# xmlyqing00/V-FloodNet

Measured on AMD Instinct MI355X. Metric: segmented frames/sec at 480p, higher is better.
Workload: dtype f32

## Files before the change

### v-floodnet_amd/_lib.py

```python
import ctypes as C
import os
import re

import torch

_HERE = os.path.dirname(os.path.abspath(__file__))
LIB_PATH = os.environ.get('VFN_LIB_PATH') or os.path.join(_HERE, 'libvfn_hip.so')

_lib = None

c_fp = C.c_void_p

_SCALARS = {'int': C.c_int, 'float': C.c_float, 'double': C.c_double, 'long long': C.c_longlong}
_POINTEES = set(_SCALARS) | {'void', 'char', 'unsigned char', 'short', 'unsigned short', 'unsigned long long'}
_RENAMED = {'in': 'inp'}
_DECLARATOR = re.compile(r'(?:const\s+)?([A-Za-z_][\w ]*?)(?:\s*(\*)\s*|\s+)(\w+)\s*(?:\[([^\]]*)\])?')


def parse_header(text):
    defines, enums, structs, protos = {}, {}, {}, {}

    def fail(why, decl):
        raise RuntimeError(f'vfn_hip.h: {why}: {" ".join(decl.split())[:120]!r}')

    def number(expr, decl):
        try:
            if not re.fullmatch(r'[\w\s()+*-]+', expr):
                raise ValueError(expr)
            return int(eval(expr, {'__builtins__': {}}, {**defines, **enums}))
        except Exception:
            fail(f'cannot evaluate {expr.strip()!r}', decl)

    def declarator(item, decl, param):
        m = _DECLARATOR.fullmatch(item.strip())
        if not m:
            fail('declaration not understood', decl)
        base, star, name, bound = ' '.join(m.group(1).split()), m.group(2), m.group(3), m.group(4)
        if base not in _POINTEES and base not in structs:
            fail(f'unknown base type {base!r}', decl)
        if bound is not None and (star or param):
            fail('array of pointers or array parameter', decl)
        if star:
            if base == 'char':
                t = C.c_char_p
            elif base in structs and param and not name.endswith('_dev'):
                t = C.POINTER(structs[base])
            else:
                t = C.c_void_p
        elif base in _SCALARS:
            t = _SCALARS[base]
        elif base in structs and not param:
            t = structs[base]
        else:
            fail(f'{base!r} by value', decl)
        return _RENAMED.get(name, name), t if bound is None else t * number(bound, decl)

    text = re.sub(r'/\*.*?\*/', ' ', text, flags=re.S)
    text = re.sub(r'//[^\n]*', ' ', text)
    text = re.sub(r'^[ \t]*#[ \t]*ifdef[ \t]+__cplusplus\b.*?^[ \t]*#[ \t]*endif\b[^\n]*$', ' ', text, flags=re.S | re.M)
    code = []
    for line in text.split('\n'):
        if not line.lstrip().startswith('#'):
            code.append(line)
        elif not re.fullmatch(r'\s*#\s*(ifndef\s+\w+|define\s+\w+|endif)\s*', line):
            m = re.fullmatch(r'\s*#\s*define\s+(\w+)\b(?!\()(.+)', line)
            if not m:
                fail('directive not understood', line)
            defines[m.group(1)] = number(m.group(2), line)
    text = '\n'.join(code)

    decls, depth, start = [], 0, 0
    for pos, ch in enumerate(text):
        depth += (ch == '{') - (ch == '}')
        if depth < 0:
            fail('unbalanced declaration', text[start:pos + 1])
        if ch == ';' and depth == 0:
            decls.append(text[start:pos])
            start = pos + 1
    if text[start:].strip():
        fail('unbalanced declaration', text[start:])

    for decl in decls:
        m = re.fullmatch(r'\s*enum\s*\{(.*)\}\s*', decl, flags=re.S)
        if m:
            value = -1
            for item in m.group(1).split(','):
                name, _, expr = item.partition('=')
                value = number(expr, decl) if expr.strip() else value + 1
                enums[name.strip()] = value
            continue
        m = re.fullmatch(r'\s*typedef\s+struct\s*(\w*)\s*\{(.*)\}\s*(\w+)\s*', decl, flags=re.S)
        if m:
            if m.group(1) not in ('', m.group(3)):
                fail('struct tag and typedef name differ', decl)
            fields = []
            for member in m.group(2).split(';'):
                if member.strip():
                    first, *more = member.split(',')
                    head = _DECLARATOR.fullmatch(first.strip())
                    if more and (not head or head.group(2)):
                        fail('several declarators after a pointer', member)
                    fields.append(declarator(first, member, False))
                    fields += [declarator(f'{head.group(1)} {item}', member, False) for item in more]
            structs[m.group(3)] = type(m.group(3), (C.Structure,), {'_fields_': fields})
            continue
        m = re.fullmatch(r'\s*int\s+(vfn_\w+)\s*\((.*)\)\s*', decl, flags=re.S)
        if m:
            if m.group(1) in protos:
                fail('declared twice', decl)
            params = m.group(2).strip()
            protos[m.group(1)] = [] if params == 'void' else [declarator(p, decl, True)[1] for p in params.split(',')]
            continue
        fail('declaration not understood', decl)
    return defines, enums, structs, protos


with open(os.path.join(os.path.dirname(_HERE), 'include', 'vfn_hip.h')) as _f:
    DEFINES, ENUMS, STRUCTS, SIGNATURES = parse_header(_f.read())
ALL_SYMBOLS = sorted(SIGNATURES)
ABI_VERSION = DEFINES['VFN_ABI_VERSION']
TRAIN_AUG_MAX_T, TRAIN_AUG_MAX_SIDE, TRAIN_AUG_MAX_OUT, TRAIN_AUG_MAX_OBJ = (
    DEFINES['VFN_TRAIN_AUG_MAX_' + _k] for _k in ('T', 'SIDE', 'OUT', 'OBJ'))

ConvDesc = STRUCTS['vfn_conv_desc']
WgradDesc = STRUCTS['vfn_wgrad_desc']
RefreshFilter = STRUCTS['vfn_refresh_filter']
RefreshEpilogue = STRUCTS['vfn_refresh_epilogue']
GatherEntry = STRUCTS['vfn_gather_entry']
StemDesc = STRUCTS['vfn_stem_desc']
BankScanDesc = STRUCTS['vfn_bankscan_desc']
MemReadDesc = STRUCTS['vfn_memread_desc']
BankMatchDesc = STRUCTS['vfn_bankmatch_desc']
BankDesc = STRUCTS['vfn_bank_desc']
TrainAugFrame = STRUCTS['vfn_train_aug_frame']
TrainAugDesc = STRUCTS['vfn_train_aug_desc']

DESC_IDS = {ENUMS['VFN_DESC_' + _k]: _c for _k, _c in (
    ('CONV', ConvDesc), ('STEM', StemDesc), ('BANKSCAN', BankScanDesc), ('MEMREAD', MemReadDesc), ('BANK', BankDesc),
    ('WGRAD', WgradDesc), ('REFRESH_FILTER', RefreshFilter), ('REFRESH_EPILOGUE', RefreshEpilogue), ('GATHER', GatherEntry),
    ('BANKMATCH', BankMatchDesc), ('TRAIN_AUG', TrainAugDesc))}


def lib():
    global _lib
    if _lib is None:
        if not os.path.isfile(LIB_PATH):
            raise RuntimeError(
                f'{LIB_PATH} not found: build the HIP kernels first '
                '(python -c "import __graft_entry__ as g; g.build()" or make -C v-floodnet_amd/csrc)')
        L = C.CDLL(LIB_PATH)

        def declare(name):
            if not hasattr(L, name):
                raise RuntimeError(f'{LIB_PATH} lacks {name}, which include/vfn_hip.h declares: rebuild it (make -C v-floodnet_amd/csrc)')
            fn = getattr(L, name)
            fn.argtypes, fn.restype = SIGNATURES[name], C.c_int
            return fn

        if declare('vfn_abi_version')() != ABI_VERSION:
            raise RuntimeError(f'{LIB_PATH} has ABI version {L.vfn_abi_version()}, this package expects {ABI_VERSION} '
                               '(descriptor layouts differ): rebuild it (make -C v-floodnet_amd/csrc)')
        declare('vfn_sizeof_desc')
        for which, cls in DESC_IDS.items():
            if L.vfn_sizeof_desc(which) != C.sizeof(cls):
                raise RuntimeError(f'{LIB_PATH}: sizeof({cls.__name__}) is {L.vfn_sizeof_desc(which)} in the library, '
                                   f'{C.sizeof(cls)} in this binding: rebuild it (make -C v-floodnet_amd/csrc)')
        for name in SIGNATURES:
            declare(name)
        _lib = L
    return _lib


def check(status, what):
    if status != 0:
        raise RuntimeError(f'HIP kernel launcher {what} failed with status {status}')


def ptr(t):
    if t is None:
        return None
    return C.c_void_p(t.data_ptr())


_raw_stream = getattr(torch._C, '_cuda_getCurrentRawStream', None)


def stream():
    if _raw_stream is not None:
        return C.c_void_p(_raw_stream(torch.cuda.current_device()))
    return C.c_void_p(torch.cuda.current_stream().cuda_stream)


def require_gpu(t, what='tensor'):
    if not t.is_cuda:
        raise RuntimeError(f'{what} must live on the GPU: the V-FloodNet hot path has no CPU fallback')


PROBES = []


def independent_stream(device, beside=(), tries=12, priority=0):
    device = torch.device(device)
    cur = torch.cuda.current_stream(device)
    others = [cur] + [s_ for s_ in beside if s_ is not None]
    big, small = torch.zeros(16 * 1024 * 1024, device=device), torch.zeros(16, device=device)

    def overlaps(cand, ref):
        torch.cuda.synchronize(device)
        ref_end, cand_end = torch.cuda.Event(), torch.cuda.Event()
        with torch.cuda.stream(ref):
            for _ in range(64):
                big.add_(1.0)
            ref_end.record()
        with torch.cuda.stream(cand):
            small.add_(1.0)
            cand_end.record()
        cand_end.synchronize()
        ok = not ref_end.query()
        torch.cuda.synchronize(device)
        return ok

    cand = None
    for n_ in range(tries):
        cand = torch.cuda.Stream(device=device, priority=priority)
        if all(overlaps(cand, o_) for o_ in others):
            PROBES.append((True, n_ + 1))
            return cand
    PROBES.append((False, tries))
    import warnings
    warnings.warn('vfloodnet_amd: no stream with a hardware queue of its own found; side-stream work will run in order with the frame loop')
    return cand
```

### v-floodnet_amd/csrc/conv_winograd.hip

```cpp
#include "common.h"
#include "conv_internal.h"
#include "../../include/vfn_hip.h"

namespace {

__device__ __forceinline__ void bt6(const f32x4 (&v)[6], f32x4 (&t)[6]) {
    t[0] = 4.f * v[0] - 5.f * v[2] + v[4];
    t[1] = -4.f * (v[1] + v[2]) + v[3] + v[4];
    t[2] = 4.f * (v[1] - v[2]) - v[3] + v[4];
    t[3] = -2.f * v[1] - v[2] + 2.f * v[3] + v[4];
    t[4] = 2.f * v[1] - v[2] - 2.f * v[3] + v[4];
    t[5] = 4.f * v[1] - 5.f * v[3] + v[5];
}

template <bool LPOUT = false>
__global__ __launch_bounds__(256)
void winograd_input_kernel(const float* __restrict__ x, int N, int H, int W, int C, int ld_x, int relu, float* __restrict__ V,
                           int rows_pad) {
    const int th = (H + 3) / 4, tw = (W + 3) / 4;
    const int c4n = C / 4;
    const long long total = (long long)N * th * tw * c4n;
    const __amdgpu_buffer_rsrc_t rx = __builtin_amdgcn_make_buffer_rsrc(const_cast<float*>(x), 0, (int)((size_t)N * H * W * ld_x * 4), 0x00020000);
    const float floor_ = relu ? 0.f : -INFINITY;
    for (long long i = vfn_xcd_block(blockIdx.x, gridDim.x) * (long long)blockDim.x + threadIdx.x; i < total; i += (long long)gridDim.x * blockDim.x) {
        const int c4 = (int)(i % c4n);
        const int tile = (int)(i / c4n);
        const int tx = tile % tw, ty = (tile / tw) % th, n = tile / (tw * th);
        f32x4 d[6][6];
#pragma unroll
        for (int a = 0; a < 6; ++a) {
            const int yy = 4 * ty - 1 + a;
#pragma unroll
            for (int b = 0; b < 6; ++b) {
                const int xx = 4 * tx - 1 + b;
                const bool ok = (unsigned)yy < (unsigned)H && (unsigned)xx < (unsigned)W;
                const int off = ok ? (((n * H + yy) * W + xx) * ld_x + c4 * 4) * 4 : 0x7ffffff0;
                d[a][b] = __builtin_bit_cast(f32x4, __builtin_amdgcn_raw_buffer_load_b128(rx, off, 0, 0));
            }
        }
#pragma unroll
        for (int a = 0; a < 6; ++a)
#pragma unroll
            for (int b = 0; b < 6; ++b)
#pragma unroll
                for (int e = 0; e < 4; ++e) d[a][b][e] = vfn_floor_nan(d[a][b][e], floor_);
#pragma unroll
        for (int b = 0; b < 6; ++b) {
            f32x4 v[6], t[6];
#pragma unroll
            for (int a = 0; a < 6; ++a) v[a] = d[a][b];
            bt6(v, t);
#pragma unroll
            for (int a = 0; a < 6; ++a) d[a][b] = t[a];
        }
#pragma unroll
        for (int a = 0; a < 6; ++a) {
            f32x4 t[6];
            bt6(d[a], t);
#pragma unroll
            for (int b = 0; b < 6; ++b) {
                if constexpr (LPOUT) {
                    const vfn_bf16x4 h = {(__bf16)t[b][0], (__bf16)t[b][1], (__bf16)t[b][2], (__bf16)t[b][3]};
                    *reinterpret_cast<vfn_bf16x4*>(reinterpret_cast<__bf16*>(V) + ((size_t)(a * 6 + b) * rows_pad + tile) * C + c4 * 4) = h;
                } else {
                    *reinterpret_cast<f32x4*>(V + ((size_t)(a * 6 + b) * rows_pad + tile) * C + c4 * 4) = t[b];
                }
            }
        }
    }
}

__device__ __forceinline__ void at6(const f32x4 (&m)[6], f32x4 (&y)[4]) {
    const f32x4 s12 = m[1] + m[2], d12 = m[1] - m[2], s34 = m[3] + m[4], d34 = m[3] - m[4];
    y[0] = m[0] + s12 + s34;
    y[1] = d12 + 2.f * d34;
    y[2] = s12 + 4.f * s34;
    y[3] = d12 + 8.f * d34 + m[5];
}

template <bool MASK>
__global__ __launch_bounds__(256)
void winograd_output_kernel(const float* __restrict__ Mb, int rows_pad, int N, int H, int W, int Cout,
                            const float* __restrict__ scale, const float* __restrict__ shift, const float* __restrict__ res, int res_ld,
                            int res_mod, int relu_out, float* __restrict__ out, int out_ld, const float* __restrict__ mask, int mask_ld,
                            int mask_after) {
    const int th = (H + 3) / 4, tw = (W + 3) / 4;
    const int c4n = Cout / 4;
    const long long total = (long long)N * th * tw * c4n;
    const int npix = N * H * W;
    const __amdgpu_buffer_rsrc_t ro = __builtin_amdgcn_make_buffer_rsrc(out, 0, (int)((size_t)npix * out_ld * 4), 0x00020000);
    const __amdgpu_buffer_rsrc_t rr = __builtin_amdgcn_make_buffer_rsrc(const_cast<float*>(res ? res : Mb), 0,
                                                                        res ? (int)((size_t)(res_mod > 0 ? res_mod : npix) * res_ld * 4) : 0, 0x00020000);
    const __amdgpu_buffer_rsrc_t rm = __builtin_amdgcn_make_buffer_rsrc(const_cast<float*>(MASK ? mask : Mb), 0,
                                                                        MASK ? (int)((size_t)npix * mask_ld * 4) : 0, 0x00020000);
    const float floor_ = relu_out ? 0.f : -INFINITY;
    for (long long i = vfn_xcd_block(blockIdx.x, gridDim.x) * (long long)blockDim.x + threadIdx.x; i < total; i += (long long)gridDim.x * blockDim.x) {
        const int c4 = (int)(i % c4n);
        const int tile = (int)(i / c4n);
        const int tx = tile % tw, ty = (tile / tw) % th, n = tile / (tw * th);
        f32x4 m[6][6];
#pragma unroll
        for (int a = 0; a < 6; ++a)
#pragma unroll
            for (int b = 0; b < 6; ++b) m[a][b] = *reinterpret_cast<const f32x4*>(Mb + ((size_t)(a * 6 + b) * rows_pad + tile) * Cout + c4 * 4);
        f32x4 sc = {1.f, 1.f, 1.f, 1.f}, sh = {0.f, 0.f, 0.f, 0.f};
        if (scale) sc = *reinterpret_cast<const f32x4*>(scale + c4 * 4);
        if (shift) sh = *reinterpret_cast<const f32x4*>(shift + c4 * 4);
        f32x4 t[6][4];
#pragma unroll
        for (int a = 0; a < 6; ++a) at6(m[a], t[a]);
        int rowi[4][4];
#pragma unroll
        for (int a = 0; a < 4; ++a)
#pragma unroll
            for (int b = 0; b < 4; ++b) {
                const int yy = 4 * ty + a, xx = 4 * tx + b;
                rowi[a][b] = (yy < H && xx < W) ? (n * H + yy) * W + xx : -1;
            }
        f32x4 rv[4][4], mk[MASK ? 4 : 1][MASK ? 4 : 1];
#pragma unroll
        for (int a = 0; a < 4; ++a)
#pragma unroll
            for (int b = 0; b < 4; ++b) {
                const int row = rowi[a][b];
                const int rrow = res_mod > 0 ? row % res_mod : row;
                rv[a][b] = __builtin_bit_cast(f32x4, __builtin_amdgcn_raw_buffer_load_b128(rr, row >= 0 ? (rrow * res_ld + c4 * 4) * 4 : 0x7ffffff0, 0, 0));
                if constexpr (MASK)
                    mk[a][b] = __builtin_bit_cast(f32x4, __builtin_amdgcn_raw_buffer_load_b128(rm, row >= 0 ? (row * mask_ld + c4 * 4) * 4 : 0x7ffffff0, 0, 0));
            }
#pragma unroll
        for (int b = 0; b < 4; ++b) {
            f32x4 col[6], y[4];
#pragma unroll
            for (int a = 0; a < 6; ++a) col[a] = t[a][b];
            at6(col, y);
#pragma unroll
            for (int a = 0; a < 4; ++a) {
                f32x4 v;
#pragma unroll
                for (int e = 0; e < 4; ++e) v[e] = y[a][e] * sc[e] + sh[e];
                if constexpr (MASK) {
                    if (!mask_after) {
#pragma unroll
                        for (int e = 0; e < 4; ++e) v[e] = mk[a][b][e] > 0.f ? v[e] : 0.f;
                    }
                }
                v += rv[a][b];
                if constexpr (MASK) {
                    if (mask_after) {
#pragma unroll
                        for (int e = 0; e < 4; ++e) v[e] = mk[a][b][e] > 0.f ? v[e] : 0.f;
                    }
                }
#pragma unroll
                for (int e = 0; e < 4; ++e) v[e] = vfn_floor_nan(v[e], floor_);
                const int row = rowi[a][b];
                __builtin_amdgcn_raw_buffer_store_b128(__builtin_bit_cast(__attribute__((ext_vector_type(4))) unsigned, v), ro,
                                                       row >= 0 ? (row * out_ld + c4 * 4) * 4 : 0x7ffffff0, 0, 0);
            }
        }
    }
}

__device__ __forceinline__ void a6(const f32x4 (&v)[4], f32x4 (&z)[6]) {
    const f32x4 e = v[0] + v[2], o = v[1] + v[3];
    const f32x4 e4 = v[0] + 4.f * v[2], o8 = 2.f * v[1] + 8.f * v[3];
    z[0] = v[0];
    z[1] = e + o;
    z[2] = e - o;
    z[3] = e4 + o8;
    z[4] = e4 - o8;
    z[5] = v[3];
}

__global__ __launch_bounds__(256)
void winograd_gy_kernel(const float* __restrict__ gy, int N, int H, int W, int C, int ld, float* __restrict__ Z, int rows_pad) {
    const int th = (H + 3) / 4, tw = (W + 3) / 4;
    const int c4n = C / 4;
    const long long total = (long long)N * th * tw * c4n;
    for (long long i = vfn_xcd_block(blockIdx.x, gridDim.x) * (long long)blockDim.x + threadIdx.x; i < total; i += (long long)gridDim.x * blockDim.x) {
        const int c4 = (int)(i % c4n);
        const int tile = (int)(i / c4n);
        const int tx = tile % tw, ty = (tile / tw) % th, n = tile / (tw * th);
        f32x4 t[6][4];
#pragma unroll
        for (int b = 0; b < 4; ++b) {
            f32x4 col[4], z[6];
            const int xx = 4 * tx + b;
#pragma unroll
            for (int a = 0; a < 4; ++a) {
                const int yy = 4 * ty + a;
                f32x4 v = {0.f, 0.f, 0.f, 0.f};
                if (yy < H && xx < W) v = *reinterpret_cast<const f32x4*>(gy + ((size_t)(n * H + yy) * W + xx) * ld + c4 * 4);
                col[a] = v;
            }
            a6(col, z);
#pragma unroll
            for (int a = 0; a < 6; ++a) t[a][b] = z[a];
        }
#pragma unroll
        for (int a = 0; a < 6; ++a) {
            f32x4 z[6];
            a6(t[a], z);
#pragma unroll
            for (int b = 0; b < 6; ++b)
                *reinterpret_cast<f32x4*>(Z + ((size_t)(a * 6 + b) * rows_pad + tile) * C + c4 * 4) = z[b];
        }
    }
}

__device__ __forceinline__ void gt3(const f32x4 (&u)[6], f32x4 (&w)[3]) {
    const f32x4 s12 = u[1] + u[2], d12 = u[2] - u[1], s34 = u[3] + u[4], d34 = u[3] - u[4];
    w[0] = 0.25f * u[0] - (1.f / 6.f) * s12 + (1.f / 24.f) * s34;
    w[1] = (1.f / 6.f) * d12 + (1.f / 12.f) * d34;
    w[2] = -(1.f / 6.f) * s12 + (1.f / 6.f) * s34 + u[5];
}

__global__ __launch_bounds__(256)
void winograd_dw_kernel(const float* __restrict__ dU, int Cout, int Cin, const float* __restrict__ rowscale, float* __restrict__ dw,
                        int accumulate) {
    const int c4n = Cin / 4;
    const long long total = (long long)Cout * c4n;
    const size_t bank = (size_t)Cout * Cin;
    for (long long i = vfn_xcd_block(blockIdx.x, gridDim.x) * (long long)blockDim.x + threadIdx.x; i < total; i += (long long)gridDim.x * blockDim.x) {
        const int c4 = (int)(i % c4n), co = (int)(i / c4n);
        f32x4 t[3][6];
#pragma unroll
        for (int j = 0; j < 6; ++j) {
            f32x4 u[6], w[3];
#pragma unroll
            for (int a = 0; a < 6; ++a) u[a] = *reinterpret_cast<const f32x4*>(dU + (size_t)(a * 6 + j) * bank + (size_t)co * Cin + c4 * 4);
            gt3(u, w);
#pragma unroll
            for (int a = 0; a < 3; ++a) t[a][j] = w[a];
        }
        const float sc = rowscale ? rowscale[co] : 1.f;
#pragma unroll
        for (int a = 0; a < 3; ++a) {
            f32x4 w[3];
            gt3(t[a], w);
#pragma unroll
            for (int b = 0; b < 3; ++b) {
                f32x4* o = reinterpret_cast<f32x4*>(dw + ((size_t)co * 9 + a * 3 + b) * Cin + c4 * 4);
                f32x4 v = w[b] * sc;
                if (accumulate) v += *o;
                *o = v;
            }
        }
    }
}


struct wino_gemm_args {
    const float* V;
    const float* U;
    float* Mb;
    int comps, rows_pad, C, Cout, cout_pad;
    int mtiles, ntiles;
    int a_ld, out_ld, res_ld, res_mod, relu_in, relu_out;
    const float* scale;
    const float* shift;
    const float* res;
};

template <int BM, int BN, int WM, int WN, int PD, bool CONV = false, bool LP = false>
__global__ __launch_bounds__(WM * WN * 64)
void wino_gemm_kernel(const wino_gemm_args p) {
    static_assert(!(CONV && LP), "the reduced-precision form is the transform-domain GEMM only");
    constexpr int BK = 32;
    constexpr int KT = LP ? 64 : 32;
    constexpr int ES = LP ? 2 : 4;
    constexpr int NT = WM * WN * 64;
    constexpr int TM = BM / WM / 32, TN = BN / WN / 32;
    constexpr int AC = BM * 8 / NT, BC = BN * 8 / NT, RSTEP = NT / 8;
    static_assert(AC >= 1 && BC >= 1, "tile too small for the thread count");
    extern __shared__ __attribute__((aligned(16))) char smem[];
    float* sA = reinterpret_cast<float*>(smem);
    float* sB = sA + 2 * BM * BK;

    const int tid = threadIdx.x, lane = tid & 63, wave = tid >> 6;
    const int wm = wave / WN, wn = wave % WN;
    const int li = lane & 31, lh = lane >> 5;

    const int per = p.mtiles * p.ntiles, total = p.comps * per;
    const int gx = (int)gridDim.x >> 3, xcd = (int)blockIdx.x & 7, loc = (int)blockIdx.x >> 3;
    const int q = total >> 3, r8 = total & 7;
    const int u_begin = xcd < r8 ? xcd * (q + 1) : r8 * (q + 1) + (xcd - r8) * q;
    const int u_end = u_begin + q + (xcd < r8 ? 1 : 0);
    const int first = u_begin + loc;
    const int n_units = first < u_end ? (u_end - first + gx - 1) / gx : 0;
    const int nk = p.C / KT;
    const int T = n_units * nk;
    if (T == 0) return;

    const int c16 = tid & 7, r0 = tid >> 3;
    const int a_ld = CONV ? p.a_ld : p.C;
    const __amdgpu_buffer_rsrc_t rsV = __builtin_amdgcn_make_buffer_rsrc(const_cast<float*>(p.V), 0, (int)((size_t)p.comps * p.rows_pad * a_ld * ES), 0x00020000);
    const __amdgpu_buffer_rsrc_t rsU = __builtin_amdgcn_make_buffer_rsrc(const_cast<float*>(p.U), 0, (int)((size_t)p.comps * p.cout_pad * p.C * ES), 0x00020000);
    int a_thr[AC], b_thr[BC];
#pragma unroll
    for (int j = 0; j < AC; ++j) a_thr[j] = (r0 + j * RSTEP) * a_ld * ES + c16 * 16;
#pragma unroll
    for (int j = 0; j < BC; ++j) b_thr[j] = (r0 + j * RSTEP) * p.C * ES + c16 * 16;

    int lu = 0, lkt = 0, la_base = 0, lb_base = 0;
    int n0_cur = 0;
    auto unit_bases = [&](int ui, int& a_base, int& b_base, size_t& o_base, int* n0 = nullptr) {
        const int u = first + ui * gx;
        const int xi = u / per, rem = u - xi * per;
        const int mt = rem / p.ntiles, nt = rem - mt * p.ntiles;
        a_base = (xi * p.rows_pad + mt * BM) * a_ld * ES;
        b_base = (xi * p.cout_pad + nt * BN) * p.C * ES;
        o_base = CONV ? (size_t)mt * BM : ((size_t)xi * p.rows_pad + mt * BM) * p.Cout + nt * BN;
        if (n0) *n0 = nt * BN;
    };
    size_t o_dummy;
    unit_bases(0, la_base, lb_base, o_dummy);
    f32x4 ra[PD][AC], rb[PD][BC];
    auto request = [&](int slot) {
        const int koff = lkt * 128;
#pragma unroll
        for (int j = 0; j < AC; ++j)
            ra[slot][j] = __builtin_bit_cast(f32x4, __builtin_amdgcn_raw_buffer_load_b128(rsV, a_thr[j], la_base + koff, 0));
#pragma unroll
        for (int j = 0; j < BC; ++j)
            rb[slot][j] = __builtin_bit_cast(f32x4, __builtin_amdgcn_raw_buffer_load_b128(rsU, b_thr[j], lb_base + koff, 0));
        if (++lkt == nk) {
            lkt = 0;
            if (++lu < n_units) unit_bases(lu, la_base, lb_base, o_dummy);
        }
    };
    const float relu_floor = (CONV && p.relu_in) ? 0.f : -INFINITY;
    auto stage = [&](int buf, int slot) {
        float* dA = sA + buf * BM * BK;
        float* dB = sB + buf * BN * BK;
#pragma unroll
        for (int j = 0; j < AC; ++j) {
            const int r = r0 + j * RSTEP;
            f32x4 v = ra[slot][j];
            if constexpr (CONV) {
#pragma unroll
                for (int e = 0; e < 4; ++e) v[e] = fmaxf(v[e], relu_floor);
            }
            *reinterpret_cast<f32x4*>(dA + r * BK + ((c16 ^ ((r >> 1) & 7)) << 2)) = v;
        }
#pragma unroll
        for (int j = 0; j < BC; ++j) {
            const int r = r0 + j * RSTEP;
            *reinterpret_cast<f32x4*>(dB + r * BK + ((c16 ^ ((r >> 1) & 7)) << 2)) = rb[slot][j];
        }
    };

    f32x16 acc[TM][TN];
#pragma unroll
    for (int i = 0; i < TM; ++i)
#pragma unroll
        for (int j = 0; j < TN; ++j)
#pragma unroll
            for (int r = 0; r < 16; ++r) acc[i][j][r] = 0.f;

    int cu = 0, ckt = 0, ca_dummy, cb_dummy;
    size_t o_base;
    unit_bases(0, ca_dummy, cb_dummy, o_base, &n0_cur);

#pragma unroll
    for (int d = 0; d < PD; ++d)
        if (d < T) request(d);
    stage(0, 0);
    __syncthreads();

    for (int t0 = 0; t0 < T; t0 += PD) {
#pragma unroll
        for (int uu = 0; uu < PD; ++uu) {
            const int t = t0 + uu;
            if (t >= T) break;
            const int buf = t & 1;
            const bool more = t + 1 < T;
            const bool more_req = t + PD < T;
            const float* cA = sA + buf * BM * BK + (wm * TM * 32) * BK;
            const float* cB = sB + buf * BN * BK + (wn * TN * 32) * BK;
            auto read_frags = [&](int kk, f32x4 (&a)[TM], f32x4 (&b)[TN]) {
                const int lc = 2 * kk + lh;
#pragma unroll
                for (int i = 0; i < TM; ++i) {
                    const int r = i * 32 + li;
                    a[i] = *reinterpret_cast<const f32x4*>(cA + r * BK + ((lc ^ ((r >> 1) & 7)) << 2));
                }
#pragma unroll
                for (int j = 0; j < TN; ++j) {
                    const int r = j * 32 + li;
                    b[j] = *reinterpret_cast<const f32x4*>(cB + r * BK + ((lc ^ ((r >> 1) & 7)) << 2));
                }
            };
            f32x4 fa[2][TM], fb[2][TN];
            read_frags(0, fa[0], fb[0]);
#pragma unroll
            for (int kk = 0; kk < 4; ++kk) {
                if (PD > 1 && kk == 0 && more) stage(buf ^ 1, (uu + 1) % PD);
                if (kk == 1 && more_req) request(uu);
                if (PD == 1 && kk == 3 && more) stage(buf ^ 1, 0);
                if (kk + 1 < 4) read_frags(kk + 1, fa[(kk + 1) & 1], fb[(kk + 1) & 1]);
                if constexpr (LP) {
                    typedef __attribute__((ext_vector_type(8))) __bf16 bf16x8_;
#pragma unroll
                    for (int i = 0; i < TM; ++i)
#pragma unroll
                        for (int j = 0; j < TN; ++j)
                            acc[i][j] = __builtin_amdgcn_mfma_f32_32x32x16_bf16(__builtin_bit_cast(bf16x8_, fa[kk & 1][i]), __builtin_bit_cast(bf16x8_, fb[kk & 1][j]),
                                                                                acc[i][j], 0, 0, 0);
                } else {
#pragma unroll
                for (int e = 0; e < 4; ++e)
#pragma unroll
                    for (int i = 0; i < TM; ++i)
#pragma unroll
                        for (int j = 0; j < TN; ++j)
                            acc[i][j] = __builtin_amdgcn_mfma_f32_32x32x2f32(fa[kk & 1][i][e], fb[kk & 1][j][e], acc[i][j], 0, 0, 0);
                }
            }
            if (++ckt == nk) {
                if constexpr (CONV) {
                    const int m0 = (int)o_base;
                    const int npix = p.rows_pad;
                    const __amdgpu_buffer_rsrc_t rso = __builtin_amdgcn_make_buffer_rsrc(p.Mb, 0, (int)((size_t)npix * p.out_ld * 4), 0x00020000);
                    const __amdgpu_buffer_rsrc_t rsr = __builtin_amdgcn_make_buffer_rsrc(const_cast<float*>(p.res ? p.res : p.V), 0,
                        p.res ? (int)((size_t)(p.res_mod > 0 ? p.res_mod : npix) * p.res_ld * 4) : 0, 0x00020000);
                    const float floor_ = p.relu_out ? 0.f : -INFINITY;
                    float rv[TM][TN][16];
#pragma unroll
                    for (int j = 0; j < TN; ++j) {
                        const int col = n0_cur + (wn * TN + j) * 32 + li;
#pragma unroll
                        for (int i = 0; i < TM; ++i)
#pragma unroll
                            for (int r = 0; r < 16; ++r) {
                                const int row = m0 + (wm * TM + i) * 32 + 4 * lh + (r & 3) + 8 * (r >> 2);
                                const int rrow = p.res_mod > 0 ? row % p.res_mod : row;
                                rv[i][j][r] = __builtin_bit_cast(float, __builtin_amdgcn_raw_buffer_load_b32(
                                    rsr, (row < npix && col < p.Cout) ? (rrow * p.res_ld + col) * 4 : 0x7ffffff0, 0, 0));
                            }
                    }
#pragma unroll
                    for (int j = 0; j < TN; ++j) {
                        const int col = n0_cur + (wn * TN + j) * 32 + li;
                        const bool cok = col < p.Cout;
                        const float sc = (p.scale && cok) ? p.scale[col] : 1.f;
                        const float sh = (p.shift && cok) ? p.shift[col] : 0.f;
#pragma unroll
                        for (int i = 0; i < TM; ++i)
#pragma unroll
                            for (int r = 0; r < 16; ++r) {
                                const int row = m0 + (wm * TM + i) * 32 + 4 * lh + (r & 3) + 8 * (r >> 2);
                                const float v = vfn_floor_nan(acc[i][j][r] * sc + sh + rv[i][j][r], floor_);
                                __builtin_amdgcn_raw_buffer_store_b32(__builtin_bit_cast(unsigned, v), rso,
                                                                      (row < npix && cok) ? (row * p.out_ld + col) * 4 : 0x7ffffff0, 0, 0);
                                acc[i][j][r] = 0.f;
                            }
                    }
                } else {
                float* o = p.Mb + o_base;
#pragma unroll
                for (int j = 0; j < TN; ++j) {
                    const int col = (wn * TN + j) * 32 + li;
#pragma unroll
                    for (int i = 0; i < TM; ++i) {
                        const int rbase = (wm * TM + i) * 32 + 4 * lh;
#pragma unroll
                        for (int r = 0; r < 16; ++r) {
                            if (n0_cur + col < p.Cout)
                                o[(size_t)(rbase + (r & 3) + 8 * (r >> 2)) * p.Cout + col] = acc[i][j][r];
                            acc[i][j][r] = 0.f;
                        }
                    }
                }
                }
                ckt = 0;
                if (++cu < n_units) unit_bases(cu, ca_dummy, cb_dummy, o_base, &n0_cur);
            }
            __syncthreads();
        }
    }
}

template <int BM, int BN, int WM, int WN, int PD, bool CONV, bool LP>
int launch_wino_gemm(const wino_gemm_args& a, int wgs, hipStream_t s) {
    constexpr size_t lds = 2 * (size_t)(BM + BN) * 32 * sizeof(float);
    static const bool lds_ready = vfn_allow_lds(&wino_gemm_kernel<BM, BN, WM, WN, PD, CONV, LP>, lds);
    (void)lds_ready;
    wino_gemm_args p = a;
    p.mtiles = (a.rows_pad + BM - 1) / BM;
    p.ntiles = (a.Cout + BN - 1) / BN;
    const int total = p.comps * p.mtiles * p.ntiles;
    int grid = wgs > 0 ? wgs : 512;
    if (grid > total) grid = total;
    grid = (grid + 7) / 8 * 8;
    hipLaunchKernelGGL((wino_gemm_kernel<BM, BN, WM, WN, PD, CONV, LP>), dim3(grid), dim3(WM * WN * 64), lds, s, p);
    return vfn_check_launch();
}

constexpr int kWinoTile[4][4] = {{128, 128, 4, 2}, {64, 128, 2, 4}, {128, 64, 4, 2}, {64, 64, 2, 2}};
constexpr int kWinoCfgs = 8;

template <bool CONV, bool LP>
int launch_wino_cfg(const wino_gemm_args& a, int cfg, int wgs, hipStream_t s) {
    return vfn_dispatch<kWinoCfgs>(cfg, [&](auto id) -> int {
        constexpr int c = decltype(id)::value;
        constexpr const int* t = kWinoTile[c & 3];
        return launch_wino_gemm<t[0], t[1], t[2], t[3], 1 + (c >> 2), CONV, LP>(a, wgs, s);
    });
}

inline bool tensors_fit_32bit(int N, int H, int W, int ld, int res_ld, int mask_ld, int res_mod) {
    const long long px = (long long)N * H * W;
    return px * ld * 4 < 0x7fffff00LL && (res_mod > 0 ? (long long)res_mod : px) * res_ld * 4 < 0x7fffff00LL && px * mask_ld * 4 < 0x7fffff00LL;
}

inline int grid_of(long long total) {
    long long b = (total + 255) / 256;
    return (int)(b < 16384 ? (b ? b : 1) : 16384);
}

}

extern "C" int vfn_winograd_tiles(int N, int H, int W) { return N * ((H + 3) / 4) * ((W + 3) / 4); }

extern "C" int vfn_winograd_input_f32(const float* x, int N, int H, int W, int C, int ld_x, int relu, float* V, int rows_pad, void* stream) {
    if (!x || !V || N < 1 || H < 1 || W < 1 || C < 4 || C % 4 || ld_x < C || ld_x % 4 || rows_pad < vfn_winograd_tiles(N, H, W)) return VFN_ERR_ARG;
    const long long total = (long long)vfn_winograd_tiles(N, H, W) * (C / 4);
    if (!tensors_fit_32bit(N, H, W, ld_x, 0, 0, 0)) return VFN_ERR_ARG;
    hipLaunchKernelGGL(winograd_input_kernel<false>, dim3(grid_of(total)), dim3(256), 0, (hipStream_t)stream, x, N, H, W, C, ld_x, relu, V, rows_pad);
    return vfn_check_launch();
}

extern "C" int vfn_winograd_output_f32(const float* Mb, int rows_pad, int N, int H, int W, int Cout, const float* scale, const float* shift,
                                       const float* res, int res_ld, int res_mod, int relu_out, float* out, int out_ld, void* stream) {
    if (!Mb || !out || N < 1 || H < 1 || W < 1 || Cout < 4 || Cout % 4 || out_ld < Cout || out_ld % 4 || (res && res_ld % 4) ||
        rows_pad < vfn_winograd_tiles(N, H, W)) return VFN_ERR_ARG;
    const long long total = (long long)vfn_winograd_tiles(N, H, W) * (Cout / 4);
    if (!tensors_fit_32bit(N, H, W, out_ld, res ? res_ld : 0, 0, res_mod)) return VFN_ERR_ARG;
    hipLaunchKernelGGL(winograd_output_kernel<false>, dim3(grid_of(total)), dim3(256), 0, (hipStream_t)stream, Mb, rows_pad, N, H, W, Cout, scale, shift,
                       res, res_ld, res_mod, relu_out, out, out_ld, (const float*)nullptr, 0, 0);
    return vfn_check_launch();
}

extern "C" int vfn_winograd_output_masked_f32(const float* Mb, int rows_pad, int N, int H, int W, int Cout, const float* res, int res_ld,
                                              const float* mask, int mask_ld, int mask_after, float* out, int out_ld, void* stream) {
    if (!Mb || !out || N < 1 || H < 1 || W < 1 || Cout < 4 || Cout % 4 || out_ld < Cout || out_ld % 4 || (res && res_ld % 4) ||
        (mask && mask_ld % 4) || rows_pad < vfn_winograd_tiles(N, H, W)) return VFN_ERR_ARG;
    const long long total = (long long)vfn_winograd_tiles(N, H, W) * (Cout / 4);
    if (!tensors_fit_32bit(N, H, W, out_ld, res ? res_ld : 0, mask ? mask_ld : 0, 0)) return VFN_ERR_ARG;
    if (mask)
        hipLaunchKernelGGL(winograd_output_kernel<true>, dim3(grid_of(total)), dim3(256), 0, (hipStream_t)stream, Mb, rows_pad, N, H, W, Cout,
                           (const float*)nullptr, (const float*)nullptr, res, res_ld, 0, 0, out, out_ld, mask, mask_ld, mask_after);
    else
        hipLaunchKernelGGL(winograd_output_kernel<false>, dim3(grid_of(total)), dim3(256), 0, (hipStream_t)stream, Mb, rows_pad, N, H, W, Cout,
                           (const float*)nullptr, (const float*)nullptr, res, res_ld, 0, 0, out, out_ld, (const float*)nullptr, 0, 0);
    return vfn_check_launch();
}

extern "C" int vfn_winograd_gy_f32(const float* gy, int N, int H, int W, int C, int ld, float* Z, int rows_pad, void* stream) {
    if (!gy || !Z || N < 1 || H < 1 || W < 1 || C < 4 || C % 4 || ld < C || ld % 4 || rows_pad < vfn_winograd_tiles(N, H, W)) return VFN_ERR_ARG;
    const long long total = (long long)vfn_winograd_tiles(N, H, W) * (C / 4);
    hipLaunchKernelGGL(winograd_gy_kernel, dim3(grid_of(total)), dim3(256), 0, (hipStream_t)stream, gy, N, H, W, C, ld, Z, rows_pad);
    return vfn_check_launch();
}

extern "C" int vfn_winograd_dw_f32(const float* dU, int Cout, int Cin, const float* rowscale, float* dw, int accumulate, void* stream) {
    if (!dU || !dw || Cout < 1 || Cin < 4 || Cin % 4) return VFN_ERR_ARG;
    hipLaunchKernelGGL(winograd_dw_kernel, dim3(grid_of((long long)Cout * (Cin / 4))), dim3(256), 0, (hipStream_t)stream, dU, Cout, Cin, rowscale,
                       dw, accumulate);
    return vfn_check_launch();
}

extern "C" int vfn_winograd_gemm_f32(const float* V, const float* U, float* Mb, int comps, int rows_pad, int C, int Cout, int cout_pad, int cfg,
                                     int wgs, void* stream) {
    if (!V || !U || !Mb || comps < 1 || rows_pad < 1 || C < 32 || C % 32 || Cout < 1 || cout_pad < Cout || cfg < 0 || cfg >= kWinoCfgs) return VFN_ERR_ARG;
    const int bm = kWinoTile[cfg & 3][0], bn = kWinoTile[cfg & 3][1];
    if (rows_pad % bm || cout_pad < (Cout + bn - 1) / bn * bn) return VFN_ERR_ARG;
    if ((long long)comps * rows_pad * C * 4 >= 0x7fffff00LL || (long long)comps * cout_pad * C * 4 >= 0x7fffff00LL) return VFN_ERR_ARG;
    wino_gemm_args a{V, U, Mb, comps, rows_pad, C, Cout, cout_pad, 0, 0, 0, 0, 0, 0, 0, 0, nullptr, nullptr, nullptr};
    return launch_wino_cfg<false, false>(a, cfg, wgs, (hipStream_t)stream);
}

extern "C" int vfn_conv1x1_persistent_f32(const vfn_conv_desc* d, int cfg, int wgs, void* stream) {
    if (!d || !d->in || !d->w || !d->out || cfg < 0 || cfg >= kWinoCfgs) return VFN_ERR_ARG;
    if (d->KH != 1 || d->KW != 1 || d->stride != 1 || d->pad != 0 || d->mask || d->in_lp || d->out_lp || d->w_packed || d->ksplit > 1 ||
        d->w_batch_rows || d->Cin % 32 || d->in_ld % 4 || d->M < 1 || d->M != d->N * d->H * d->W) return VFN_ERR_ARG;
    const int bn = kWinoTile[cfg & 3][1];
    if (d->cout_pad < (d->Cout + bn - 1) / bn * bn) return VFN_ERR_ARG;
    const long long lim = 0x7fffff00LL;
    if ((long long)d->M * d->in_ld * 4 >= lim || (long long)d->M * d->out_ld * 4 >= lim || (long long)d->cout_pad * d->Cin * 4 >= lim ||
        (d->res && (long long)(d->res_mod > 0 ? d->res_mod : d->M) * d->res_ld * 4 >= lim)) return VFN_ERR_ARG;
    wino_gemm_args a{d->in, d->w, d->out, 1, d->M, d->Cin, d->Cout, d->cout_pad, 0, 0,
                     d->in_ld, d->out_ld, d->res ? d->res_ld : 0, d->res_mod, d->relu_in, d->relu_out, d->scale, d->shift, d->res};
    return launch_wino_cfg<true, false>(a, cfg, wgs, (hipStream_t)stream);
}

extern "C" int vfn_winograd_input_bf16(const float* x, int N, int H, int W, int C, int ld_x, int relu, void* V, int rows_pad, void* stream) {
    if (!x || !V || N < 1 || H < 1 || W < 1 || C < 4 || C % 4 || ld_x < C || ld_x % 4 || rows_pad < vfn_winograd_tiles(N, H, W)) return VFN_ERR_ARG;
    const long long total = (long long)vfn_winograd_tiles(N, H, W) * (C / 4);
    if (!tensors_fit_32bit(N, H, W, ld_x, 0, 0, 0)) return VFN_ERR_ARG;
    hipLaunchKernelGGL(winograd_input_kernel<true>, dim3(grid_of(total)), dim3(256), 0, (hipStream_t)stream, x, N, H, W, C, ld_x, relu,
                       reinterpret_cast<float*>(V), rows_pad);
    return vfn_check_launch();
}

extern "C" int vfn_winograd_gemm_bf16(const void* V, const void* U, float* Mb, int comps, int rows_pad, int C, int Cout, int cout_pad, int cfg,
                                      int wgs, void* stream) {
    if (!V || !U || !Mb || comps < 1 || rows_pad < 1 || C < 64 || C % 64 || Cout < 1 || cout_pad < Cout || cfg < 0 || cfg >= kWinoCfgs) return VFN_ERR_ARG;
    const int bm = kWinoTile[cfg & 3][0], bn = kWinoTile[cfg & 3][1];
    if (rows_pad % bm || cout_pad < (Cout + bn - 1) / bn * bn) return VFN_ERR_ARG;
    if ((long long)comps * rows_pad * C * 2 >= 0x7fffff00LL || (long long)comps * cout_pad * C * 2 >= 0x7fffff00LL) return VFN_ERR_ARG;
    wino_gemm_args a{reinterpret_cast<const float*>(V), reinterpret_cast<const float*>(U), Mb, comps, rows_pad, C, Cout, cout_pad, 0, 0, 0, 0, 0, 0, 0, 0,
                     nullptr, nullptr, nullptr};
    return launch_wino_cfg<false, true>(a, cfg, wgs, (hipStream_t)stream);
}
```

### v-floodnet_amd/csrc/refresh.hip

```cpp
#include "common.h"
#include "../../include/vfn_hip.h"

namespace {

constexpr int ELEMS_PER_BLOCK = 4096;

__device__ __forceinline__ float bn_scale(const float* gamma, const float* var, float eps, int c) {
    return __fdiv_rn(gamma[c], __fsqrt_rn(__fadd_rn(var[c], eps)));
}

__global__ __launch_bounds__(256)
void refresh_filters_kernel(const vfn_refresh_filter* __restrict__ table, int n) {
    int lo = 0, hi = n - 1;
    while (lo < hi) {
        const int mid = (lo + hi + 1) >> 1;
        if (table[mid].block0 <= (int)blockIdx.x) lo = mid; else hi = mid - 1;
    }
    const vfn_refresh_filter e = table[lo];
    const int T = e.kh * e.kw;
    const long long base = (long long)((int)blockIdx.x - e.block0) * ELEMS_PER_BLOCK;
    if (e.kind >= 4) {
        const long long pairs = (long long)e.cout * e.cin;
        const double G[6][3] = {{0.25, 0.0, 0.0}, {-1.0 / 6, -1.0 / 6, -1.0 / 6}, {-1.0 / 6, 1.0 / 6, -1.0 / 6},
                                {1.0 / 24, 1.0 / 12, 1.0 / 6}, {1.0 / 24, -1.0 / 12, 1.0 / 6}, {0.0, 0.0, 1.0}};
        for (int i = threadIdx.x; i < ELEMS_PER_BLOCK; i += 256) {
            const long long idx = base + i;
            if (idx >= pairs) return;
            int co, ci;
            if (e.kind == 4) { ci = (int)(idx % e.cin); co = (int)(idx / e.cin); }
            else { co = (int)(idx % e.cout); ci = (int)(idx / e.cout); }
            const float* g = e.src + ((size_t)co * e.cin_total + e.cin_off + ci) * 9;
            const float sc = e.gamma ? bn_scale(e.gamma, e.var, e.eps, co) : 1.f;
            double w[3][3];
#pragma unroll
            for (int t = 0; t < 9; ++t) {
                float v = g[e.kind == 4 ? t : 8 - t];
                if (e.gamma) v = __fmul_rn(v, sc);
                w[t / 3][t % 3] = (double)v;
            }
            double tmp[6][3];
#pragma unroll
            for (int a = 0; a < 6; ++a)
#pragma unroll
                for (int b = 0; b < 3; ++b) tmp[a][b] = G[a][0] * w[0][b] + G[a][1] * w[1][b] + G[a][2] * w[2][b];
            const size_t row = e.kind == 4 ? (size_t)(e.dst_row0 + co) : (size_t)(e.dst_row0 + ci);
            const size_t col = e.kind == 4 ? (size_t)ci : (size_t)(e.dst_col0 + co);
#pragma unroll
            for (int a = 0; a < 6; ++a)
#pragma unroll
                for (int b = 0; b < 6; ++b) {
                    const double u = tmp[a][0] * G[b][0] + tmp[a][1] * G[b][1] + tmp[a][2] * G[b][2];
                    e.dst[((size_t)(a * 6 + b) * e.cout_ld + row) * e.dst_ld + col] = (float)u;
                }
        }
        return;
    }
    const long long total = (long long)e.cout * e.cin * T;
    if (e.kind <= 1 && T == 9) {
        const long long pairs = (long long)e.cout * e.cin;
        const int per = ELEMS_PER_BLOCK / 9 + 1;
        for (int i = threadIdx.x; i < per; i += 256) {
            const long long idx = (long long)((int)blockIdx.x - e.block0) * per + i;
            if (idx >= pairs) return;
            int co, ci;
            if (e.kind == 0) { ci = (int)(idx % e.cin); co = (int)(idx / e.cin); }
            else { co = (int)(idx % e.cout); ci = (int)(idx / e.cout); }
            const float* g = e.src + ((size_t)co * e.cin_total + e.cin_off + ci) * 9;
            const float sc = e.gamma ? bn_scale(e.gamma, e.var, e.eps, co) : 1.f;
#pragma unroll
            for (int t = 0; t < 9; ++t) {
                float v = g[t];
                if (e.gamma) v = __fmul_rn(v, sc);
                const size_t dst = e.kind == 0 ? (size_t)(e.dst_row0 + co) * e.dst_ld + (size_t)t * e.cin + ci
                                               : (size_t)(e.dst_row0 + ci) * e.dst_ld + (size_t)(8 - t) * e.cout_ld + e.dst_col0 + co;
                e.dst[dst] = v;
            }
        }
        return;
    }
    for (int i = threadIdx.x; i < ELEMS_PER_BLOCK; i += 256) {
        const long long idx = base + i;
        if (idx >= total) return;
        int co, ci, t;
        size_t dst;
        if (e.kind == 0) {
            ci = (int)(idx % e.cin);
            t = (int)((idx / e.cin) % T);
            co = (int)(idx / ((long long)e.cin * T));
            dst = (size_t)(e.dst_row0 + co) * e.dst_ld + (size_t)t * e.cin + ci;
        } else if (e.kind == 1) {
            co = (int)(idx % e.cout);
            const int tf = (int)((idx / e.cout) % T);
            ci = (int)(idx / ((long long)e.cout * T));
            t = T - 1 - tf;
            dst = (size_t)(e.dst_row0 + ci) * e.dst_ld + (size_t)tf * e.cout_ld + e.dst_col0 + co;
        } else if (e.kind == 2) {
            co = (int)(idx % e.cout);
            t = (int)((idx / e.cout) % T);
            ci = (int)(idx / ((long long)e.cout * T));
            const int y = t / e.kw, x = t % e.kw;
            dst = ((size_t)((e.dst_row0 + ci) * e.kh + y) * 8 + x) * e.dst_ld + co;
        } else {
            ci = (int)(idx % e.cin);
            co = (int)((idx / e.cin) % e.cout);
            t = (int)(idx / ((long long)e.cin * e.cout));
            dst = (size_t)(e.dst_row0 + t * e.cout + co) * e.dst_ld + ci;
        }
        float v = e.src[((size_t)co * e.cin_total + e.cin_off + ci) * T + t];
        if (e.gamma) v = __fmul_rn(v, bn_scale(e.gamma, e.var, e.eps, co));
        e.dst[dst] = v;
    }
}

__global__ __launch_bounds__(256)
void refresh_epilogues_kernel(const vfn_refresh_epilogue* __restrict__ table) {
    const vfn_refresh_epilogue e = table[blockIdx.x];
    for (int c = threadIdx.x; c < e.C; c += 256) {
        if (e.gamma) {
            const float s = bn_scale(e.gamma, e.var, e.eps, c);
            if (e.scale) e.scale[c] = s;
            if (e.shift) e.shift[c] = __fsub_rn(e.beta[c], __fmul_rn(e.mean[c], s));
        } else if (e.shift) {
            e.shift[c] = e.beta ? e.beta[c] : 0.f;
        }
    }
}

}

extern "C" int vfn_refresh_elems_per_block(void) { return ELEMS_PER_BLOCK; }

extern "C" int vfn_refresh_filters_f32(const vfn_refresh_filter* table, int n, int total_blocks, void* stream) {
    if (!table || n < 1 || total_blocks < 1) return VFN_ERR_ARG;
    hipLaunchKernelGGL(refresh_filters_kernel, dim3(total_blocks), dim3(256), 0, (hipStream_t)stream, table, n);
    return vfn_check_launch();
}

extern "C" int vfn_refresh_epilogues_f32(const vfn_refresh_epilogue* table, int n, void* stream) {
    if (!table || n < 1) return VFN_ERR_ARG;
    hipLaunchKernelGGL(refresh_epilogues_kernel, dim3(n), dim3(256), 0, (hipStream_t)stream, table);
    return vfn_check_launch();
}

namespace {
__global__ __launch_bounds__(256)
void gather_strided_kernel(const vfn_gather_entry* __restrict__ table, int n, float* __restrict__ dst) {
    int lo = 0, hi = n - 1;
    while (lo < hi) {
        const int mid = (lo + hi + 1) >> 1;
        if (table[mid].block0 <= (int)blockIdx.x) lo = mid; else hi = mid - 1;
    }
    const vfn_gather_entry e = table[lo];
    const long long total = (long long)e.shape[0] * e.shape[1] * e.shape[2] * e.shape[3];
    const long long base = (long long)((int)blockIdx.x - e.block0) * ELEMS_PER_BLOCK;
    float* out = dst + e.dst_offset;
    for (int i = threadIdx.x; i < ELEMS_PER_BLOCK; i += 256) {
        const long long idx = base + i;
        if (idx >= total) return;
        long long r = idx;
        const int i3 = (int)(r % e.shape[3]); r /= e.shape[3];
        const int i2 = (int)(r % e.shape[2]); r /= e.shape[2];
        const int i1 = (int)(r % e.shape[1]);
        const int i0 = (int)(r / e.shape[1]);
        out[idx] = e.src[i0 * e.stride[0] + i1 * e.stride[1] + i2 * e.stride[2] + i3 * e.stride[3]];
    }
}
}

extern "C" int vfn_gather_strided_f32(const vfn_gather_entry* table, int n, int total_blocks, float* dst, void* stream) {
    if (!table || !dst || n < 1 || total_blocks < 1) return VFN_ERR_ARG;
    hipLaunchKernelGGL(gather_strided_kernel, dim3(total_blocks), dim3(256), 0, (hipStream_t)stream, table, n, dst);
    return vfn_check_launch();
}
```

### v-floodnet_amd/engine.py

```python
import math
import os

import torch

from . import _lib, ops, weights as W
from ._lib import ptr, stream, check, MemReadDesc, BankScanDesc
from .feature_bank import pick_nsplit, pick_scan_slices, MAX_SPLIT, MAX_SPLIT_SCAN, QT_SCAN, DK, DV

_CFG_EFF = {(128, 128): 1.00, (128, 64): 0.95, (64, 128): 0.95, (64, 64): 0.86, (32, 64): 0.74,
            (64, 32): 0.74, (128, 32): 0.80, (256, 128): 0.97}
_CFG_TILES = None
_TUNED = {}
_TUNED_PATH = __import__('os').path.join(__import__('os').path.dirname(__import__('os').path.abspath(__file__)),
                                         'tuned_gfx950.json')
_TUNED_BF16 = {}
_TUNED_BF16_PATH = _TUNED_PATH.replace('tuned_gfx950.json', 'tuned_gfx950_bf16.json')
_TUNED_BF16X3 = {}
_TUNED_BF16X3_PATH = _TUNED_PATH.replace('tuned_gfx950.json', 'tuned_gfx950_bf16x3.json')
_TABLES = (_TUNED, _TUNED_BF16, _TUNED_BF16X3)
_TABLE_PATHS = (_TUNED_PATH, _TUNED_BF16_PATH, _TUNED_BF16X3_PATH)


def _load_tuned():
    import json
    import os
    if os.environ.get('VFN_IGNORE_TUNED') == '1':
        return
    for path, table in zip(_TABLE_PATHS, _TABLES):
        alt = os.environ.get('VFN_TUNED_DIR')
        if alt and os.path.isfile(os.path.join(alt, os.path.basename(path))):
            path = os.path.join(alt, os.path.basename(path))
        if os.path.isfile(path):
            for k, v in json.load(open(path)).items():
                t = (int(v[0]), int(v[1]), int(v[2]) if len(v) > 2 else 0)
                table[tuple(int(x) for x in k.split(','))] = t + tuple(int(x) for x in v[3:6]) if len(v) >= 6 else t


def save_tuned(path=None, mode=0):
    import json
    table = _TABLES[mode]
    with open(path or _TABLE_PATHS[mode], 'w') as f:
        json.dump({','.join(str(x) for x in k): list(v) for k, v in sorted(table.items())}, f, indent=0)


_load_tuned()


def pad_divide_by(h, w, d=16):
    new_h = h + d - h % d if h % d > 0 else h
    new_w = w + d - w % d if w % d > 0 else w
    lh = int((new_h - h) / 2)
    uh = int(new_h - h) - lh
    lw = int((new_w - w) / 2)
    uw = int(new_w - w) - lw
    return (lw, uw, lh, uh), new_h, new_w


WS_FLOATS = 16 * 1024 * 1024
_WINOGRAD_TRAIN = os.environ.get('VFN_WINOGRAD_TRAIN', '1') == '1'
_BATCH_MEMREAD = os.environ.get('VFN_TRAIN_BATCH_MEMREAD', '1') == '1'
MAX_GROUP = 16
_TRAIN_SLOTS = int(os.environ.get('VFN_TRAIN_SLOTS', 2))
_WINOGRAD = os.environ.get('VFN_WINOGRAD', '1')
_WINOGRAD_LP = os.environ.get('VFN_WINOGRAD_LP', '1') == '1'
_WINOGRAD_MIN_M = int(os.environ.get('VFN_WINOGRAD_MIN_M', 10000))
_WINO_TABLE = {}
_WINO_TABLE_BF16 = {}
_WINO_PATH = os.path.join(os.path.dirname(os.path.abspath(__file__)), 'wino_gfx950.json')
if os.environ.get('VFN_IGNORE_TUNED') != '1':
    for _path, _tab in ((_WINO_PATH, _WINO_TABLE), (_WINO_PATH.replace('.json', '_bf16.json'), _WINO_TABLE_BF16)):
        if os.path.isfile(_path):
            _tab.update({tuple(int(x) for x in k.split(',')): int(v) for k, v in __import__('json').load(open(_path)).items()})
_INLAUNCH_SPLITK = __import__('os').environ.get('VFN_INLAUNCH_SPLITK', '1') == '1'


def _tiles():
    global _CFG_TILES
    if _CFG_TILES is None:
        _CFG_TILES = ops.conv_cfg_tiles()
    return _CFG_TILES


def apply_choice(desc, choice, ws, counters=None):
    cfg, ks, split_from = choice[:3]
    if ks > 1 and (desc.out_ld % 4 or (desc.res and desc.res_ld % 4)):
        ks, split_from = 1, 0
    if cfg >= ops.PCONV_CFG0 and not ops.pconv_eligible(desc, 0):
        fb = tuple(choice[3:6]) if len(choice) >= 6 else choose_cfg(desc.M, desc.Cout, desc.KH * desc.KW * desc.Cin, 0, use_table=False)
        return apply_choice(desc, fb, ws, counters)
    if cfg >= ops.WINO_GEMM_CFG0:
        ops.set_splitk(desc, 1, None)
        return cfg
    if ops.conv_cfg_kind(cfg) == 2:
        if counters is None or ws is None or ws.numel() < ops.SK_WS_FLOATS:
            ws, counters = ops.streamk_scratch(ws.device if ws is not None else torch.device('cuda', torch.cuda.current_device()))
        ops.set_streamk(desc, ws, counters)
        return cfg
    if ks > 1:
        bm, bn = _tiles()[cfg]
        n_tiles = (desc.Cout + bn - 1) // bn
        rows = desc.M - (split_from // n_tiles) * bm
        if desc.Cout % bn or not _INLAUNCH_SPLITK or ops.conv_cfg_kind(cfg) != 0 or desc.w_packed or desc.in_lp or desc.out_lp:
            counters = None
        ops.set_splitk(desc, ks, ws, split_from, rows, counters)
    else:
        ops.set_splitk(desc, 1, None)
    return cfg


def _scores_buffer(p, fb):
    if os.environ.get('VFN_STORE_SCORES', '1') == '0':
        return None
    per_obj = ((fb._cap + 63) // 64) * ((p.HW + 127) // 128) * 8192
    if fb.obj_n * per_obj * 4 > float(os.environ.get('VFN_SCORES_MAX_GB', 48)) * 2 ** 30:
        return None
    key = (fb.obj_n, per_obj)
    if getattr(p, '_scores_key', None) != key:
        p._scores = torch.empty(fb.obj_n, per_obj, device=p.dec_in.device)
        p._scores_key = key
    return p._scores


def choose_cfg(M, cout, K, mode=0, use_table=True):
    global _CFG_TILES
    key = (M, cout, K)
    table = _TABLES[mode]
    if use_table and key in table:
        return table[key]
    _tiles()
    nk = K // (64 if mode == 1 else 32)
    best, best_cost = 0, None
    for c, (bm, bn) in enumerate(_CFG_TILES[:8]):
        if bn > 32 and cout <= 32:
            continue
        if bn >= 128 and cout < 128:
            continue
        blocks = ((M + bm - 1) // bm) * ((cout + bn - 1) // bn)
        rounds = (blocks + 255) // 256
        cost = rounds * bm * bn / _CFG_EFF[(bm, bn)]
        if best_cost is None or cost < best_cost:
            best, best_cost = c, cost
    c = 2 if cout >= 128 else 3
    bm, bn = _CFG_TILES[c]
    blocks = ((M + bm - 1) // bm) * ((cout + bn - 1) // bn)
    if blocks < 200 and nk >= 16 and cout % 4 == 0 and cout >= 64:
        ks = max(1, min(16, (448 + blocks - 1) // blocks, nk // 4))
        while ks > 1 and (((nk + ks - 1) // ks) * (ks - 1) >= nk or ks * M * cout > WS_FLOATS):
            ks -= 1
        return (c, ks, 0)
    return (best, 1, 0)


def tune_desc(d, bf, ws, cnt, iters=3, cfg_filter=None, allow_split=True):
    tiles = ops.conv_cfg_tiles()
    key = (d.M, d.Cout, d.KH * d.KW * d.Cin)

    def timeit(c):
        ops.conv2d_launch(d, c, bf)
        torch.cuda.synchronize()
        best_ms = None
        for _ in range(3):
            e0, e1 = torch.cuda.Event(enable_timing=True), torch.cuda.Event(enable_timing=True)
            e0.record()
            for _ in range(iters):
                ops.conv2d_launch(d, c, bf)
            e1.record()
            torch.cuda.synchronize()
            ms = e0.elapsed_time(e1)
            best_ms = ms if best_ms is None else min(best_ms, ms)
        return best_ms

    best, best_t = None, None
    if d.w_batch_rows > 0 and bf == 1:
        for c in ops.wino_gemm_cfg_options(d.w_batch_rows, d.Cout):
            if cfg_filter is not None and not cfg_filter(key, c):
                continue
            t = timeit(c)
            if best_t is None or t < best_t:
                best, best_t = (c, 1, 0), t
        return best
    if d.w_batch_rows > 0 and bf == 0 and d.M // d.w_batch_rows * d.w_batch_rows == d.M:
        for c in ops.wino_gemm_cfg_options(d.w_batch_rows, d.Cout):
            if cfg_filter is not None and not cfg_filter(key, c):
                continue
            apply_choice(d, (c, 1, 0), ws, cnt)
            try:
                t = timeit(c)
            except RuntimeError:
                continue
            if best_t is None or t < best_t:
                best, best_t = (c, 1, 0), t
    if ops.pconv_eligible(d, bf) and os.environ.get('VFN_PCONV', '1') == '1':
        for c in ops.pconv_cfg_options(d.Cout):
            if cfg_filter is not None and not cfg_filter(key, c):
                continue
            apply_choice(d, (c, 1, 0), ws, cnt)
            try:
                t = timeit(c)
            except RuntimeError:
                continue
            if best_t is None or t < best_t:
                best, best_t = (c, 1, 0), t
    for c, (bm, bn) in enumerate(tiles):
        if c not in ops.conv_cfgs(bf):
            continue
        if cfg_filter is not None and not cfg_filter(key, c):
            continue
        if d.cout_pad < ((d.Cout + bn - 1) // bn) * bn:
            continue
        if (bn > 64 and d.Cout <= 32) or (bn > 128 and d.Cout < 256):
            continue
        blocks = ((d.M + bm - 1) // bm) * ((d.Cout + bn - 1) // bn)
        options = [(c, 1, 0)]
        wk = ops.conv_cfg_wk(c)
        kind = ops.conv_cfg_kind(c)
        if kind == 2:
            if blocks > ops.SK_MAX_TILES:
                continue
        elif not allow_split:
            pass
        elif kind == 1 and wk > 1:
            if blocks < 256:
                options += [(c, k_, 0) for k_ in ops.valid_splits(d, 8, bf)[1:] if k_ * d.M * d.Cout <= WS_FLOATS]
        elif wk > 1 or ops.conv_cfg_tpb(c) > 1:
            if blocks > 1024 or d.KH * d.KW * d.Cin // (64 if bf == 1 else 32) < 2 * wk:
                continue
        elif blocks < 256:
            options += [(c, k_, 0) for k_ in ops.valid_splits(d, 16, bf)[1:] if k_ * d.M * d.Cout <= WS_FLOATS]
        else:
            options += [(c, k_, full) for (full, k_, rows) in ops.tail_split_options(d, bm, bn, 8, bf)
                        if k_ * rows * d.Cout <= WS_FLOATS and k_ in (2, 3, 4, 5, 6, 8)]
        for opt in options:
            apply_choice(d, opt, ws, cnt)
            t = timeit(c)
            if best_t is None or t < best_t:
                best, best_t = opt, t
    return best


class ConvLayer:

    def __init__(self, conv, bn=None, device=None, cin_range=None, with_bias=True, reg=None):
        w = conv.weight.detach().float()
        if cin_range is not None:
            w = w[:, cin_range[0]:cin_range[1]].contiguous()
        self.cout, self.cin, self.k, _ = w.shape
        self.stride = conv.stride[0]
        self.pad = conv.padding[0]
        self.w = ops.pad_rows(W.pack_conv_weight(w)).to(device)
        sc, sh = W.conv_epilogue(conv, bn)
        if not with_bias:
            sh = torch.zeros_like(sh)
        self.scale = sc.to(device).contiguous()
        self.shift = sh.to(device).contiguous()
        self._w_lp = {}
        self._wino_src = None
        if reg is not None and isinstance(conv, torch.nn.Module):
            from .refresh import FORWARD
            self._wino_src = [(reg, conv.weight, cin_range[0] if cin_range is not None else 0, 0)]
            reg.add_filter(conv.weight, self.w, FORWARD, cin=self.cin, cin_off=cin_range[0] if cin_range is not None else 0)
            if bn is not None:
                reg.add_epilogue(self.scale, self.shift if with_bias else None, bn=bn, eps=W.BN_EPS)
            elif conv.bias is not None and with_bias:
                reg.add_epilogue(None, self.shift, bias=conv.bias)

    def refresh_derived(self):
        for mode, t in self._w_lp.items():
            if mode == 'wino':
                if self._wino_src is not None:
                    continue
                w = self.w[:self.cout].view(self.cout, 3, 3, self.cin).permute(0, 3, 1, 2)
                t.copy_(ops.pack_winograd_weight(w).to(t.device))
            elif mode == 'wino_bf16':
                w = self.w[:self.cout].view(self.cout, 3, 3, self.cin).permute(0, 3, 1, 2)
                t.copy_(ops.pack_winograd_weight_bf16(w).to(t.device))
            else:
                new = ops.pack_weights_lp(self.w, mode)
                t.copy_(new)

    def w_lp(self, mode):
        if mode not in self._w_lp:
            self._w_lp[mode] = ops.pack_weights_lp(self.w, mode)
        return self._w_lp[mode]

    def w_wino(self):
        if 'wino' not in self._w_lp:
            assert self.k == 3
            w = self.w[:self.cout].view(self.cout, 3, 3, self.cin).permute(0, 3, 1, 2)
            self._w_lp['wino'] = ops.pack_winograd_weight(w).to(self.w.device)
            if self._wino_src is not None:
                from .refresh import WINO
                for reg, weight, cin_off, row0 in self._wino_src:
                    reg.add_filter(weight, self._w_lp['wino'], WINO, cin=self.cin, cin_off=cin_off, dst_ld=self.cin, dst_row0=row0,
                                   cout_ld=self._w_lp['wino'].shape[0] // 36)
        return self._w_lp['wino']

    def w_wino_bf16(self):
        if 'wino_bf16' not in self._w_lp:
            assert self.k == 3
            w = self.w[:self.cout].view(self.cout, 3, 3, self.cin).permute(0, 3, 1, 2)
            self._w_lp['wino_bf16'] = ops.pack_winograd_weight_bf16(w).to(self.w.device)
        return self._w_lp['wino_bf16']


class Pred2Layer:
    TAPS = 20

    def __init__(self, conv, device, reg=None):
        w = conv.weight.detach().float().cpu()
        assert w.shape[0] == 2 and w.shape[2:] == (3, 3)
        self.cin = w.shape[1]
        w18 = torch.zeros(self.TAPS, self.cin)
        for dy in range(3):
            for dx in range(3):
                for o in range(2):
                    w18[(dy * 3 + dx) * 2 + o] = w[o, :, dy, dx]
        self.cout, self.k, self.stride, self.pad = self.TAPS, 1, 1, 0
        self.w = ops.pad_rows(w18.contiguous()).to(device)
        self.scale = torch.ones(self.TAPS, device=device)
        self.shift = torch.zeros(self.TAPS, device=device)
        self.bias = conv.bias.detach().float().to(device).contiguous().clone()
        self._w_lp = {}
        self._wino_src = None
        if reg is not None:
            from .refresh import TAPS
            reg.add_filter(conv.weight, self.w, TAPS)
            reg.add_epilogue(None, self.bias, bias=conv.bias)

    refresh_derived = ConvLayer.refresh_derived

    def w_lp(self, mode):
        if mode not in self._w_lp:
            self._w_lp[mode] = ops.pack_weights_lp(self.w, mode)
        return self._w_lp[mode]


class Launch:
    __slots__ = ('fn', 'args', 'name', 'flops')

    def __init__(self, fn, args, name, flops=0.0):
        self.fn, self.args, self.name, self.flops = fn, args, name, flops

    def __call__(self):
        self.fn(*self.args)


_GRAPHS = os.environ.get('VFN_GRAPHS', '1') == '1'


class GraphCache:

    def __init__(self):
        self.graphs = {}
        self.runs = {}
        self.captures = 0

    def invalidate(self):
        self.graphs.clear()
        self.runs.clear()

    def run(self, lst, lo=0, hi=None, eager=False):
        hi = len(lst) if hi is None else hi
        if hi <= lo:
            return
        key = (id(lst), lo, hi)
        g = None if (eager or not _GRAPHS) else self.graphs.get(key)
        if g is not None:
            g.replay()
            return
        n = self.runs.get(key, 0)
        if eager or not _GRAPHS or n < 2 or hi - lo < 4:
            for l in lst[lo:hi]:
                l()
            if not eager:
                self.runs[key] = n + 1
            return
        g = torch.cuda.CUDAGraph()
        cur = torch.cuda.current_stream()
        cap = torch.cuda.Stream(device=cur.device)
        cap.wait_stream(cur)
        try:
            with torch.cuda.graph(g, stream=cap, capture_error_mode='thread_local'):
                for l in lst[lo:hi]:
                    l()
        except Exception:
            import warnings
            warnings.warn('vfloodnet_amd: HIP graph capture of a launch list failed; running it eagerly')
            self.runs[key] = -10 ** 9
            if torch.cuda.is_current_stream_capturing():
                raise RuntimeError('vfloodnet_amd: the stream is still capturing after a failed HIP graph capture')
            cur.wait_stream(cap)
            for l in lst[lo:hi]:
                l()
            return
        cur.wait_stream(cap)
        self.graphs[key] = g
        self.captures += 1
        g.replay()

    def warm(self, lst, lo=0, hi=None):
        hi = len(lst) if hi is None else hi
        if not _GRAPHS or hi - lo < 4:
            return
        key = (id(lst), lo, hi)
        while key not in self.graphs and self.runs.get(key, 0) >= 0:
            self.run(lst, lo, hi)


class FramePlan:

    def __init__(self, eng, H0, W0, obj_n, keep_acts=False):
        self.eng = eng
        self.graphs = GraphCache()
        self.keep_acts = keep_acts
        self.acts_m = {}
        self.H0, self.W0, self.obj_n = H0, W0, obj_n
        self.pad, self.Hp, self.Wp = pad_divide_by(H0, W0)
        dev = eng.device
        self.h2, self.w2 = self.Hp // 2, self.Wp // 2
        self.h4, self.w4 = self.Hp // 4, self.Wp // 4
        self.h8, self.w8 = self.Hp // 8, self.Wp // 8
        self.h16, self.w16 = self.Hp // 16, self.Wp // 16
        self.HW = self.h16 * self.w16
        f = lambda *s: torch.empty(*s, device=dev, dtype=torch.float32)
        K = obj_n
        self.frame_in = f(3, H0, W0)
        self.mask_in = f(K, H0, W0)
        self.qsets = [QuerySet(self), QuerySet(self)]
        self._qbatch = {}
        self.m = self._trunk_buffers(K)
        self.kv_m = f(K, self.HW, DK + DV)
        self.ml = f(K, self.HW, 2)
        self.ml_part = f(K, MAX_SPLIT_SCAN, self.HW, 2)
        self.work = torch.zeros(4, dtype=torch.int32, device=dev)
        self.o_part = f(K, MAX_SPLIT, self.HW, DV)
        self.dec_in = f(K, self.h16, self.w16, DV)
        self.d16 = [f(K, self.h16, self.w16, 256) for _ in range(3)]
        self.d8 = [f(K, self.h8, self.w8, 256) for _ in range(3)]
        self.d4 = [f(K, self.h4, self.w4, 256) for _ in range(3)]
        self.pp = f(K, self.h4, self.w4, 2)
        self.z4 = f(K, self.h4, self.w4, Pred2Layer.TAPS)
        self.z2 = f(K, self.h2, self.w2, Pred2Layer.TAPS)
        self.p_up = f(K, self.h2, self.w2, 2)
        self.rough = f(K, self.h2, self.w2)
        self.unc = f(self.h2, self.w2)
        fused_ok = K <= 4
        self.hs = None if fused_ok else f(K, self.h2, self.w2, 64)
        self.hr = None if fused_ok else f(K, self.h2, self.w2)
        self.hm = None if fused_ok else f(K, self.h2, self.w2)
        self.lm = f(K, self.h2, self.w2, 64)
        self.conf = f(K, self.h2, self.w2)
        self.l2 = [f(K, self.h2, self.w2, 32) for _ in range(3)]
        self.qq = f(K, self.h2, self.w2, 2)
        self.score = f(1, K, H0, W0)
        self._twins = {}
        self._lp_state = {}
        self.ws = f(WS_FLOATS)
        self.ws_q = f(WS_FLOATS)
        self.cnt = torch.zeros(ops.SK_MAX_TILES, dtype=torch.int32, device=dev)
        self.cnt_q = torch.zeros(ops.SK_MAX_TILES, dtype=torch.int32, device=dev)
        self._ws_cur, self._cnt_cur = self.ws, self.cnt
        self._wino = {}

        self.mem = []
        self._build()

    @property
    def seg_pre(self):
        return self.qsets[0].pre[1]

    @property
    def seg_post(self):
        return self.qsets[0].post[0]

    @property
    def kv_q(self):
        return self.qsets[0].kv_q[0:1]

    def all_lists(self):
        out = [self.mem]
        for qs in self.qsets:
            out += [qs.pre[1], qs.pre[2], qs.post[0], qs.post[1]]
        for qs in self._qbatch.values():
            out += [qs.pre[qs.nq]]
            if qs._dec_batch is not None:
                out += [qs._dec_batch.post]
        return out

    def batch_set(self, n):
        qs = self._qbatch.get(n)
        if qs is None:
            qs = self._qbatch[n] = QuerySet(self, nq=n)
            qs.build()
        return qs

    def _trunk_buffers(self, N):
        dev = self.eng.device
        f = lambda *s: torch.empty(*s, device=dev, dtype=torch.float32)
        b = {}
        b['r1'] = f(N, self.h2, self.w2, 64)
        b['x4'] = f(N, self.h4, self.w4, 64)
        for name, (h, w, planes) in {'res2': (self.h4, self.w4, 64), 'res3': (self.h8, self.w8, 128),
                                     'res4': (self.h16, self.w16, 256)}.items():
            hin, win = (h * 2, w * 2) if name != 'res2' else (h, w)
            b[name] = dict(t1a=f(N, hin, win, planes), t1=f(N, h, w, planes), t2=f(N, h, w, planes),
                           ds=f(N, h, w, planes * 4), o=[f(N, h, w, planes * 4) for _ in range(2)],
                           out=f(N, h, w, planes * 4))
        return b

    def _lp_args(self, out):
        if not self.eng.any_x3 or out.shape[-1] % 32:
            return ()
        self._lp_state[(out.data_ptr(), tuple(out.shape))] = True
        return (self.lp_twin(out), True)

    def lp_twin(self, t):
        st = t.untyped_storage()
        key = st.data_ptr()
        if key not in self._twins:
            self._twins[key] = torch.empty(st.nbytes() // 4, dtype=torch.float32, device=t.device)
        return torch.as_strided(self._twins[key], t.size(), t.stride(), t.storage_offset())

    def has_lp(self, t, relu):
        return self._lp_state.get((t.data_ptr(), tuple(t.shape))) == bool(relu)

    def _conv(self, lst, layer, x, out, N, H, Wd, res=None, relu_in=False, relu_out=False, name='conv',
              in_ld=None, out_ld=None, res_mod=0, lp_out=None, f32_out=True):
        bf = self.eng.layer_mode(name)
        lp = bf == 2
        if self.eng.mixed:
            f32_out = True
        if ((bf == 0 or (bf == 1 and _WINOGRAD_LP and not self.keep_acts and layer.cin % 64 == 0)) and in_ld is None and
                (_WINOGRAD_TRAIN or not self.keep_acts) and x.shape[-1] == layer.cin and self.eng.use_winograd(layer, N * H * Wd, bf)):
            return self._conv_winograd(lst, layer, x, out, N, H, Wd, res, relu_in, relu_out, name, out_ld, res_mod, bf)
        d = ops.make_conv_desc(x, layer.w, layer.cout, layer.k, layer.k, layer.stride, layer.pad, out,
                               layer.scale, layer.shift, res, relu_in, relu_out,
                               cin=layer.cin, in_ld=in_ld if in_ld is not None else x.shape[-1],
                               out_ld=out_ld, N=N, H=H, W=Wd)
        d.res_mod = int(res_mod)
        if lp and in_ld is None and layer.cin % 32 == 0 and self.has_lp(x, relu_in):
            d.inp, d.in_lp, d.relu_in = ptr(self.lp_twin(x)), 1, 0
        if lp and lp_out and layer.cout % 32 == 0 and d.out_ld % 32 == 0:
            d.out_lp, d.out_lp_relu = ptr(self.lp_twin(out)), int(lp_out == 'relu')
            self._lp_state[(out.data_ptr(), tuple(out.shape))] = (lp_out == 'relu')
            if not f32_out:
                d.out = None
        else:
            self._lp_state.pop((out.data_ptr(), tuple(out.shape)), None)
        K = layer.k * layer.k * layer.cin
        if bf == 1 and layer.cin % 64:
            bf = 2
        if bf:
            ops.use_packed_weights(d, layer.w_lp(bf))
        choice = choose_cfg(d.M, layer.cout, K, bf)
        if choice[1] > 1 and (d.out_ld % 4 or (res is not None and d.res_ld % 4)):
            choice = (choice[0], 1, 0)
        cfg = apply_choice(d, choice, self._ws_cur, self._cnt_cur)
        lst.append(Launch(ops.conv2d_launch, (d, cfg, bf), f'{name}[{d.M}x{layer.cout}x{K}]', 2.0 * d.M * layer.cout * K))
        return out

    def _conv_winograd(self, lst, layer, x, out, N, H, Wd, res, relu_in, relu_out, name, out_ld, res_mod, bf=0):
        rows = ops.winograd_rows(N, H, Wd)
        key = id(self._ws_cur)
        need_v, need_m = 36 * rows * layer.cin, 36 * rows * layer.cout
        V, Mb = self._wino.get(key, (None, None))
        if V is None or V.numel() < need_v or Mb.numel() < need_m:
            dev = self.eng.device
            V = torch.zeros(max(need_v, V.numel() if V is not None else 0), device=dev)
            Mb = torch.empty(max(need_m, Mb.numel() if Mb is not None else 0), device=dev)
            self._wino[key] = (V, Mb)
        Mb = Mb[:need_m].view(36 * rows, layer.cout)
        if bf == 1:
            V = V.view(torch.bfloat16)[:need_v].view(36 * rows, layer.cin)
            U = layer.w_wino_bf16()
        else:
            V = V[:need_v].view(36 * rows, layer.cin)
            U = layer.w_wino()
        lst.append(Launch(ops.winograd_input, (x, V, rows, relu_in, N, H, Wd, layer.cin, x.shape[-1]), name + '.wino_in'))
        dg = ops.make_winograd_gemm_desc(V, U, Mb, rows, layer.cin, layer.cout)
        if bf:
            choice = _TABLES[bf].get((dg.M, layer.cout, layer.cin))
            if choice is None or choice[0] < ops.WINO_GEMM_CFG0:
                tc = 5 if rows % 64 == 0 and layer.cout >= 128 and rows >= 1024 else 3
                choice = (ops.wino_gemm_cfg(tc, 512), 1, 0)
        else:
            choice = choose_cfg(dg.M, layer.cout, layer.cin, 0)
        cfg = apply_choice(dg, choice, self._ws_cur, self._cnt_cur)
        lst.append(Launch(ops.conv2d_launch, (dg, cfg, bf), f'{name}.wino_gemm[{dg.M}x{layer.cout}x{layer.cin}]', 2.0 * dg.M * layer.cout * layer.cin))
        self._lp_state.pop((out.data_ptr(), tuple(out.shape)), None)
        lst.append(Launch(ops.winograd_output, (Mb, rows, out, N, H, Wd, layer.cout, layer.scale, layer.shift, res,
                                                res.shape[-1] if res is not None else 0, res_mod, relu_out,
                                                out_ld if out_ld is not None else out.shape[-1]), name + '.wino_out'))
        return out

    def _trunk(self, lst, enc, bufs, N, prefix, acts=None):
        x = bufs['x4']
        lst.append(Launch(ops.maxpool3x3s2, (bufs['r1'], x), prefix + '.maxpool'))
        H, Wd = self.h4, self.w4
        for lname in ('res2', 'res3', 'res4'):
            blocks = enc[lname]
            lb = bufs[lname]
            for bi, blk in enumerate(blocks):
                s = blk['conv2'].stride
                Ho, Wo = H // s, Wd // s
                t1 = lb['t1a'] if (s == 2) else lb['t1']
                t2, ds_buf = lb['t2'], lb['ds']
                if self.keep_acts:
                    t1, t2 = torch.empty_like(t1), torch.empty_like(lb['t2'])
                    ds_buf = torch.empty_like(lb['ds'])
                nm = f'{prefix}.{lname}.{bi}'
                self._conv(lst, blk['conv1'], x, t1, N, H, Wd, relu_out=True, name=nm + '.conv1', lp_out='plain', f32_out=False)
                self._conv(lst, blk['conv2'], t1, t2, N, H, Wd, relu_out=True, name=nm + '.conv2', lp_out='plain',
                           f32_out=False)
                if 'down' in blk:
                    self._conv(lst, blk['down'], x, ds_buf, N, H, Wd, name=nm + '.down')
                    idn = ds_buf
                else:
                    idn = x
                out = lb['out'] if bi == len(blocks) - 1 else lb['o'][bi % 2]
                if self.keep_acts and bi != len(blocks) - 1:
                    out = torch.empty_like(out)
                self._conv(lst, blk['conv3'], t2, out, N, Ho, Wo, res=idn, relu_out=True, name=nm + '.conv3',
                           lp_out='plain')
                if self.keep_acts and acts is not None:
                    acts[(lname, bi)] = dict(x=x, t1=t1, t2=t2, ds=ds_buf if 'down' in blk else None, out=out, stride=s, H=H, W=Wd)
                x = out
                H, Wd = Ho, Wo
        return x

    def _resblock(self, lst, rb, x, t, out, N, H, Wd, name):
        self._conv(lst, rb['conv1'], x, t, N, H, Wd, relu_in=True, name=name + '.conv1', lp_out='relu', f32_out=False)
        self._conv(lst, rb['conv2'], t, out, N, H, Wd, res=x, relu_in=True, name=name + '.conv2')
        return out

    def _build(self):
        e = self.eng
        K = self.obj_n
        for qs in self.qsets:
            qs.build()
        self._ws_cur, self._cnt_cur = self.ws, self.cnt
        self.stem_m = ops.make_stem_desc(self.frame_in, self.mask_in, e.stem_m_w, e.stem_m_scale, e.stem_m_shift,
                                         self.m['r1'], e.mean, e.std, K, self.H0, self.W0, self.pad, self.Hp, self.Wp)
        self.mem.append(Launch(ops.stem_launch, (self.stem_m,), 'encoder_m.stem',
                               2.0 * K * self.h2 * self.w2 * 64 * 245))
        r4m = self._trunk(self.mem, e.enc_m, self.m, K, 'encoder_m', acts=self.acts_m)
        self._conv(self.mem, e.keyval, r4m, self.kv_m, K, self.h16, self.w16, name='keyval')

    def conv_flops(self, which):
        return sum(l.flops for l in getattr(self, which))


class QuerySet:

    def __init__(self, plan, nq=2):
        self.plan = plan
        self.nq = nq
        p = plan
        f = lambda *s_: torch.empty(*s_, device=p.eng.device, dtype=torch.float32)
        self.frames = f(nq, 3, p.H0, p.W0)
        self.q = p._trunk_buffers(nq)
        self.kv_q = f(nq, p.HW, DK + DV)
        self.fm_q = f(nq, p.h16, p.w16, 256)
        self.s8 = [f(nq, p.h8, p.w8, 256) for _ in range(3)]
        self.s4 = [f(nq, p.h4, p.w4, 256) for _ in range(3)]
        self.lq = f(nq, p.h2, p.w2, 32)
        self.sizes = sorted({1, nq})
        self.pre = {n: [] for n in self.sizes}
        self.acts = {n: {} for n in self.sizes}
        self.post = [[] for _ in range(nq)]
        self.split = {n: 0 for n in self.sizes}
        self.keys = [None] * nq
        self.held = [None] * nq
        self.consumed = [True] * nq
        self.stage = 0
        self.n = 0
        self.done = None
        self._dec_batch = None

    def dec_batch(self):
        if self._dec_batch is None:
            self._dec_batch = DecoderBatch(self.plan, self)
        return self._dec_batch

    @staticmethod
    def _sl(t, n):
        return t[0:n]

    def build(self):
        p, e = self.plan, self.plan.eng
        K = p.obj_n
        D = e.dec
        for n in self.sizes:
            P = self.pre[n]
            sl = lambda t: t[0:n]
            q = {k: (sl(v) if torch.is_tensor(v) else {kk: ([sl(x) for x in vv] if isinstance(vv, list) else sl(vv)) for kk, vv in v.items()})
                 for k, v in self.q.items()}
            p._ws_cur, p._cnt_cur = p.ws_q, p.cnt_q
            for i in range(n):
                d = ops.make_stem_desc(self.frames[i], None, e.stem_q_w, e.stem_q_scale, e.stem_q_shift,
                                       self.q['r1'][i:i + 1], e.mean, e.std, 1, p.H0, p.W0, p.pad, p.Hp, p.Wp)
                P.append(Launch(ops.stem_launch, (d,), 'encoder_q.stem', 2.0 * p.h2 * p.w2 * 64 * 147))
            r4 = p._trunk(P, e.enc_q, q, n, 'encoder_q', acts=self.acts[n])
            p._conv(P, e.keyval, r4, sl(self.kv_q), n, p.h16, p.w16, name='keyval')
            kvq_val = sl(self.kv_q)[:, :, DK:]
            p._conv(P, D['convFM_q'], kvq_val, sl(self.fm_q), n, p.h16, p.w16, name='decoder.convFM.q', in_ld=DK + DV)
            s8, s4 = [sl(t) for t in self.s8], [sl(t) for t in self.s4]
            p._conv(P, D['RF3']['convFS'], q['res3']['out'], s8[0], n, p.h8, p.w8, name='decoder.RF3.convFS', lp_out='relu')
            p._resblock(P, D['RF3']['ResFS'], s8[0], s8[1], s8[2], n, p.h8, p.w8, 'decoder.RF3.ResFS')
            p._conv(P, D['RF2']['convFS'], q['res2']['out'], s4[0], n, p.h4, p.w4, name='decoder.RF2.convFS', lp_out='relu')
            p._resblock(P, D['RF2']['ResFS'], s4[0], s4[1], s4[2], n, p.h4, p.w4, 'decoder.RF2.ResFS')
            p._conv(P, D['local_convFM_r1'], q['r1'], sl(self.lq), n, p.h2, p.w2, name='decoder.local_convFM.r1')
            est = [l.flops / 100e12 + 6e-6 for l in P]
            half, acc = 0.5 * sum(est), 0.0
            for i, t_ in enumerate(est):
                acc += t_
                if acc >= half:
                    self.split[n] = i + 1
                    break
        p._ws_cur, p._cnt_cur = p.ws, p.cnt
        d16, d8, d4 = p.d16, p.d8, p.d4
        for slot in range(self.nq):
            L = self.post[slot]
            o = lambda t: t[slot:slot + 1]
            p._conv(L, D['convFM_m'], p.dec_in, d16[0], K, p.h16, p.w16, res=o(self.fm_q), res_mod=p.HW,
                    name='decoder.convFM.mem', lp_out='relu')
            p._resblock(L, D['ResMM'], d16[0], d16[1], d16[2], K, p.h16, p.w16, 'decoder.ResMM')
            L.append(Launch(ops.upsample2x_add, (o(self.s8[2]), d16[2], d8[0], True) + p._lp_args(d8[0]), 'decoder.RF3.up_add'))
            p._resblock(L, D['RF3']['ResMM'], d8[0], d8[1], d8[2], K, p.h8, p.w8, 'decoder.RF3.ResMM')
            L.append(Launch(ops.upsample2x_add, (o(self.s4[2]), d8[2], d4[0], True) + p._lp_args(d4[0]), 'decoder.RF2.up_add'))
            p._resblock(L, D['RF2']['ResMM'], d4[0], d4[1], d4[2], K, p.h4, p.w4, 'decoder.RF2.ResMM')
            p._conv(L, D['pred2'], d4[2], p.z4, K, p.h4, p.w4, relu_in=True, name='decoder.pred2.taps')
            L.append(Launch(ops.pred2_gather, (p.z4, D['pred2'].bias, p.pp), 'decoder.pred2.gather'))
            L.append(Launch(ops.rough_uncertainty, (p.pp, p.p_up, p.rough, p.unc), 'decoder.rough_unc'))
            L.append(Launch(ops.local_stats, (self.q['r1'][slot], p.rough, p.hs, p.hr, p.hm, p.lm, p.conf),
                            'decoder.local_stats'))
            l2 = p.l2
            p._conv(L, D['local_convFM_loc'], p.lm, l2[0], K, p.h2, p.w2, res=o(self.lq),
                    res_mod=p.h2 * p.w2, name='decoder.local_convFM.local', lp_out='relu')
            p._resblock(L, D['local_ResMM'], l2[0], l2[1], l2[2], K, p.h2, p.w2, 'decoder.local_ResMM')
            p._conv(L, D['local_pred2'], l2[2], p.z2, K, p.h2, p.w2, relu_in=True, name='decoder.local_pred2.taps')
            L.append(Launch(ops.pred2_gather, (p.z2, D['local_pred2'].bias, p.qq), 'decoder.local_pred2.gather'))
            L.append(Launch(ops.final_logits, (p.p_up, p.unc, p.conf, p.qq, p.score, p.pad, p.H0, p.W0), 'decoder.final_logits'))


class DecoderBatch:

    def __init__(self, plan, qs):
        self.plan, self.qs, self.G = plan, qs, qs.nq
        p, G, K = plan, qs.nq, plan.obj_n
        N = G * K
        self.N = N
        f = lambda *s_: torch.empty(*s_, device=p.eng.device, dtype=torch.float32)
        self.dec_in = f(N, p.h16, p.w16, DV)
        self.d16 = [f(N, p.h16, p.w16, 256) for _ in range(3)]
        self.d8 = [f(N, p.h8, p.w8, 256) for _ in range(3)]
        self.d4 = [f(N, p.h4, p.w4, 256) for _ in range(3)]
        self.pp = f(N, p.h4, p.w4, 2)
        self.z4 = f(N, p.h4, p.w4, Pred2Layer.TAPS)
        self.z2 = f(N, p.h2, p.w2, Pred2Layer.TAPS)
        self.p_up = f(N, p.h2, p.w2, 2)
        self.rough = f(N, p.h2, p.w2)
        self.unc = f(G, p.h2, p.w2)
        self.lm = f(N, p.h2, p.w2, 64)
        self.conf = f(N, p.h2, p.w2)
        self.l2 = [f(N, p.h2, p.w2, 32) for _ in range(3)]
        self.qq = f(N, p.h2, p.w2, 2)
        self.score = f(G, K, p.H0, p.W0)
        self._mr = None
        self.post = []
        self._build()

    @property
    def mr(self):
        if self._mr is None:
            import types
            p, G, K = self.plan, self.G, self.plan.obj_n
            f = lambda *s_: torch.empty(*s_, device=p.eng.device, dtype=torch.float32)
            HWb = G * p.HW
            self._mr = types.SimpleNamespace(HW=HWb, ml=f(K, HWb, 2), ml_part=f(K, MAX_SPLIT_SCAN, HWb, 2), o_part=f(K, MAX_SPLIT, HWb, DV),
                                             work=torch.zeros(4, dtype=torch.int32, device=p.eng.device), dec_in=f(K, HWb, DV))
        return self._mr

    def __getattr__(self, name):
        return getattr(self.plan, name)

    def grp(self, t, g):
        K = self.plan.obj_n
        return t[g * K:(g + 1) * K]

    def _build(self):
        p, qs, G = self.plan, self.qs, self.G
        K, N = p.obj_n, self.N
        D = p.eng.dec
        L = self.post
        grp = self.grp
        p._ws_cur, p._cnt_cur = p.ws, p.cnt
        d16, d8, d4, l2 = self.d16, self.d8, self.d4, self.l2
        for g in range(G):
            p._conv(L, D['convFM_m'], grp(self.dec_in, g), grp(d16[0], g), K, p.h16, p.w16, res=qs.fm_q[g:g + 1], res_mod=p.HW,
                    name='decoder.convFM.mem', lp_out='relu')
        p._resblock(L, D['ResMM'], d16[0], d16[1], d16[2], N, p.h16, p.w16, 'decoder.ResMM')
        for g in range(G):
            L.append(Launch(ops.upsample2x_add, (qs.s8[2][g:g + 1], grp(d16[2], g), grp(d8[0], g), True), 'decoder.RF3.up_add'))
        p._resblock(L, D['RF3']['ResMM'], d8[0], d8[1], d8[2], N, p.h8, p.w8, 'decoder.RF3.ResMM')
        for g in range(G):
            L.append(Launch(ops.upsample2x_add, (qs.s4[2][g:g + 1], grp(d8[2], g), grp(d4[0], g), True), 'decoder.RF2.up_add'))
        p._resblock(L, D['RF2']['ResMM'], d4[0], d4[1], d4[2], N, p.h4, p.w4, 'decoder.RF2.ResMM')
        p._conv(L, D['pred2'], d4[2], self.z4, N, p.h4, p.w4, relu_in=True, name='decoder.pred2.taps')
        L.append(Launch(ops.pred2_gather, (self.z4, D['pred2'].bias, self.pp), 'decoder.pred2.gather'))
        for g in range(G):
            L.append(Launch(ops.rough_uncertainty, (grp(self.pp, g), grp(self.p_up, g), grp(self.rough, g), self.unc[g]), 'decoder.rough_unc'))
            L.append(Launch(ops.local_stats, (qs.q['r1'][g], grp(self.rough, g), p.hs, p.hr, p.hm, grp(self.lm, g), grp(self.conf, g)),
                            'decoder.local_stats'))
            p._conv(L, D['local_convFM_loc'], grp(self.lm, g), grp(l2[0], g), K, p.h2, p.w2, res=qs.lq[g:g + 1],
                    res_mod=p.h2 * p.w2, name='decoder.local_convFM.local', lp_out='relu')
        p._resblock(L, D['local_ResMM'], l2[0], l2[1], l2[2], N, p.h2, p.w2, 'decoder.local_ResMM')
        p._conv(L, D['local_pred2'], l2[2], self.z2, N, p.h2, p.w2, relu_in=True, name='decoder.local_pred2.taps')
        L.append(Launch(ops.pred2_gather, (self.z2, D['local_pred2'].bias, self.qq), 'decoder.local_pred2.gather'))
        for g in range(G):
            L.append(Launch(ops.final_logits, (grp(self.p_up, g), self.unc[g], grp(self.conf, g), grp(self.qq, g), self.score[g:g + 1],
                                               p.pad, p.H0, p.W0), 'decoder.final_logits'))


class Engine:
    def __init__(self, model):
        dev = next(model.parameters()).device
        if dev.type != 'cuda':
            raise RuntimeError('AFB_URR runs on hand-written HIP kernels only: move the model to the GPU '
                               f'(model.to("cuda")); got {dev}.  There is no CPU fallback.')
        _lib.lib()
        self.device = dev
        self.model = model
        self.plans = {}
        self.precision = getattr(model, 'precision', 'fp32')
        if self.precision not in ops.MODES:
            raise ValueError(f"precision must be one of {sorted(ops.MODES)}, got {self.precision!r}")
        self.mode = ops.MODES[self.precision]
        pm = dict(getattr(model, 'precision_map', None) or {})
        for item in filter(None, os.environ.get('VFN_PRECISION_MAP', '').split(',')):
            k_, v_ = item.split('=')
            pm.setdefault(k_.strip(), v_.strip())
        for v_ in pm.values():
            if v_ not in ops.MODES:
                raise ValueError(f'precision map: unknown mode {v_!r}')
        self.pmap = sorted(((k_, ops.MODES[v_]) for k_, v_ in pm.items()), key=lambda kv: -len(kv[0]))
        self.mixed = bool(self.pmap)
        self.any_x3 = self.mode == 2 or any(m_ == 2 for _, m_ in self.pmap)
        self.fwd_count = 0
        self.mem_count = 0
        self.eager = False
        self._side = None
        self._side_busy = None
        from .refresh import Refresher
        self.refresher = Refresher(self.device)
        self._backward = None
        self._train_slot = 0
        self._batch = None
        self._pack(model)
        self._settle()

    def _settle(self):
        try:
            self.refresher.run()
        except RuntimeError:
            pass

    def refresh(self, check=True):
        self.refresher.run(verify=check)
        for layer in self._layers():
            if layer._w_lp:
                layer.refresh_derived()

    def _layers(self):
        def walk(o):
            if isinstance(o, (ConvLayer, Pred2Layer)):
                yield o
            elif isinstance(o, dict):
                for v in o.values():
                    yield from walk(v)
            elif isinstance(o, (list, tuple)):
                for v in o:
                    yield from walk(v)
        yield from walk([self.enc_q, self.enc_m, self.keyval, self.dec])

    def backward(self):
        from .backward import ModelBackward
        if self._backward is None:
            self._backward = ModelBackward(self)
            self._settle()
        self._backward.reset()
        return self._backward

    def use_winograd(self, layer, M, bf=0):
        if _WINOGRAD == '0' or getattr(layer, 'k', 0) != 3 or layer.stride != 1 or layer.pad != 1:
            return False
        if layer.cin % 32 or layer.cout % 4 or layer.cout < 32:
            return False
        if _WINOGRAD == '2':
            return True
        hit = (_WINO_TABLE_BF16.get((M, layer.cin, layer.cout)) if bf == 1 else None)
        if hit is None:
            hit = _WINO_TABLE.get((M, layer.cin, layer.cout))
        if hit is not None:
            return bool(hit)
        return layer.cin >= 128 and layer.cout >= 128 and M >= _WINOGRAD_MIN_M

    def layer_mode(self, name):
        for prefix, m_ in self.pmap:
            if name.startswith(prefix):
                return m_
        return self.mode

    def layer_precision(self, name):
        return {v: k for k, v in ops.MODES.items()}[self.layer_mode(name)]

    def _pack_trunk(self, enc):
        dev = self.device
        out = {}
        for lname in ('res2', 'res3', 'res4'):
            blocks = []
            for blk in getattr(enc, lname):
                reg = self.refresher
                b = dict(conv1=ConvLayer(blk.conv1, blk.bn1, dev, reg=reg), conv2=ConvLayer(blk.conv2, blk.bn2, dev, reg=reg),
                         conv3=ConvLayer(blk.conv3, blk.bn3, dev, reg=reg))
                if hasattr(blk, 'downsample'):
                    b['down'] = ConvLayer(blk.downsample[0], blk.downsample[1], dev, reg=reg)
                blocks.append(b)
            out[lname] = blocks
        return out

    def _pack(self, m):
        dev = self.device
        with torch.no_grad():
            self.mean = [float(x) for x in m.encoder_q.mean.flatten().cpu()]
            self.std = [float(x) for x in m.encoder_q.std.flatten().cpu()]
            mm = [float(x) for x in m.encoder_m.mean.flatten().cpu()]
            ms = [float(x) for x in m.encoder_m.std.flatten().cpu()]
            if mm != self.mean or ms != self.std:
                raise RuntimeError('encoder_m / encoder_q normalisation buffers differ; unsupported checkpoint')
            from .refresh import FORWARD, STEM
            reg = self.refresher
            self.stem_q_w = ops.pack_stem_weight([m.encoder_q.conv1.weight]).to(dev)
            self.stem_q_scale, self.stem_q_shift = [t.to(dev).clone() for t in W.bn_scale_shift(m.encoder_q.bn1)]
            stem_m = [m.encoder_m.conv1, m.encoder_m.conv1_m, m.encoder_m.conv1_o]
            self.stem_m_w = ops.pack_stem_weight([c.weight for c in stem_m]).to(dev)
            self.stem_m_scale, self.stem_m_shift = [t.to(dev).clone() for t in W.bn_scale_shift(m.encoder_m.bn1)]
            reg.add_filter(m.encoder_q.conv1.weight, self.stem_q_w, STEM)
            reg.add_epilogue(self.stem_q_scale, self.stem_q_shift, bn=m.encoder_q.bn1, eps=W.BN_EPS)
            plane = 0
            for c in stem_m:
                reg.add_filter(c.weight, self.stem_m_w, STEM, dst_row0=plane)
                plane += c.weight.shape[1]
            reg.add_epilogue(self.stem_m_scale, self.stem_m_shift, bn=m.encoder_m.bn1, eps=W.BN_EPS)
            self.enc_q = self._pack_trunk(m.encoder_q)
            self.enc_m = self._pack_trunk(m.encoder_m)
            kv = m.keyval_r4
            wk = torch.cat([kv.Key.weight.detach().float(), kv.Value.weight.detach().float()], 0)
            bk = torch.cat([kv.Key.bias.detach().float(), kv.Value.bias.detach().float()], 0)
            holder = type('KV', (), {})()
            holder.weight, holder.bias, holder.stride, holder.padding = wk, bk, (1, 1), (1, 1)
            self.keyval = ConvLayer(holder, None, dev)
            self.keyval.shift = self.keyval.shift.clone()
            row = 0
            self.keyval._wino_src = []
            for c in (kv.Key, kv.Value):
                reg.add_filter(c.weight, self.keyval.w, FORWARD, dst_row0=row)
                reg.add_epilogue(None, self.keyval.shift[row:row + c.weight.shape[0]], bias=c.bias)
                self.keyval._wino_src.append((reg, c.weight, 0, row))
                row += c.weight.shape[0]
            d = m.decoder
            cl = lambda c: ConvLayer(c, None, dev, reg=reg)
            rb = lambda r: dict(conv1=cl(r.conv1), conv2=cl(r.conv2))
            rf = lambda r: dict(convFS=cl(r.convFS), ResFS=rb(r.ResFS), ResMM=rb(r.ResMM))
            self.dec = dict(convFM_m=ConvLayer(d.convFM, None, dev, (0, DV), with_bias=False, reg=reg),
                            convFM_q=ConvLayer(d.convFM, None, dev, (DV, 2 * DV), reg=reg),
                            local_convFM_r1=ConvLayer(d.local_convFM, None, dev, (0, 64), reg=reg),
                            local_convFM_loc=ConvLayer(d.local_convFM, None, dev, (64, 128), with_bias=False, reg=reg),
                            ResMM=rb(d.ResMM), RF3=rf(d.RF3), RF2=rf(d.RF2), pred2=Pred2Layer(d.pred2, dev, reg=reg),
                            local_ResMM=rb(d.local_ResMM),
                            local_pred2=Pred2Layer(d.local_pred2, dev, reg=reg))

    def plan(self, H0, W0, obj_n, keep_acts=False, slot=0):
        key = (H0, W0, obj_n, bool(keep_acts)) + ((slot,) if slot else ())
        p = self.plans.get(key)
        if p is None:
            if len(self.plans) >= 6:
                self.plans.pop(next(iter(self.plans)))
            p = FramePlan(self, H0, W0, obj_n, keep_acts=bool(keep_acts))
            self.plans[key] = p
            if self.refresher._tables is None:
                self._settle()
        return p

    @staticmethod
    def _check_frame(frame, batch_ok=False):
        if frame.dim() != 4 or frame.shape[1] != 3 or frame.shape[0] < 1 or (frame.shape[0] != 1 and not batch_ok):
            raise RuntimeError(f'expected RGB frames [{"bs" if batch_ok else "1"},3,h,w], got {tuple(frame.shape)}')
        _lib.require_gpu(frame, 'frame')

    def _join_backward(self, plan=None):
        if self._backward is not None:
            if plan is None:
                self._backward.join()
            else:
                self._backward.wait_plan(plan)

    def memorize(self, frame, mask, training=False):
        self._check_frame(frame)
        self._join_backward()
        _, K, H, Wd = mask.shape
        p = self.plan(frame.shape[2], frame.shape[3], K, keep_acts=training)
        self.last_memorize = p
        self.mem_count += 1
        p.frame_in.copy_(frame[0])
        p.mask_in.copy_(mask[0])
        p.graphs.run(p.mem, eager=training or self.eager)
        kv = p.kv_m
        k_list = [kv[i, :, :DK].t() for i in range(K)]
        v_list = [kv[i, :, DK:].t() for i in range(K)]
        return k_list, v_list

    def segment(self, frame, fb, update_bank, training=False):
        self._check_frame(frame, batch_ok=True)
        bs = frame.shape[0]
        K = fb.obj_n
        H, Wd = frame.shape[2], frame.shape[3]
        if training and (H % 16 or Wd % 16):
            raise RuntimeError(f'training-mode segment does not pad (AFB_URR.py:278): {H}x{Wd} is not a multiple of 16')
        slot = 0
        batch = self._batched_slot(frame) if training and bs == 1 else None
        if batch is not None:
            p = batch[0]
        else:
            if training and _TRAIN_SLOTS > 1:
                slot, self._train_slot = self._train_slot, (self._train_slot + 1) % _TRAIN_SLOTS
            p = self.plan(H, Wd, K, keep_acts=training, slot=slot)
        self._join_backward(p)
        if fb._kbuf is None:
            raise RuntimeError('feature bank is empty: call fb.init_bank() first')
        if fb._hw != p.HW:
            raise RuntimeError('feature bank was built for a different frame size')
        out = p.score if bs == 1 else torch.empty(bs, K, H, Wd, device=self.device, dtype=torch.float32)
        for b in range(bs):
            fr = frame[b:b + 1]
            if batch is not None:
                qs, slot = batch[1], batch[2]
            else:
                qs, slot = self._take_prefetched(p, fr, frame._version) if b == 0 else (None, 0)
            if qs is None:
                qs = self._idle_set(p)
                if self._side_busy is not None:
                    torch.cuda.current_stream().wait_event(self._side_busy)
                qs.frames[0].copy_(fr[0])
                qs.keys, qs.held, qs.consumed, qs.stage, qs.n = [None, None], [None, None], [True, True], 0, 0
                p.graphs.run(qs.pre[1], eager=training or self.eager)
                slot = 0
            self._memory_read(p, fb, update_bank and b == 0, qs.kv_q[slot:slot + 1])
            p.graphs.run(qs.post[slot], eager=training or self.eager)
            self.last_query = (p, qs, slot)
            self.fwd_count += 1
            if bs > 1:
                out[b].copy_(p.score[0])
        return out

    def query_batch(self, frames, obj_n):
        n, H, Wd = frames.shape[0], frames.shape[2], frames.shape[3]
        if H % 16 or Wd % 16:
            raise RuntimeError(f'training-mode segment does not pad (AFB_URR.py:278): {H}x{Wd} is not a multiple of 16')
        self._join_backward()
        p = self.plan(H, Wd, obj_n, keep_acts=True)
        qs = p.batch_set(n)
        if self.refresher._tables is None:
            self._settle()
        qs.frames[:n].copy_(frames)
        for l in qs.pre[n]:
            l()
        qs.keys = [self._key(frames[i:i + 1]) for i in range(n)]
        qs.held, qs.consumed, qs.n, qs.stage = [frames] * n, [False] * n, n, 2
        self._batch = (p, qs)
        return qs

    def segment_batch(self, fb):
        if self._batch is None:
            raise RuntimeError('segment_batch follows query_batch')
        p, qs = self._batch
        if fb.obj_n != p.obj_n or fb._kbuf is None or fb._hw != p.HW:
            raise RuntimeError('feature bank does not match the batch (objects / frame size), or is empty')
        self._join_backward()
        b = qs.dec_batch()
        if self.refresher._tables is None:
            self._settle()
        K, G = p.obj_n, qs.n
        if _BATCH_MEMREAD:
            self._memory_read(b.mr, fb, False, qs.kv_q[0:G])
            b.dec_in.view(G, K, p.HW, DV).copy_(b.mr.dec_in.view(K, G, p.HW, DV).permute(1, 0, 2, 3))
        else:
            for g in range(G):
                self._memory_read(p, fb, False, qs.kv_q[g:g + 1], out=b.grp(b.dec_in, g))
        for l in b.post:
            l()
        qs.consumed = [True] * qs.n
        self.fwd_count += qs.n
        self.last_batch = (b, qs)
        return b.score

    @torch.no_grad()
    def segment_group(self, frames, fb, update_bank, prefetch=None):
        if isinstance(frames, (list, tuple)):
            for fr in frames:
                self._check_frame(fr)
                if fr.shape != frames[0].shape:
                    raise RuntimeError(f'segment_group: frames of one size, got {tuple(fr.shape)} and {tuple(frames[0].shape)}')
            G, H, Wd = len(frames), frames[0].shape[2], frames[0].shape[3]
        else:
            self._check_frame(frames, batch_ok=True)
            G, H, Wd = frames.shape[0], frames.shape[2], frames.shape[3]
        K = fb.obj_n
        p = self.plan(H, Wd, K)
        self._join_backward(p)
        if fb._kbuf is None:
            raise RuntimeError('feature bank is empty: call fb.init_bank() first')
        if fb._hw != p.HW:
            raise RuntimeError('feature bank was built for a different frame size')
        if G > MAX_GROUP:
            raise RuntimeError(f'segment_group: at most {MAX_GROUP} frames per group, got {G}')
        keys = [self._key(fr) for fr in frames] if isinstance(frames, (list, tuple)) else None
        qs = self._group_qset(p, G)
        hit = keys is not None and qs.stage == 2 and qs.keys == keys and not any(qs.consumed)
        b = qs.dec_batch()
        if self.refresher._tables is None:
            self._settle()
        if hit:
            torch.cuda.current_stream().wait_event(qs.done)
        else:
            if self._side_busy is not None:
                torch.cuda.current_stream().wait_event(self._side_busy)
            if isinstance(frames, (list, tuple)):
                for i, fr in enumerate(frames):
                    qs.frames[i].copy_(fr[0])
            else:
                qs.frames[:G].copy_(frames)
            p.graphs.run(qs.pre[qs.nq], eager=self.eager)
        qs.consumed, qs.held, qs.stage = [True] * G, [None] * G, 0
        for g in range(G):
            self._memory_read(p, fb, update_bank, qs.kv_q[g:g + 1], out=b.grp(b.dec_in, g))
        p.graphs.run(b.post, eager=self.eager)
        if prefetch:
            self.prefetch_group(prefetch, K)
        self.fwd_count += G
        return b.score[:G]

    @staticmethod
    def _group_qset(p, G):
        if G not in p._qbatch:
            built = [n for n, q_ in p._qbatch.items() if n > G and q_._dec_batch is not None]
            if built:
                return p._qbatch[min(built)]
        return p.batch_set(G)

    def prefetch_group(self, frames, obj_n):
        for fr in frames:
            self._check_frame(fr)
        G = len(frames)
        p = self.plan(frames[0].shape[2], frames[0].shape[3], obj_n)
        qs = self._group_qset(p, G)
        qs.dec_batch()
        if self.refresher._tables is None:
            self._settle()
        self.side_stream()
        ready = torch.cuda.Event()
        ready.record()
        with torch.cuda.stream(self._side):
            self._side.wait_event(ready)
            for i, fr in enumerate(frames):
                qs.frames[i].copy_(fr[0])
            p.graphs.run(qs.pre[qs.nq], eager=self.eager)
            qs.done = torch.cuda.Event()
            qs.done.record()
        self._side_busy = qs.done
        qs.keys = [self._key(fr) for fr in frames]
        qs.held = list(frames)
        qs.consumed = [False] * G
        qs.n, qs.stage = G, 2

    def _batched_slot(self, frame):
        if self._batch is None:
            return None
        p, qs = self._batch
        key = self._key(frame)
        for slot in range(qs.n):
            if qs.keys[slot] == key and not qs.consumed[slot]:
                qs.consumed[slot] = True
                return p, qs, slot
        return None

    @staticmethod
    def _key(frame, version=None):
        return (frame.data_ptr(), frame._version if version is None else version, tuple(frame.shape))

    def _take_prefetched(self, p, fr, version):
        key = self._key(fr, version)
        for qs in p.qsets:
            for slot in range(qs.n):
                if qs.stage > 0 and qs.keys[slot] == key and not qs.consumed[slot]:
                    if qs.stage == 1:
                        self.prefetch_finish(p)
                    torch.cuda.current_stream().wait_event(qs.done)
                    qs.consumed[slot] = True
                    qs.held[slot] = None
                    return qs, slot
        return None, 0

    def _idle_set(self, p):
        def live(qs):
            return 0 if qs.stage == 0 else sum(1 for i in range(qs.n) if not qs.consumed[i])
        return min(p.qsets, key=live)

    def prefetched_keys(self, p):
        return [qs.keys[i] for qs in p.qsets if qs.stage > 0 for i in range(qs.n) if not qs.consumed[i]]

    def prefetch_pending(self, p):
        return any(qs.stage == 1 for qs in p.qsets)

    def prefetch_begin(self, frames, obj_n, full=False):
        for fr in frames:
            self._check_frame(fr)
        n = len(frames)
        assert n in (1, 2)
        p = self.plan(frames[0].shape[2], frames[0].shape[3], obj_n)
        if self.prefetch_pending(p):
            self.prefetch_finish(p)
        qs = self._idle_set(p)
        self.side_stream()
        ready = torch.cuda.Event()
        ready.record()
        with torch.cuda.stream(self._side):
            self._side.wait_event(ready)
            for i, fr in enumerate(frames):
                qs.frames[i].copy_(fr[0])
            lst = qs.pre[n]
            cut = len(lst) if full else qs.split[n]
            p.graphs.run(lst, 0, cut, eager=self.eager)
            qs.done = torch.cuda.Event()
            qs.done.record()
        self._side_busy = qs.done
        qs.keys = [self._key(fr) for fr in frames] + [None] * (2 - n)
        qs.held = list(frames) + [None] * (2 - n)
        qs.consumed = [False] * n + [True] * (2 - n)
        qs.n = n
        qs.stage = 2 if full else 1
        return True

    def prefetch_finish(self, p=None):
        plans = [p] if p is not None else list(self.plans.values())
        for pl in plans:
            for qs in pl.qsets:
                if qs.stage != 1:
                    continue
                ready = torch.cuda.Event()
                ready.record()
                with torch.cuda.stream(self._side):
                    self._side.wait_event(ready)
                    pl.graphs.run(qs.pre[qs.n], qs.split[qs.n], None, eager=self.eager)
                    qs.done = torch.cuda.Event()
                    qs.done.record()
                self._side_busy = qs.done
                qs.stage = 2

    def side_stream(self):
        if self._side is None:
            self._side = _lib.independent_stream(self.device)
        return self._side

    def prefetch_query(self, frame, obj_n):
        return self.prefetch_begin([frame], obj_n, full=True)

    def _memory_read(self, p, fb, update_bank, kv_q=None, out=None):
        L = _lib.lib()
        s = stream()
        kv_q = p.kv_q if kv_q is None else kv_q
        out = p.dec_in if out is None else out
        K, HW, cap = fb.obj_n, p.HW, fb._cap
        nsplit_scan = pick_scan_slices(HW, K, fb.len_upper())
        scale = 1.0 / math.sqrt(DK)
        d = BankScanDesc()
        d.q, d.bank_k, d.bank_len, d.rowscale, d.part = ptr(kv_q), ptr(fb._kbuf), ptr(fb._len_dev), None, ptr(p.ml_part)
        d.stride_q, d.stride_k, d.stride_rs = 0, cap * DK, 0
        d.scale = scale
        d.ldq, d.q_per_obj, d.HW, d.obj_n, d.nsplit, d.mode = DK + DV, 0, HW, K, nsplit_scan, 0
        mr_mode = self.layer_mode('memread') if hasattr(self, 'layer_mode') else self.mode
        d.precision = mr_mode
        d.work_counter = ptr(p.work)
        klp, vlp = fb.lp_image() if mr_mode else (None, None)
        d.bank_k_lp = ptr(klp) if klp is not None else None
        scores = _scores_buffer(p, fb) if mr_mode == 0 else None
        if scores is not None:
            d.scores, d.stride_scores = ptr(scores), scores.shape[1]
        check(L.vfn_bank_scan(_lib.C.byref(d), s), 'vfn_bank_scan')
        check(L.vfn_bank_scan_finish(ptr(p.ml_part), nsplit_scan, HW, K, 0, ptr(p.ml), None, None, None, s),
              'vfn_bank_scan_finish')
        m = MemReadDesc()
        m.q = ptr(kv_q)
        m.qv = None
        m.bank_k, m.bank_v, m.bank_len, m.ml, m.o_part = ptr(fb._kbuf), ptr(fb._vbuf), ptr(fb._len_dev), ptr(p.ml), ptr(p.o_part)
        m.cnt = ptr(fb._cnt) if update_bank else None
        m.info, m.out = ptr(fb._ibuf), ptr(out)
        m.stride_k, m.stride_v, m.stride_cnt, m.stride_info = cap * DK, cap * DV, cap, cap * 2
        m.scale, m.thres = scale, 1e-3
        m.ldq, m.ldqv, m.ld_out, m.HW, m.obj_n = DK + DV, DK + DV, out.shape[-1], HW, K
        m.precision = mr_mode
        m.nsplit = pick_nsplit(HW, K, fb.len_upper(), QT_SCAN, MAX_SPLIT)
        if klp is not None:
            m.bank_k_lp, m.bank_v_lp = ptr(klp), ptr(vlp)
        if scores is not None:
            m.scores, m.stride_scores = ptr(scores), scores.shape[1]
        check(L.vfn_memread_apply(_lib.C.byref(m), s), 'vfn_memread_apply')
        check(L.vfn_memread_finish(_lib.C.byref(m), s), 'vfn_memread_finish')

    def capture(self, H0, W0, obj_n, group=0):
        p = self.plan(H0, W0, obj_n)
        if not _GRAPHS or self.eager or p.keep_acts:
            return 0
        before = p.graphs.captures
        torch.cuda.current_stream().synchronize()
        p.graphs.warm(p.mem)
        for qs in p.qsets:
            for n in qs.sizes:
                lst = qs.pre[n]
                p.graphs.warm(lst)
                if 0 < qs.split[n] < len(lst):
                    p.graphs.warm(lst, 0, qs.split[n])
                    p.graphs.warm(lst, qs.split[n], None)
            for L in qs.post:
                p.graphs.warm(L)
        for G in ([group] if group and group > 1 else []):
            qs = p.batch_set(G)
            b = qs.dec_batch()
            if self.refresher._tables is None:
                self._settle()
            p.graphs.warm(qs.pre[G])
            p.graphs.warm(b.post)
        torch.cuda.current_stream().synchronize()
        return p.graphs.captures - before

    def autotune(self, H0, W0, obj_n, iters=3, only_missing=False, shape_filter=None, cfg_filter=None):
        p = self.plan(H0, W0, obj_n)
        seen = {}
        side_sets = list(p.qsets) + ([] if p.keep_acts else list(p._qbatch.values()))
        side_lists = [id(qs.pre[n]) for qs in side_sets for n in qs.sizes]
        for lst in p.all_lists():
            for l in lst:
                l_side = id(lst) in side_lists
                if l.fn is ops.conv2d_launch:
                    d = l.args[0]
                    key = (d.M, d.Cout, d.KH * d.KW * d.Cin, int(l.args[2]))
                    if only_missing and key[:3] in _TABLES[key[3]]:
                        continue
                    if shape_filter is not None and not shape_filter(key[:3]):
                        continue
                    seen.setdefault(key, []).append((l, l_side))
        for key, launches in seen.items():
            d = launches[0][0].args[0]
            bf = key[3]
            best = tune_desc(d, bf, p.ws, p.cnt, iters=iters, cfg_filter=cfg_filter)
            _TABLES[bf][key[:3]] = best
            for l, in_q in launches:
                l.args = (l.args[0], apply_choice(l.args[0], best, p.ws_q if in_q else p.ws, p.cnt_q if in_q else p.cnt), bf)
        if seen:
            p.graphs.invalidate()
        return dict(_TABLES[self.mode])
```

### v-floodnet_amd/ops.py

```python
import ctypes as C
import os

import torch

from . import _lib
from ._lib import ptr, stream, check, ConvDesc


_cfg_tiles = None


def conv_cfg_tiles():
    global _cfg_tiles
    if _cfg_tiles is None:
        L = _lib.lib()
        out = []
        for c in range(L.vfn_conv_cfg_count()):
            bm, bn = C.c_int(), C.c_int()
            L.vfn_conv_cfg_tile(c, C.byref(bm), C.byref(bn))
            out.append((bm.value, bn.value))
        _cfg_tiles = tuple(out)
    return _cfg_tiles


def conv_cfg_wk(cfg):
    return _lib.lib().vfn_conv_cfg_wk(int(cfg))


def conv_cfg_tpb(cfg):
    return _lib.lib().vfn_conv_cfg_tpb(int(cfg))


def conv_cfgs(mode, _cache={}):
    mode = int(mode)
    if mode not in _cache:
        L = _lib.lib()
        _cache[mode] = tuple(c for c in range(L.vfn_conv_cfg_count()) if L.vfn_conv_cfg_modes(c) >> mode & 1)
    return _cache[mode]


def __getattr__(name):
    if name == 'BF16_CFGS':
        return conv_cfgs(1)
    raise AttributeError(f'module {__name__!r} has no attribute {name!r}')


def conv_cfg_kind(cfg):
    return _lib.lib().vfn_conv_cfg_kind(int(cfg))


SK_WS_FLOATS, SK_MAX_TILES = _lib.DEFINES['VFN_CONV_SK_WS_FLOATS'], _lib.DEFINES['VFN_CONV_SK_MAX_TILES']
_sk_scratch = {}


def streamk_scratch(device):
    key = str(device)
    if key not in _sk_scratch:
        _sk_scratch[key] = (torch.empty(SK_WS_FLOATS, dtype=torch.float32, device=device),
                            torch.zeros(SK_MAX_TILES, dtype=torch.int32, device=device))
    return _sk_scratch[key]


def set_streamk(desc, workspace, counters):
    assert workspace.numel() >= SK_WS_FLOATS and counters.numel() >= SK_MAX_TILES
    desc.ksplit, desc.split_from = 1, 0
    desc.partial, desc.tile_counters = ptr(workspace), ptr(counters)
    return desc


def conv_cfg_names(mode=0):
    L = _lib.lib()
    out = []
    for c in range(L.vfn_conv_cfg_count()):
        v = [C.c_int() for _ in range(5)]
        L.vfn_conv_cfg_info(c, *[C.byref(x) for x in v])
        bm, bn, wm, wn, dma = [x.value for x in v]
        wk, tpb = L.vfn_conv_cfg_wk(c), L.vfn_conv_cfg_tpb(c)
        if L.vfn_conv_cfg_kind(c) > 0:
            buf = C.create_string_buffer(96)
            L.vfn_conv_cfg_name(c, buf, 96)
            out.append(buf.value.decode())
            continue
        out.append(f'conv_igemm_dma_kernel<{bm}, {bn}, {wm}, {wn}, {dma}>' if dma else
                   f'conv_igemm_wk_kernel<{bm}, {bn}, {wm}, {wn}, {wk}, {4 if tpb > 1 else 3}, {tpb}, {int(mode)}>' if (wk > 1 or tpb > 1) else
                   f'conv_igemm_kernel<{bm}, {bn}, {wm}, {wn}, {int(mode)}>')
    return out


def pad_rows(wp, mult=256):
    cout = wp.shape[0]
    cp = (cout + mult - 1) // mult * mult
    if cp == cout:
        return wp.contiguous()
    out = torch.zeros(cp, wp.shape[1], dtype=wp.dtype, device=wp.device)
    out[:cout] = wp
    return out


def pack_weights_lp(wp, mode):
    if mode == 1:
        return wp.to(torch.bfloat16).contiguous()
    assert mode == 2 and wp.shape[1] % 32 == 0
    hi = wp.to(torch.bfloat16)
    lo = (wp - hi.float()).to(torch.bfloat16)
    cp, K = wp.shape
    return torch.cat([hi.view(cp, K // 32, 32), lo.view(cp, K // 32, 32)], dim=2).contiguous()


def make_conv_desc(x, wp, cout, kh, kw, stride, pad, out, scale=None, shift=None, res=None,
                   relu_in=False, relu_out=False, cin=None, in_ld=None, out_ld=None, res_ld=None,
                   N=None, H=None, W=None):
    if N is None:
        N, H, W = x.shape[0], x.shape[1], x.shape[2]
    in_ld = in_ld if in_ld is not None else x.shape[-1]
    cin = cin if cin is not None else in_ld
    Ho = (H + 2 * pad - kh) // stride + 1
    Wo = (W + 2 * pad - kw) // stride + 1
    out_ld = out_ld if out_ld is not None else out.shape[-1]
    d = ConvDesc()
    d.inp, d.w, d.scale, d.shift, d.res, d.out = ptr(x), ptr(wp), ptr(scale), ptr(shift), ptr(res), ptr(out)
    d.N, d.H, d.W, d.Cin, d.in_ld = N, H, W, cin, in_ld
    d.Ho, d.Wo, d.Cout, d.cout_pad = Ho, Wo, cout, wp.shape[0]
    d.out_ld = out_ld
    d.res_ld = res_ld if res_ld is not None else (res.shape[-1] if res is not None else 0)
    d.KH, d.KW, d.stride, d.pad = kh, kw, stride, pad
    d.relu_in, d.relu_out = int(relu_in), int(relu_out)
    d.M = N * Ho * Wo
    d.ksplit, d.split_from, d.partial = 1, 0, None
    d.tile_counters = None
    d.res_mod = 0
    d.w_packed = 0
    d.in_lp, d.out_lp_relu, d.out_lp = 0, 0, None
    d.mask, d.mask_ld, d.mask_after = None, 0, 0
    d.w_batch_rows = 0
    assert wp.shape[1] == kh * kw * cin
    return d


def use_packed_weights(desc, w_lp):
    desc.w = ptr(w_lp)
    desc.w_packed = 1
    return desc


def set_splitk(desc, ksplit, workspace, split_from=0, rows=None, counters=None):
    if ksplit > 1:
        rows = desc.M if rows is None else rows
        assert workspace is not None and workspace.numel() >= ksplit * rows * desc.Cout
        desc.ksplit, desc.split_from, desc.partial = int(ksplit), int(split_from), ptr(workspace)
        desc.tile_counters = ptr(counters) if counters is not None else None
    else:
        desc.ksplit, desc.split_from, desc.partial = 1, 0, None
        desc.tile_counters = None
    return desc


def tail_split_options(desc, bm, bn, max_split=8, mode=0):
    m_tiles = (desc.M + bm - 1) // bm
    n_tiles = (desc.Cout + bn - 1) // bn
    tiles = m_tiles * n_tiles
    out = []
    for unit in (256, 512):
        full = (tiles // unit) * unit
        full -= full % n_tiles
        if full <= 0 or full >= tiles:
            continue
        rows = desc.M - (full // n_tiles) * bm
        for ks in valid_splits(desc, max_split, mode)[1:]:
            out.append((full, ks, rows))
    return out


def valid_splits(desc, max_split=16, mode=0):
    nk = desc.KH * desc.KW * (desc.Cin // (64 if mode == 1 else 32))
    out = [1]
    if desc.Cout % 4 or desc.out_ld % 4 or (desc.res and desc.res_ld % 4):
        return out
    for s_ in range(2, max_split + 1):
        per = (nk + s_ - 1) // s_
        if per * (s_ - 1) < nk and per >= 4:
            out.append(s_)
    return out


MODES = {'fp32': 0, 'bf16': 1, 'bf16x3': 2}
_CONV_FN = ('vfn_conv2d_nhwc_f32', 'vfn_conv2d_nhwc_bf16', 'vfn_conv2d_nhwc_bf16x3')


WINO_GEMM_CFG0 = 1000
WINO_GEMM_TILES = ((128, 128, 4, 2), (64, 128, 2, 4), (128, 64, 4, 2), (64, 64, 2, 2))


def wino_gemm_cfg(tile_cfg, wgs=512):
    return WINO_GEMM_CFG0 + int(tile_cfg) + 8 * (int(wgs) // 128)


def wino_gemm_cfg_options(rows_pad, cout):
    out = []
    for tc in range(8):
        bm, bn = WINO_GEMM_TILES[tc & 3][:2]
        if rows_pad % bm or (bn > 64 and cout < 128):
            continue
        out += [wino_gemm_cfg(tc, w) for w in (256, 512, 768)]
    return out


PCONV_CFG0 = 2000


def pconv_cfg(tile_cfg, wgs=512):
    return PCONV_CFG0 + int(tile_cfg) + 8 * (int(wgs) // 128)


def pconv_eligible(desc, mode=0):
    lim = 0x7fffff00
    return (mode == 0 and desc.KH == 1 and desc.KW == 1 and desc.stride == 1 and desc.pad == 0 and not desc.mask and not desc.in_lp and
            not desc.out_lp and not desc.w_packed and not desc.w_batch_rows and desc.Cin % 32 == 0 and desc.in_ld % 4 == 0 and
            desc.M >= 1 and desc.M == desc.N * desc.H * desc.W and desc.M * desc.in_ld * 4 < lim and desc.M * desc.out_ld * 4 < lim and
            desc.cout_pad * desc.Cin * 4 < lim and
            (not desc.res or (desc.res_mod if desc.res_mod > 0 else desc.M) * desc.res_ld * 4 < lim))


def pconv_cfg_options(cout):
    out = []
    for tc in range(8):
        if WINO_GEMM_TILES[tc & 3][1] > 64 and cout < 128:
            continue
        out += [pconv_cfg(tc, w) for w in (256, 512, 768)]
    return out


def conv2d_launch(desc, cfg, mode=0):
    cfg = int(cfg)
    if cfg >= PCONV_CFG0:
        c = cfg - PCONV_CFG0
        if mode != 0:
            raise RuntimeError('the persistent 1x1 convolution is an f32 kernel')
        check(_lib.lib().vfn_conv1x1_persistent_f32(C.byref(desc), c & 7, (c >> 3) * 128, stream()), 'vfn_conv1x1_persistent_f32')
        return
    if cfg >= WINO_GEMM_CFG0:
        c, rows = cfg - WINO_GEMM_CFG0, desc.w_batch_rows
        if mode == 1 and rows > 0:
            check(_lib.lib().vfn_winograd_gemm_bf16(desc.inp, desc.w, desc.out, desc.M // rows, rows, desc.Cin, desc.Cout, desc.cout_pad, c & 7,
                                                    (c >> 3) * 128, stream()), 'vfn_winograd_gemm_bf16')
            return
        if mode != 0 or rows <= 0:
            raise RuntimeError('the persistent GEMM takes an f32 (or plain-bf16) Winograd-domain descriptor (w_batch_rows)')
        check(_lib.lib().vfn_winograd_gemm_f32(desc.inp, desc.w, desc.out, desc.M // rows, rows, desc.Cin, desc.Cout, desc.cout_pad, c & 7,
                                               (c >> 3) * 128, stream()), 'vfn_winograd_gemm_f32')
        return
    name = _CONV_FN[int(mode)]
    check(getattr(_lib.lib(), name)(C.byref(desc), cfg, stream()), name)


def conv_cfg_name(cfg, mode=0, _cache={}):
    cfg = int(cfg)
    if cfg >= WINO_GEMM_CFG0:
        c = (cfg - (PCONV_CFG0 if cfg >= PCONV_CFG0 else WINO_GEMM_CFG0)) & 7
        bm, bn, wm, wn = WINO_GEMM_TILES[c & 3]
        return f'wino_gemm_kernel<{bm}, {bn}, {wm}, {wn}, {1 + (c >> 2)}, {"true" if cfg >= PCONV_CFG0 else "false"}, {"true" if mode == 1 else "false"}>'
    if mode not in _cache:
        _cache[mode] = conv_cfg_names(mode)
    return _cache[mode][cfg]


def conv2d_nhwc(x, wp, cout, kh, kw, stride, pad, scale=None, shift=None, res=None,
                relu_in=False, relu_out=False, cfg=3, out=None, mode=0):
    N, H, W, _ = x.shape
    Ho = (H + 2 * pad - kh) // stride + 1
    Wo = (W + 2 * pad - kw) // stride + 1
    if out is None:
        out = torch.empty(N, Ho, Wo, cout, device=x.device, dtype=torch.float32)
    d = make_conv_desc(x, wp, cout, kh, kw, stride, pad, out, scale, shift, res, relu_in, relu_out)
    if mode == 0 and conv_cfg_kind(cfg) == 2:
        set_streamk(d, *streamk_scratch(x.device))
    conv2d_launch(d, cfg, mode)
    return out


_WINO_G = torch.tensor([[1 / 4, 0, 0], [-1 / 6, -1 / 6, -1 / 6], [-1 / 6, 1 / 6, -1 / 6], [1 / 24, 1 / 12, 1 / 6], [1 / 24, -1 / 12, 1 / 6], [0, 0, 1]],
                       dtype=torch.float64)
WINO_ROW_MULT = 256
_WINO_KROT = int(os.environ.get('VFN_KROT', '0'))


def pack_winograd_weight(w):
    cout, cin = w.shape[0], w.shape[1]
    assert tuple(w.shape[2:]) == (3, 3)
    g = w.detach().double().cpu()
    U = torch.einsum('ia,ocab,jb->ijoc', _WINO_G, g, _WINO_G)
    cp = (cout + 255) // 256 * 256
    out = torch.zeros(36, cp, cin, dtype=torch.float32)
    out[:, :cout] = U.reshape(36, cout, cin).float()
    return out.reshape(36 * cp, cin).contiguous()


def winograd_rows(N, H, W):
    t = N * ((H + 3) // 4) * ((W + 3) // 4)
    return (t + WINO_ROW_MULT - 1) // WINO_ROW_MULT * WINO_ROW_MULT


def pack_winograd_weight_bf16(w):
    return pack_winograd_weight(w).to(torch.bfloat16).contiguous()


def winograd_input(x, V, rows_pad, relu, N=None, H=None, W=None, cin=None, ld_x=None):
    if N is None:
        N, H, W = x.shape[0], x.shape[1], x.shape[2]
    cin = cin if cin is not None else x.shape[-1]
    ld_x = ld_x if ld_x is not None else x.shape[-1]
    if V.dtype == torch.bfloat16:
        check(_lib.lib().vfn_winograd_input_bf16(ptr(x), N, H, W, cin, ld_x, int(relu), ptr(V), rows_pad, stream()), 'vfn_winograd_input_bf16')
        return
    check(_lib.lib().vfn_winograd_input_f32(ptr(x), N, H, W, cin, ld_x, int(relu), ptr(V), rows_pad, stream()), 'vfn_winograd_input_f32')


def winograd_output(Mb, rows_pad, out, N, H, W, cout, scale, shift, res, res_ld, res_mod, relu_out, out_ld=None):
    check(_lib.lib().vfn_winograd_output_f32(ptr(Mb), rows_pad, N, H, W, cout, ptr(scale), ptr(shift), ptr(res), int(res_ld), int(res_mod),
                                             int(relu_out), ptr(out), out_ld if out_ld is not None else out.shape[-1], stream()),
          'vfn_winograd_output_f32')


def make_winograd_gemm_desc(V, U, Mb, rows_pad, cin, cout):
    d = make_conv_desc(V, U, cout, 1, 1, 1, 0, Mb, None, None, None, False, False, cin=cin, in_ld=cin, out_ld=cout, N=1, H=1, W=36 * rows_pad)
    d.cout_pad = U.shape[0] // 36
    d.w_batch_rows = rows_pad
    d.k_rot = _WINO_KROT
    return d


def winograd_gemm(V, U, Mb, rows_pad, cin, cout, cfg=0, wgs=0, comps=36):
    check(_lib.lib().vfn_winograd_gemm_f32(ptr(V), ptr(U), ptr(Mb), comps, rows_pad, cin, cout, U.shape[0] // comps, int(cfg), int(wgs), stream()),
          'vfn_winograd_gemm_f32')


def conv2d_winograd(x, w, scale=None, shift=None, res=None, relu_in=False, relu_out=False, cfg=2, res_mod=0):
    N, H, W, cin = x.shape
    cout = w.shape[0]
    rows = winograd_rows(N, H, W)
    U = pack_winograd_weight(w).to(x.device)
    V = torch.empty(36 * rows, cin, device=x.device, dtype=torch.float32)
    Mb = torch.empty(36 * rows, cout, device=x.device, dtype=torch.float32)
    out = torch.empty(N, H, W, cout, device=x.device, dtype=torch.float32)
    if rows > vfn_winograd_tiles(N, H, W):
        V.view(36, rows, cin)[:, vfn_winograd_tiles(N, H, W):].zero_()
    winograd_input(x, V, rows, relu_in)
    d = make_winograd_gemm_desc(V, U, Mb, rows, cin, cout)
    if conv_cfg_kind(cfg) == 2:
        set_streamk(d, *streamk_scratch(x.device))
    conv2d_launch(d, cfg, 0)
    winograd_output(Mb, rows, out, N, H, W, cout, scale, shift, res, res.shape[-1] if res is not None else 0, res_mod, relu_out)
    return out


def vfn_winograd_tiles(N, H, W):
    return N * ((H + 3) // 4) * ((W + 3) // 4)


def make_stem_desc(frame, mask, w, scale, shift, out, mean, std, N, H0, W0, pad, Hp, Wp):
    from ._lib import StemDesc
    d = StemDesc()
    d.frame, d.mask, d.w, d.scale, d.shift, d.out = ptr(frame), ptr(mask), ptr(w), ptr(scale), ptr(shift), ptr(out)
    for i in range(3):
        d.mean[i] = float(mean[i])
        d.std[i] = float(std[i])
    d.N, d.cin = N, (5 if mask is not None else 3)
    d.H0, d.W0 = H0, W0
    d.pad_top, d.pad_left = pad[2], pad[0]
    d.Hp, d.Wp, d.Ho, d.Wo = Hp, Wp, Hp // 2, Wp // 2
    return d


def stem_launch(desc):
    check(_lib.lib().vfn_stem_conv7x7_f32(C.byref(desc), stream()), 'vfn_stem_conv7x7_f32')


def pack_stem_weight(ws):
    w = torch.cat([x.detach().float() for x in ws], dim=1)
    P = w.shape[1]
    out = torch.zeros(P, 7, 8, 64, dtype=torch.float32, device=w.device)
    out[:, :, :7, :] = w.permute(1, 2, 3, 0)
    return out.reshape(P * 56, 64).contiguous()


def maxpool3x3s2(x, out):
    N, H, W, Cc = x.shape
    check(_lib.lib().vfn_maxpool3x3s2_nhwc_f32(ptr(x), ptr(out), N, H, W, Cc, stream()), 'vfn_maxpool3x3s2_nhwc_f32')
    return out


def upsample2x_add(s, pm, out, s_bcast, out_lp=None, lp_relu=False):
    N, h, w, Cc = out.shape
    if out_lp is not None:
        check(_lib.lib().vfn_upsample2x_add_lp_nhwc_f32(ptr(s), ptr(pm), ptr(out), ptr(out_lp), int(lp_relu), N, h, w, Cc,
                                                        int(s_bcast), stream()), 'vfn_upsample2x_add_lp_nhwc_f32')
        return out
    check(_lib.lib().vfn_upsample2x_add_nhwc_f32(ptr(s), ptr(pm), ptr(out), N, h, w, Cc, int(s_bcast), stream()),
          'vfn_upsample2x_add_nhwc_f32')
    return out


def rough_uncertainty(p, p_up, rough, unc):
    obj_n, h, w, _ = p.shape
    check(_lib.lib().vfn_rough_uncertainty_f32(ptr(p), ptr(p_up), ptr(rough), ptr(unc), obj_n, h, w, stream()),
          'vfn_rough_uncertainty_f32')


def local_stats(r1, rough, hs, hr, hm, lm, conf):
    obj_n, h, w = rough.shape
    Cc = r1.shape[-1]
    L = _lib.lib()
    if Cc == 64 and obj_n <= 4:
        check(L.vfn_local_stats_f32(ptr(r1), ptr(rough), ptr(lm), ptr(conf), obj_n, h, w, Cc, stream()), 'vfn_local_stats_f32')
        return
    check(L.vfn_local_hpass_f32(ptr(r1), ptr(rough), ptr(hs), ptr(hr), ptr(hm), obj_n, h, w, Cc, stream()),
          'vfn_local_hpass_f32')
    check(L.vfn_local_vpass_f32(ptr(hs), ptr(hr), ptr(hm), ptr(lm), ptr(conf), obj_n, h, w, Cc, stream()),
          'vfn_local_vpass_f32')


def local_stats_two_pass(r1, rough, hs, hr, hm, lm, conf):
    obj_n, h, w = rough.shape
    Cc = r1.shape[-1]
    L = _lib.lib()
    check(L.vfn_local_hpass_f32(ptr(r1), ptr(rough), ptr(hs), ptr(hr), ptr(hm), obj_n, h, w, Cc, stream()), 'vfn_local_hpass_f32')
    check(L.vfn_local_vpass_f32(ptr(hs), ptr(hr), ptr(hm), ptr(lm), ptr(conf), obj_n, h, w, Cc, stream()), 'vfn_local_vpass_f32')


def pred2_gather(z, bias, out):
    N, h, w, ldz = z.shape
    check(_lib.lib().vfn_pred2_gather_f32(ptr(z), ptr(bias), ptr(out), N, h, w, ldz, stream()), 'vfn_pred2_gather_f32')
    return out


def final_logits(p_up, unc, conf, q, score, pad, H0, W0):
    obj_n, h, w, _ = p_up.shape
    check(_lib.lib().vfn_final_logits_f32(ptr(p_up), ptr(unc), ptr(conf), ptr(q), ptr(score), obj_n, h, w,
                                          pad[2], pad[0], H0, W0, stream()), 'vfn_final_logits_f32')


def segment_uncertainty(score):
    bs, obj_n, H, W = score.shape
    assert score.is_contiguous()
    partial = torch.empty(bs * 64, device=score.device, dtype=torch.float32)
    out = torch.empty(1, device=score.device, dtype=torch.float32)
    check(_lib.lib().vfn_segment_uncertainty_f32(ptr(score), bs, obj_n, H * W, ptr(partial), ptr(out), stream()),
          'vfn_segment_uncertainty_f32')
    return out[0]


def segment_loss(score, label, lu, want_grad=True):
    bs, obj_n, H, W = score.shape
    assert score.is_contiguous()
    lab = label.to(device=score.device, dtype=torch.int32).contiguous()
    partial = torch.empty(2 * bs * 64, device=score.device, dtype=torch.float32)
    stats = torch.empty(3 + bs, device=score.device, dtype=torch.float32)
    grad = torch.empty_like(score) if want_grad else None
    check(_lib.lib().vfn_segment_loss_f32(ptr(score), ptr(lab), bs, obj_n, H * W, float(lu), ptr(partial), ptr(stats), ptr(grad),
                                          stream()), 'vfn_segment_loss_f32')
    return stats, grad


_wgrad_ws = {}
_WGRAD_INLAUNCH = os.environ.get('VFN_WGRAD_INLAUNCH', '0') == '1'
_STEM_WGRAD = os.environ.get('VFN_STEM_WGRAD', '1') == '1'


def conv_wgrad(x, gy, k, stride, pad, cin=None, cout=None, ld_x=None, relu=False, rowscale=None, out=None, accumulate=False,
               N=None, H=None, W=None, ksplit=None, batch=1, x_bstride=0, g_bstride=0):
    from ._lib import WgradDesc
    if N is None:
        N, H, W = x.shape[0], x.shape[1], x.shape[2]
    Ho, Wo = gy.shape[1], gy.shape[2]
    ld_x = ld_x if ld_x is not None else (x.stride(-2) if x.dim() >= 2 else x.shape[-1])
    cin = cin if cin is not None else x.shape[-1]
    cout = cout if cout is not None else gy.shape[-1]
    ld_g = gy.stride(-2)
    assert x.stride(-1) == 1 and gy.stride(-1) == 1
    Kc = k * k * cin
    if out is None:
        assert not accumulate
        out = torch.empty(cout, Kc, device=x.device, dtype=torch.float32)
    assert out.is_contiguous() and out.numel() == batch * cout * Kc
    M = N * Ho * Wo
    if (_STEM_WGRAD and k == 7 and stride == 2 and pad == 3 and cout == 64 and cin in (3, 5) and ld_x == cin and ld_g == 64 and batch == 1
            and not relu and ksplit is None and Ho == (H - 1) // 2 + 1 and Wo == (W - 1) // 2 + 1):
        L = _lib.lib()
        key = (str(x.device), torch.cuda.current_stream(x.device).cuda_stream, 'stem')
        need = L.vfn_stem_wgrad_scratch_floats(cin)
        part = _wgrad_ws.get(key)
        if part is None or part.numel() < need:
            part = _wgrad_ws[key] = torch.empty(need, device=x.device, dtype=torch.float32)
        check(L.vfn_stem_wgrad_f32(ptr(x), ptr(gy), ptr(rowscale), ptr(out), ptr(part), part.numel(), N, H, W, cin, Ho, Wo, int(accumulate),
                                   stream()), 'vfn_stem_wgrad_f32')
        return out
    tiles = ((cout + 63) // 64 if cout > 32 else 1) * k * k * ((cin + (31 if cin <= 32 else 63)) // (32 if cin <= 32 else 64))
    tiles *= batch
    if ksplit is None:
        ksplit = max(1, min(64, 2048 // tiles, M // 300))
        if batch == 1 and cin > 32:
            ksplit = max(1, min(64, M // 300, max((256 + tiles - 1) // tiles, M // 800)))
    d = WgradDesc()
    d.x, d.gy, d.rowscale, d.dw = ptr(x), ptr(gy), ptr(rowscale), ptr(out)
    d.N, d.H, d.W, d.Cin, d.ld_x = N, H, W, cin, ld_x
    d.Ho, d.Wo, d.Cout, d.ld_g = Ho, Wo, cout, ld_g
    d.k, d.stride, d.pad, d.relu, d.accumulate, d.ksplit = k, stride, pad, int(relu), int(accumulate), int(ksplit)
    d.batch, d.x_bstride, d.g_bstride = int(batch), int(x_bstride), int(g_bstride)
    part = None
    if ksplit > 1:
        key = (str(x.device), torch.cuda.current_stream(x.device).cuda_stream)
        need = batch * ksplit * cout * Kc
        hit = _wgrad_ws.get(key)
        if hit is None or hit[0].numel() < need:
            hit = (torch.empty(max(need, 8 * 1024 * 1024), device=x.device, dtype=torch.float32),
                   hit[1] if hit is not None else torch.zeros(16384, dtype=torch.int32, device=x.device))
            _wgrad_ws[key] = hit
        part = hit[0]
        if _WGRAD_INLAUNCH and tiles <= hit[1].numel() and need * 4 < 0x7fffff00:
            d.tile_counters = ptr(hit[1])
    d.partial = ptr(part)
    check(_lib.lib().vfn_conv_wgrad_f32(C.byref(d), stream()), 'vfn_conv_wgrad_f32')
    return out


def winograd_gy(gy, Z, rows_pad, N, H, W, cout, ld_g):
    check(_lib.lib().vfn_winograd_gy_f32(ptr(gy), N, H, W, cout, ld_g, ptr(Z), rows_pad, stream()), 'vfn_winograd_gy_f32')


_wino_wgrad_ws = {}


def conv_wgrad_winograd(x, gy, cin=None, cout=None, ld_x=None, relu=False, rowscale=None, out=None, accumulate=False, N=None, H=None, W=None):
    if N is None:
        N, H, W = x.shape[0], x.shape[1], x.shape[2]
    ld_x = ld_x if ld_x is not None else x.stride(-2)
    cin = cin if cin is not None else x.shape[-1]
    cout = cout if cout is not None else gy.shape[-1]
    ld_g = gy.stride(-2)
    assert cin % 4 == 0 and cout % 4 == 0 and x.stride(-1) == 1 and gy.stride(-1) == 1
    if out is None:
        assert not accumulate
        out = torch.empty(cout, 9 * cin, device=x.device, dtype=torch.float32)
    tiles = vfn_winograd_tiles(N, H, W)
    rows = winograd_rows(N, H, W)
    key = (str(x.device), torch.cuda.current_stream(x.device).cuda_stream)
    need = (36 * rows * cin, 36 * rows * cout, 36 * cout * cin)
    ws = _wino_wgrad_ws.get(key)
    if ws is None or any(t.numel() < n_ for t, n_ in zip(ws, need)):
        old = ws or (None, None, None)
        ws = tuple(t if (t is not None and t.numel() >= n_) else torch.empty(n_, device=x.device, dtype=torch.float32) for t, n_ in zip(old, need))
        _wino_wgrad_ws[key] = ws
    V, Z, dU = ws[0][:need[0]], ws[1][:need[1]], ws[2][:need[2]]
    winograd_input(x, V, rows, relu, N, H, W, cin, ld_x)
    winograd_gy(gy, Z, rows, N, H, W, cout, ld_g)
    conv_wgrad(V[:tiles * cin].view(1, 1, tiles, cin), Z[:tiles * cout].view(1, 1, tiles, cout), 1, 1, 0, cin=cin, cout=cout, ld_x=cin,
               out=dU.view(36 * cout, cin), N=1, H=1, W=tiles, batch=36, x_bstride=rows * cin, g_bstride=rows * cout)
    check(_lib.lib().vfn_winograd_dw_f32(ptr(dU), cout, cin, ptr(rowscale), ptr(out), int(accumulate), stream()), 'vfn_winograd_dw_f32')
    return out


def segment_uncertainty_backward(score, g_unc, g_score=None):
    bs, obj_n, H, W = score.shape
    assert score.is_contiguous() and g_unc.is_cuda and g_unc.numel() == 1 and g_unc.dtype == torch.float32
    if g_score is not None:
        g_score = g_score.to(torch.float32).contiguous()
        assert g_score.shape == score.shape
    partial = torch.empty(2 * bs * 64, device=score.device, dtype=torch.float32)
    stats = torch.empty(3 + bs, device=score.device, dtype=torch.float32)
    grad = torch.empty_like(score)
    check(_lib.lib().vfn_segment_uncertainty_backward_f32(ptr(score), bs, obj_n, H * W, ptr(g_unc), ptr(g_score), ptr(partial),
                                                          ptr(stats), ptr(grad), stream()), 'vfn_segment_uncertainty_backward_f32')
    return grad


def resize_bicubic(x, Ho, Wo, out=None):
    shp = x.shape
    Cc, Hi, Wi = shp[-3], shp[-2], shp[-1]
    assert x.is_contiguous() and x.numel() == Cc * Hi * Wi
    if out is None:
        out = torch.empty(*shp[:-2], Ho, Wo, device=x.device, dtype=torch.float32)
    check(_lib.lib().vfn_resize_bicubic_f32(ptr(x), ptr(out), Cc, Hi, Wi, Ho, Wo, stream()), 'vfn_resize_bicubic_f32')
    return out


def resize_nearest(x, Ho, Wo, out=None):
    shp = x.shape
    Cc, Hi, Wi = shp[-3], shp[-2], shp[-1]
    assert x.is_contiguous() and x.numel() == Cc * Hi * Wi
    if out is None:
        out = torch.empty(*shp[:-2], Ho, Wo, device=x.device, dtype=torch.float32)
    check(_lib.lib().vfn_resize_nearest_f32(ptr(x), ptr(out), Cc, Hi, Wi, Ho, Wo, stream()), 'vfn_resize_nearest_f32')
    return out


def softmax_objects(score, out=None):
    obj_n = score.shape[-3]
    n = score.shape[-2] * score.shape[-1]
    assert score.is_contiguous()
    if out is None:
        out = torch.empty_like(score)
    check(_lib.lib().vfn_softmax_objects_f32(ptr(score), ptr(out), obj_n, n, stream()), 'vfn_softmax_objects_f32')
    return out


def resize_argmax(prob, Ho, Wo, out=None):
    obj_n, Hi, Wi = prob.shape[-3], prob.shape[-2], prob.shape[-1]
    assert prob.is_contiguous()
    if out is None:
        out = torch.empty(Ho, Wo, device=prob.device, dtype=torch.uint8)
    check(_lib.lib().vfn_resize_argmax_u8(ptr(prob), ptr(out), obj_n, Hi, Wi, Ho, Wo, stream()), 'vfn_resize_argmax_u8')
    return out


def postprocess_pred(pred_np):
    import numpy as np
    pred_np = np.ascontiguousarray(pred_np, dtype=np.uint8)
    out = np.empty_like(pred_np)
    H, W = pred_np.shape
    check(_lib.lib().vfn_postprocess_pred_u8(pred_np.ctypes.data_as(C.c_void_p), H, W,
                                             out.ctypes.data_as(C.c_void_p)), 'vfn_postprocess_pred_u8')
    return out


def postprocess_pred_device(label, out=None, scratch=None):
    H, W = label.shape
    if out is None:
        out = torch.empty_like(label)
    if scratch is None:
        scratch = torch.empty(2 * H * W + 8, dtype=torch.int32, device=label.device)
    check(_lib.lib().vfn_postprocess_pred_device_u8(ptr(label), ptr(out), ptr(scratch), H, W, stream()),
          'vfn_postprocess_pred_device_u8')
    return out


def to_tensor_device(img_u8, out=None):
    H, W, c = img_u8.shape
    assert c == 3 and img_u8.dtype == torch.uint8 and img_u8.is_contiguous()
    if out is None:
        out = torch.empty(3, H, W, device=img_u8.device, dtype=torch.float32)
    check(_lib.lib().vfn_to_tensor_u8(ptr(img_u8), ptr(out), H, W, stream()), 'vfn_to_tensor_u8')
    return out


_palette_cache = {}


def overlay_device(frame, label, palette, alpha=0.4, cscale=1, out=None):
    _, H, W = frame.shape
    key = (tuple(palette), frame.device)
    if key not in _palette_cache:
        pal = (list(palette) + [0] * 768)[:768]
        _palette_cache[key] = (torch.tensor(pal, dtype=torch.uint8, device=frame.device),
                               torch.empty(1, dtype=torch.int32, device=frame.device))
    pal, scratch = _palette_cache[key]
    if out is None:
        out = torch.empty(H, W, 3, dtype=torch.uint8, device=frame.device)
    check(_lib.lib().vfn_overlay_u8(ptr(frame), ptr(label), ptr(pal), ptr(scratch), ptr(out), H, W,
                                    float(alpha), float(cscale), stream()), 'vfn_overlay_u8')
    return out


def row_norms(x, stride_obj, ld, dim, len_dev, rows, obj_n, nrm, inv, stride_n):
    check(_lib.lib().vfn_row_norms(ptr(x), int(stride_obj), ld, dim, ptr(len_dev), rows, obj_n, ptr(nrm), ptr(inv),
                                   int(stride_n), stream()), 'vfn_row_norms')


def scatter_mean_checked_launch(src, index, index_s0, out, status):
    D, S = src.shape
    check(_lib.lib().vfn_scatter_mean_checked_f32(ptr(src), src.stride(0), src.stride(1), ptr(index), int(index_s0), S, ptr(out),
                                                  out.stride(0), out.stride(1), D, out.shape[1], ptr(status), stream()),
          'vfn_scatter_mean_checked_f32')


def scatter_mean_launch(src, index_row, out):
    D, S = src.shape
    check(_lib.lib().vfn_scatter_mean_f32(ptr(src), src.stride(0), src.stride(1), ptr(index_row), S, ptr(out),
                                          out.stride(0), out.stride(1), D, stream()), 'vfn_scatter_mean_f32')


def _host_ints(values, cols, what):
    import numpy as np
    a = np.asarray(values)
    if a.ndim != 2 or a.shape[1] != cols or a.shape[0] < 1 or a.dtype.kind not in 'iu':
        raise ValueError(f'{what}: expected integers [R][{cols}] with R >= 1, got {a.dtype} {a.shape}')
    a = np.ascontiguousarray(a, dtype=np.int32)
    return a.ctypes.data_as(C.POINTER(C.c_int)), a.shape[0], a


def inverse_homography(homo_mat):
    import numpy as np
    m = np.asarray(homo_mat, dtype=np.float64)
    if m.shape != (3, 3) or not np.isfinite(m).all():
        raise ValueError(f'homography: expected a finite 3 x 3 matrix, got shape {m.shape}')
    inv = np.ascontiguousarray(np.linalg.inv(m), dtype=np.float64).reshape(9)
    if not np.isfinite(inv).all():
        raise ValueError('homography: the matrix has no finite inverse')
    return inv


def warp_perspective_u8(img, homo_mat, out=None, inverse=None):
    _lib.require_gpu(img, 'warp_perspective_u8: img')
    inv = inverse_homography(homo_mat) if inverse is None else inverse
    minv = inv.ctypes.data_as(C.POINTER(C.c_double))
    if not img.is_contiguous():
        raise ValueError('warp_perspective_u8: img must be contiguous')
    if out is None:
        out = torch.empty_like(img)
    if out.shape != img.shape or out.dtype != img.dtype or not out.is_contiguous() or out.data_ptr() == img.data_ptr():
        raise ValueError('warp_perspective_u8: out must be another contiguous tensor of the shape and type of img')
    if img.dtype == torch.float32 and img.dim() == 3 and img.shape[0] == 3:
        _, H, W = img.shape
        check(_lib.lib().vfn_warp_perspective_f32(ptr(img), ptr(out), H, W, minv, stream()), 'vfn_warp_perspective_f32')
    elif img.dtype == torch.uint8 and (img.dim() == 2 or (img.dim() == 3 and img.shape[2] in (1, 3))):
        H, W = img.shape[:2]
        check(_lib.lib().vfn_warp_perspective_u8(ptr(img), ptr(out), H, W, 1 if img.dim() == 2 else img.shape[2], minv, stream()),
              'vfn_warp_perspective_u8')
    else:
        raise ValueError(f'warp_perspective_u8: uint8 [H,W] / [H,W,1] / [H,W,3] or float32 [3,H,W], got {img.dtype} {tuple(img.shape)}')
    return out


def _log_args(log, t, R, what):
    if not (log.is_cuda and log.dtype == torch.int32 and log.dim() == 2 and log.is_contiguous() and log.shape[1] == R):
        raise ValueError(f'{what}: log must be a contiguous int32 [T][{R}] tensor on the GPU')
    if not 0 <= int(t) < log.shape[0]:
        raise ValueError(f'{what}: row {t} outside a log of {log.shape[0]} rows')


def waterline_scan(label, keypoints, log, t, water_label=1):
    _lib.require_gpu(label, 'waterline_scan: label')
    if label.dtype != torch.uint8 or label.dim() != 2 or not label.is_contiguous():
        raise ValueError('waterline_scan: label must be a contiguous uint8 [H,W] tensor')
    H, W = label.shape
    kp, R, a = _host_ints(keypoints, 2, 'waterline_scan: keypoints')
    _log_args(log, t, R, 'waterline_scan')
    if ((a[:, 0] < 0) | (a[:, 0] >= W) | (a[:, 1] < 0) | (a[:, 1] >= H)).any():
        raise ValueError(f'waterline_scan: key point outside the {W} x {H} image: {a.tolist()}')
    check(_lib.lib().vfn_waterline_scan(ptr(label), H, W, kp, R, int(water_label), ptr(log), log.shape[0], int(t), stream()),
          'vfn_waterline_scan')
    return log


def waterlevel_draw(overlay, boxes, log, t):
    _lib.require_gpu(overlay, 'waterlevel_draw: overlay')
    if overlay.dtype != torch.uint8 or overlay.dim() != 3 or overlay.shape[2] != 3 or not overlay.is_contiguous():
        raise ValueError('waterlevel_draw: overlay must be a contiguous uint8 [H,W,3] tensor')
    H, W, _ = overlay.shape
    bx, R, a = _host_ints(boxes, 4, 'waterlevel_draw: boxes')
    _log_args(log, t, R, 'waterlevel_draw')
    if (a[:, 2:] < 0).any() or (abs(a) > 1 << 24).any():
        raise ValueError(f'waterlevel_draw: boxes must have w, h >= 0 and image-sized coordinates: {a.tolist()}')
    check(_lib.lib().vfn_waterlevel_draw_u8(ptr(overlay), H, W, bx, R, ptr(log), log.shape[0], int(t), stream()),
          'vfn_waterlevel_draw_u8')
    return overlay


TRACK_MAX_SIDE, TRACK_MAX_RADIUS = _lib.DEFINES['VFN_TRACK_MAX_SIDE'], _lib.DEFINES['VFN_TRACK_MAX_RADIUS']


def track_luma(frame, out=None):
    _lib.require_gpu(frame, 'track_luma: frame')
    if frame.dtype != torch.float32 or frame.dim() != 3 or frame.shape[0] != 3 or not frame.is_contiguous():
        raise ValueError(f'track_luma: frame must be a contiguous float32 [3,H,W] tensor, got {frame.dtype} {tuple(frame.shape)}')
    _, H, W = frame.shape
    if out is None:
        out = torch.empty(H, W, dtype=torch.uint8, device=frame.device)
    if out.dtype != torch.uint8 or tuple(out.shape) != (H, W) or not out.is_contiguous() or out.device != frame.device:
        raise ValueError('track_luma: out must be a contiguous uint8 [H,W] tensor beside the frame')
    check(_lib.lib().vfn_track_luma_f32(ptr(frame), ptr(out), H, W, stream()), 'vfn_track_luma_f32')
    return out


class TrackState:

    def __init__(self, boxes, radius, device):
        import numpy as np
        self.radius = int(radius)
        self.R = boxes.shape[0]
        self.sizes = np.ascontiguousarray(boxes[:, 2:], dtype=np.int32)
        area = self.sizes[:, 0].astype(np.int64) * self.sizes[:, 1]
        self.offsets = [int(v) for v in np.concatenate([[0], np.cumsum(area)])]
        self.box = torch.zeros(self.R, 4, dtype=torch.int32, device=device)
        self.t16 = torch.zeros(max(1, self.offsets[-1]), dtype=torch.int16, device=device)
        self.acc = torch.zeros(self.R * (2 * self.radius + 1) ** 2 * 3, dtype=torch.int64, device=device)

    def template(self, r):
        w, h = (int(v) for v in self.sizes[r])
        return (self.t16[self.offsets[r]:self.offsets[r + 1]].cpu().numpy().view('uint16').astype('int64')).reshape(h, w)


def _luma_args(luma, what):
    _lib.require_gpu(luma, f'{what}: luma')
    if luma.dtype != torch.uint8 or luma.dim() != 2 or not luma.is_contiguous():
        raise ValueError(f'{what}: luma must be a contiguous uint8 [H,W] tensor')
    return luma.shape


def track_init(luma, boxes, radius=16):
    H, W = _luma_args(luma, 'track_init')
    bx, R, a = _host_ints(boxes, 4, 'track_init: boxes')
    if not 1 <= int(radius) <= TRACK_MAX_RADIUS:
        raise ValueError(f'track_init: search radius {radius} outside 1 .. {TRACK_MAX_RADIUS}')
    if R > 32 or (a[:, 2:] < 1).any() or (a[:, 2:] > TRACK_MAX_SIDE).any():
        raise ValueError(f'track_init: at most 32 boxes with sides 1 .. {TRACK_MAX_SIDE}: {a.tolist()}')
    if (a[:, :2] < 0).any() or (a[:, 0] + a[:, 2] > W).any() or (a[:, 1] + a[:, 3] > H).any():
        raise ValueError(f'track_init: box outside the {W} x {H} image: {a.tolist()}')
    st = TrackState(a, radius, luma.device)
    check(_lib.lib().vfn_track_init(ptr(luma), H, W, bx, R, st.radius, ptr(st.box), ptr(st.t16), st.t16.numel(), ptr(st.acc),
                                    st.acc.numel(), stream()), 'vfn_track_init')
    return st


def track_update(state, luma, box_log, ok_log, score_log, t):
    H, W = _luma_args(luma, 'track_update')
    R = state.R
    T = box_log.shape[0]
    for log, dt, shape, what in ((box_log, torch.int32, (T, R, 4), 'box_log'), (ok_log, torch.int32, (T, R), 'ok_log'),
                                 (score_log, torch.float32, (T, R), 'score_log')):
        if not (log.is_cuda and log.dtype == dt and tuple(log.shape) == shape and log.is_contiguous()):
            raise ValueError(f'track_update: {what} must be a contiguous {dt} tensor of shape {shape} on the GPU')
    if not 0 <= int(t) < T:
        raise ValueError(f'track_update: row {t} outside logs of {T} rows')
    check(_lib.lib().vfn_track_update(ptr(luma), H, W, state.sizes.ctypes.data_as(C.POINTER(C.c_int)), R, state.radius, ptr(state.box),
                                      ptr(state.t16), state.t16.numel(), ptr(state.acc), state.acc.numel(), ptr(box_log), ptr(ok_log),
                                      ptr(score_log), T, int(t), stream()), 'vfn_track_update')


def _dev_boxes(boxes, what):
    if not (boxes.is_cuda and boxes.dtype == torch.int32 and boxes.dim() == 2 and boxes.shape[1] == 4 and boxes.shape[0] >= 1
            and boxes.is_contiguous()):
        raise ValueError(f'{what}: boxes must be a contiguous int32 [R,4] tensor on the GPU')
    return boxes.shape[0]


def waterline_scan_dev(label, boxes, log, t, water_label=1):
    _lib.require_gpu(label, 'waterline_scan_dev: label')
    if label.dtype != torch.uint8 or label.dim() != 2 or not label.is_contiguous():
        raise ValueError('waterline_scan_dev: label must be a contiguous uint8 [H,W] tensor')
    H, W = label.shape
    R = _dev_boxes(boxes, 'waterline_scan_dev')
    _log_args(log, t, R, 'waterline_scan_dev')
    check(_lib.lib().vfn_waterline_scan_dev(ptr(label), H, W, ptr(boxes), R, int(water_label), ptr(log), log.shape[0], int(t), stream()),
          'vfn_waterline_scan_dev')
    return log


def waterlevel_draw_dev(overlay, boxes, log, t):
    _lib.require_gpu(overlay, 'waterlevel_draw_dev: overlay')
    if overlay.dtype != torch.uint8 or overlay.dim() != 3 or overlay.shape[2] != 3 or not overlay.is_contiguous():
        raise ValueError('waterlevel_draw_dev: overlay must be a contiguous uint8 [H,W,3] tensor')
    H, W, _ = overlay.shape
    R = _dev_boxes(boxes, 'waterlevel_draw_dev')
    _log_args(log, t, R, 'waterlevel_draw_dev')
    check(_lib.lib().vfn_waterlevel_draw_dev(ptr(overlay), H, W, ptr(boxes), R, ptr(log), log.shape[0], int(t), stream()),
          'vfn_waterlevel_draw_dev')
    return overlay
```

### v-floodnet_amd/refresh.py

```python
import ctypes as C

import torch

from . import _lib
from ._lib import check, stream, RefreshFilter, RefreshEpilogue

FORWARD, DGRAD, STEM, TAPS, WINO, WINO_DGRAD = 0, 1, 2, 3, 4, 5


def _addr(t):
    return 0 if t is None else t.data_ptr()


class Refresher:
    def __init__(self, device):
        self.device = device
        self._filters = []
        self._epilogues = []
        self._tables = None
        self._addresses = None
        self.runs = 0

    def add_filter(self, src, dst, kind, cin=None, cin_off=0, dst_ld=None, dst_row0=0, dst_col0=0, cout_ld=0, bn=None, eps=None):
        cout, cin_total, kh, kw = src.shape
        cin = cin_total if cin is None else cin
        self._filters.append(dict(src=src, dst=dst, kind=kind, cout=cout, cin=cin, cin_off=cin_off, cin_total=cin_total, kh=kh, kw=kw,
                                  dst_ld=dst.shape[-1] if dst_ld is None else dst_ld, dst_row0=dst_row0, dst_col0=dst_col0,
                                  cout_ld=cout_ld or cout, bn=bn, eps=eps))
        self._tables = None

    def add_epilogue(self, scale, shift, bn=None, bias=None, eps=None):
        C_ = (scale if scale is not None else shift).numel()
        self._epilogues.append(dict(scale=scale, shift=shift, bn=bn, bias=bias, eps=eps, C=C_))
        self._tables = None

    @staticmethod
    def _usable(t):
        return t is not None and t.is_cuda and t.dtype == torch.float32 and t.is_contiguous()

    def _collect(self):
        out = []
        for e in self._filters:
            ts = [e['src'].data, e['dst']] + ([e['bn'].weight.data, e['bn'].running_var] if e['bn'] is not None else [])
            for t in ts:
                if not self._usable(t):
                    raise RuntimeError('refresh: a parameter is not a contiguous f32 device tensor')
                out.append(t.data_ptr())
        for e in self._epilogues:
            bn = e['bn']
            ts = [bn.weight.data, bn.bias.data, bn.running_mean, bn.running_var] if bn is not None else ([e['bias'].data] if e['bias'] is not None else [])
            for t in ts:
                if not self._usable(t):
                    raise RuntimeError('refresh: a parameter is not a contiguous f32 device tensor')
                out.append(t.data_ptr())
            out += [_addr(e['scale']), _addr(e['shift'])]
        return out

    def _build(self):
        L = _lib.lib()
        per_block = L.vfn_refresh_elems_per_block()
        ft = (RefreshFilter * max(1, len(self._filters)))()
        block = 0
        for i, e in enumerate(self._filters):
            f = ft[i]
            f.src, f.dst = e['src'].data.data_ptr(), e['dst'].data_ptr()
            bn = e['bn']
            if bn is not None:
                f.gamma, f.var, f.eps = bn.weight.data.data_ptr(), bn.running_var.data_ptr(), float(e['eps'] if e['eps'] is not None else bn.eps)
            f.kind = e['kind']
            f.cout, f.cin, f.cin_off, f.cin_total, f.kh, f.kw = e['cout'], e['cin'], e['cin_off'], e['cin_total'], e['kh'], e['kw']
            f.dst_ld, f.dst_row0, f.dst_col0, f.cout_ld = e['dst_ld'], e['dst_row0'], e['dst_col0'], e['cout_ld']
            f.block0 = block
            elems = e['cout'] * e['cin'] * (1 if e['kind'] >= WINO else e['kh'] * e['kw'])
            block += (elems + per_block - 1) // per_block
        et = (RefreshEpilogue * max(1, len(self._epilogues)))()
        for i, e in enumerate(self._epilogues):
            q = et[i]
            bn = e['bn']
            if bn is not None:
                q.gamma, q.beta = bn.weight.data.data_ptr(), bn.bias.data.data_ptr()
                q.mean, q.var = bn.running_mean.data_ptr(), bn.running_var.data_ptr()
                q.eps = float(e['eps'] if e['eps'] is not None else bn.eps)
            elif e['bias'] is not None:
                q.beta = e['bias'].data.data_ptr()
            q.scale, q.shift, q.C = _addr(e['scale']) or None, _addr(e['shift']) or None, e['C']

        def upload(arr):
            host = torch.frombuffer(bytearray(bytes(arr)), dtype=torch.uint8)
            return host.to(self.device)
        self._tables = (upload(ft), len(self._filters), block, upload(et), len(self._epilogues))

    def run(self, verify=True):
        if verify or self._tables is None:
            addresses = self._collect()
            if self._tables is None or addresses != self._addresses:
                self._build()
                self._addresses = addresses
        ft, nf, blocks, et, ne = self._tables
        L = _lib.lib()
        if nf:
            check(L.vfn_refresh_filters_f32(C.c_void_p(ft.data_ptr()), nf, blocks, stream()), 'vfn_refresh_filters_f32')
        if ne:
            check(L.vfn_refresh_epilogues_f32(C.c_void_p(et.data_ptr()), ne, stream()), 'vfn_refresh_epilogues_f32')
        self.runs += 1
```

Baseline: 160.8.

## Add Winograd F(6x6,3x3) convolution path with input/output transforms and weight packing

Adds a larger-tile Winograd variant that uses 8x8 transforms producing 6x6 output tiles, with new input and output transform kernels, device-side weight-bank refresh, and a separate tuning table. Layers are routed to it by default when the Winograd table marks a shape as preferring it. Larger tiles cut the multiply count per output and the number of tiles, but they add transform work and 64 GEMM components instead of 36, and f32 numerical error grows. The input kernel also zero-fills the padded rows itself, so the separate zeroing pass is dropped.

```diff
diff --git a/include/vfn_winograd6.h b/include/vfn_winograd6.h
--- /dev/null
+++ b/include/vfn_winograd6.h
@@ -0,0 +1,16 @@
+#ifndef VFN_WINOGRAD6_H
+#define VFN_WINOGRAD6_H
+
+#ifdef __cplusplus
+extern "C" {
+#endif
+
+int vfn_winograd6_input_f32(const float* x, int N, int H, int W, int C, int ld_x, int relu, float* V, int rows_pad, void* stream);
+int vfn_winograd6_output_f32(const float* Mb, int rows_pad, int N, int H, int W, int Cout, const float* scale, const float* shift,
+                             const float* res, int res_ld, int res_mod, int relu_out, float* out, int out_ld, void* stream);
+
+#ifdef __cplusplus
+}
+#endif
+
+#endif
diff --git a/v-floodnet_amd/_lib.py b/v-floodnet_amd/_lib.py
--- a/v-floodnet_amd/_lib.py
+++ b/v-floodnet_amd/_lib.py
@@ -118,6 +118,8 @@
 with open(os.path.join(os.path.dirname(_HERE), 'include', 'vfn_hip.h')) as _f:
     DEFINES, ENUMS, STRUCTS, SIGNATURES = parse_header(_f.read())
 ALL_SYMBOLS = sorted(SIGNATURES)
+with open(os.path.join(os.path.dirname(_HERE), 'include', 'vfn_winograd6.h')) as _f:
+    SIGNATURES_WINOGRAD6 = parse_header(_f.read())[3]
 ABI_VERSION = DEFINES['VFN_ABI_VERSION']
 TRAIN_AUG_MAX_T, TRAIN_AUG_MAX_SIDE, TRAIN_AUG_MAX_OUT, TRAIN_AUG_MAX_OBJ = (
     DEFINES['VFN_TRAIN_AUG_MAX_' + _k] for _k in ('T', 'SIDE', 'OUT', 'OBJ'))
@@ -150,11 +152,11 @@
                 '(python -c "import __graft_entry__ as g; g.build()" or make -C v-floodnet_amd/csrc)')
         L = C.CDLL(LIB_PATH)
 
-        def declare(name):
+        def declare(name, signatures=SIGNATURES, header='vfn_hip.h'):
             if not hasattr(L, name):
-                raise RuntimeError(f'{LIB_PATH} lacks {name}, which include/vfn_hip.h declares: rebuild it (make -C v-floodnet_amd/csrc)')
+                raise RuntimeError(f'{LIB_PATH} lacks {name}, which include/{header} declares: rebuild it (make -C v-floodnet_amd/csrc)')
             fn = getattr(L, name)
-            fn.argtypes, fn.restype = SIGNATURES[name], C.c_int
+            fn.argtypes, fn.restype = signatures[name], C.c_int
             return fn
 
         if declare('vfn_abi_version')() != ABI_VERSION:
@@ -167,6 +169,8 @@
                                    f'{C.sizeof(cls)} in this binding: rebuild it (make -C v-floodnet_amd/csrc)')
         for name in SIGNATURES:
             declare(name)
+        for name in SIGNATURES_WINOGRAD6:
+            declare(name, SIGNATURES_WINOGRAD6, 'vfn_winograd6.h')
         _lib = L
     return _lib
 
diff --git a/v-floodnet_amd/csrc/conv_winograd.hip b/v-floodnet_amd/csrc/conv_winograd.hip
--- a/v-floodnet_amd/csrc/conv_winograd.hip
+++ b/v-floodnet_amd/csrc/conv_winograd.hip
@@ -1,6 +1,7 @@
 #include "common.h"
 #include "conv_internal.h"
 #include "../../include/vfn_hip.h"
+#include "../../include/vfn_winograd6.h"
 
 namespace {
 
@@ -162,6 +163,159 @@
     }
 }
 
+typedef float f32x2 __attribute__((ext_vector_type(2)));
+typedef unsigned u32x2 __attribute__((ext_vector_type(2)));
+
+__device__ __forceinline__ void bt8(const f32x2 (&v)[8], f32x2 (&t)[8]) {
+    const f32x2 e1 = v[2] + v[6] - 4.25f * v[4], o1 = v[1] + v[5] - 4.25f * v[3];
+    const f32x2 e2 = v[6] + 0.25f * v[2] - 1.25f * v[4], o2 = 0.5f * v[1] - 2.5f * v[3] + 2.f * v[5];
+    const f32x2 e3 = v[6] + 4.f * v[2] - 5.f * v[4], o3 = 2.f * v[1] - 2.5f * v[3] + 0.5f * v[5];
+    t[0] = v[0] - v[6] + 5.25f * (v[4] - v[2]);
+    t[1] = e1 + o1;
+    t[2] = e1 - o1;
+    t[3] = e2 + o2;
+    t[4] = e2 - o2;
+    t[5] = e3 + o3;
+    t[6] = e3 - o3;
+    t[7] = v[7] - v[1] + 5.25f * (v[3] - v[5]);
+}
+
+inline int winograd6_tiles(int N, int H, int W) { return N * ((H + 5) / 6) * ((W + 5) / 6); }
+
+__global__ __launch_bounds__(256, 2)
+void winograd6_input_kernel(const float* __restrict__ x, int N, int H, int W, int C, int ld_x, int relu, float* __restrict__ V,
+                            int rows_pad) {
+    const int th = (H + 5) / 6, tw = (W + 5) / 6, tiles = N * th * tw;
+    const int c2n = C / 2;
+    const long long total = (long long)rows_pad * c2n;
+    const __amdgpu_buffer_rsrc_t rx = __builtin_amdgcn_make_buffer_rsrc(const_cast<float*>(x), 0, (int)((size_t)N * H * W * ld_x * 4), 0x00020000);
+    const __amdgpu_buffer_rsrc_t rv = __builtin_amdgcn_make_buffer_rsrc(V, 0, (int)((size_t)64 * rows_pad * C * 4), 0x00020000);
+    const int comp4 = rows_pad * C * 4;
+    const float floor_ = relu ? 0.f : -INFINITY;
+    const long long i = vfn_xcd_block(blockIdx.x, gridDim.x) * (long long)blockDim.x + threadIdx.x;
+    if (i >= total) return;
+    {
+        const int c2 = (int)(i % c2n);
+        const int tile = (int)(i / c2n);
+        const int vo = (tile * C + c2 * 2) * 4;
+        if (tile >= tiles) {
+#pragma unroll
+            for (int xi = 0; xi < 64; ++xi) __builtin_amdgcn_raw_buffer_store_b64(u32x2{0u, 0u}, rv, vo, xi * comp4, 0);
+            return;
+        }
+        const int tx = tile % tw, ty = (tile / tw) % th, n = tile / (tw * th);
+        const int y0 = 6 * ty - 1, x0 = 6 * tx - 1;
+        const int base = (((n * H + y0) * W + x0) * ld_x + c2 * 2) * 4;
+        f32x2 d[8][8];
+#pragma unroll
+        for (int a = 0; a < 8; ++a) {
+#pragma unroll
+            for (int b = 0; b < 8; ++b) {
+                const bool ok = (unsigned)(y0 + a) < (unsigned)H && (unsigned)(x0 + b) < (unsigned)W;
+                d[a][b] = __builtin_bit_cast(f32x2, __builtin_amdgcn_raw_buffer_load_b64(rx, ok ? base + (a * W + b) * ld_x * 4 : 0x7ffffff0, 0, 0));
+            }
+        }
+#pragma unroll
+        for (int a = 0; a < 8; ++a)
+#pragma unroll
+            for (int b = 0; b < 8; ++b)
+#pragma unroll
+                for (int e = 0; e < 2; ++e) d[a][b][e] = vfn_floor_nan(d[a][b][e], floor_);
+#pragma unroll
+        for (int b = 0; b < 8; ++b) {
+            f32x2 v[8], t[8];
+#pragma unroll
+            for (int a = 0; a < 8; ++a) v[a] = d[a][b];
+            bt8(v, t);
+#pragma unroll
+            for (int a = 0; a < 8; ++a) d[a][b] = t[a];
+        }
+#pragma unroll
+        for (int a = 0; a < 8; ++a) {
+            f32x2 t[8];
+            bt8(d[a], t);
+#pragma unroll
+            for (int b = 0; b < 8; ++b) __builtin_amdgcn_raw_buffer_store_b64(__builtin_bit_cast(u32x2, t[b]), rv, vo, (a * 8 + b) * comp4, 0);
+        }
+    }
+}
+
+__device__ __forceinline__ void at8(const f32x2 (&m)[8], f32x2 (&y)[6]) {
+    const f32x2 s12 = m[1] + m[2], d12 = m[1] - m[2], s34 = m[3] + m[4], d34 = m[3] - m[4], s56 = m[5] + m[6], d56 = m[5] - m[6];
+    y[0] = m[0] + s12 + s34 + s56;
+    y[1] = d12 + 2.f * d34 + 0.5f * d56;
+    y[2] = s12 + 4.f * s34 + 0.25f * s56;
+    y[3] = d12 + 8.f * d34 + 0.125f * d56;
+    y[4] = s12 + 16.f * s34 + 0.0625f * s56;
+    y[5] = d12 + 32.f * d34 + 0.03125f * d56 + m[7];
+}
+
+template <bool RES>
+__global__ __launch_bounds__(256, RES ? 1 : 2)
+void winograd6_output_kernel(const float* __restrict__ Mb, int rows_pad, int N, int H, int W, int Cout,
+                             const float* __restrict__ scale, const float* __restrict__ shift, const float* __restrict__ res, int res_ld,
+                             int res_mod, int relu_out, float* __restrict__ out, int out_ld) {
+    const int th = (H + 5) / 6, tw = (W + 5) / 6;
+    const int c2n = Cout / 2;
+    const long long total = (long long)N * th * tw * c2n;
+    const int npix = N * H * W;
+    const __amdgpu_buffer_rsrc_t rm = __builtin_amdgcn_make_buffer_rsrc(const_cast<float*>(Mb), 0, (int)((size_t)64 * rows_pad * Cout * 4), 0x00020000);
+    const __amdgpu_buffer_rsrc_t ro = __builtin_amdgcn_make_buffer_rsrc(out, 0, (int)((size_t)npix * out_ld * 4), 0x00020000);
+    const __amdgpu_buffer_rsrc_t rr = __builtin_amdgcn_make_buffer_rsrc(const_cast<float*>(res ? res : Mb), 0,
+                                                                        res ? (int)((size_t)(res_mod > 0 ? res_mod : npix) * res_ld * 4) : 0, 0x00020000);
+    const float floor_ = relu_out ? 0.f : -INFINITY;
+    const int comp4 = rows_pad * Cout * 4;
+    const long long i = vfn_xcd_block(blockIdx.x, gridDim.x) * (long long)blockDim.x + threadIdx.x;
+    if (i >= total) return;
+    {
+        int iw = (int)i;
+        const int mo = ((iw / c2n) * Cout + (iw % c2n) * 2) * 4;
+        f32x2 m[8][8];
+#pragma unroll
+        for (int a = 0; a < 8; ++a)
+#pragma unroll
+            for (int b = 0; b < 8; ++b) m[a][b] = __builtin_bit_cast(f32x2, __builtin_amdgcn_raw_buffer_load_b64(rm, mo, (a * 8 + b) * comp4, 0));
+        f32x2 t[8][6];
+#pragma unroll
+        for (int a = 0; a < 8; ++a) at8(m[a], t[a]);
+        __builtin_amdgcn_sched_barrier(0);
+        asm volatile("" : "+v"(iw));
+        const int c2 = iw % c2n, tile = iw / c2n;
+        const int tx = tile % tw, ty = (tile / tw) % th, n = tile / (tw * th);
+        f32x2 sc = {1.f, 1.f}, sh = {0.f, 0.f};
+        if (scale) sc = *reinterpret_cast<const f32x2*>(scale + c2 * 2);
+        if (shift) sh = *reinterpret_cast<const f32x2*>(shift + c2 * 2);
+        const int y0 = 6 * ty, x0 = 6 * tx, row0 = (n * H + y0) * W + x0;
+        const int rb = ((row0 - (res_mod > 0 ? (n * H * W) / res_mod * res_mod : 0)) * res_ld + c2 * 2) * 4;
+        f32x2 rv[RES ? 6 : 1][RES ? 6 : 1];
+        if constexpr (RES) {
+#pragma unroll
+            for (int a = 0; a < 6; ++a)
+#pragma unroll
+                for (int b = 0; b < 6; ++b) {
+                    const bool ok = y0 + a < H && x0 + b < W;
+                    rv[a][b] = __builtin_bit_cast(f32x2, __builtin_amdgcn_raw_buffer_load_b64(rr, ok ? rb + (a * W + b) * res_ld * 4 : 0x7ffffff0, 0, 0));
+                }
+        }
+        const int oo = (row0 * out_ld + c2 * 2) * 4;
+#pragma unroll
+        for (int b = 0; b < 6; ++b) {
+            f32x2 col[8], y[6];
+#pragma unroll
+            for (int a = 0; a < 8; ++a) col[a] = t[a][b];
+            at8(col, y);
+#pragma unroll
+            for (int a = 0; a < 6; ++a) {
+                f32x2 v;
+#pragma unroll
+                for (int e = 0; e < 2; ++e) v[e] = vfn_floor_nan(y[a][e] * sc[e] + sh[e] + (RES ? rv[a][b][e] : 0.f), floor_);
+                const bool ok = y0 + a < H && x0 + b < W;
+                __builtin_amdgcn_raw_buffer_store_b64(__builtin_bit_cast(u32x2, v), ro, ok ? oo + (a * W + b) * out_ld * 4 : 0x7ffffff0, 0, 0);
+            }
+        }
+    }
+}
+
 __device__ __forceinline__ void a6(const f32x4 (&v)[4], f32x4 (&z)[6]) {
     const f32x4 e = v[0] + v[2], o = v[1] + v[3];
     const f32x4 e4 = v[0] + 4.f * v[2], o8 = 2.f * v[1] + 8.f * v[3];
@@ -543,6 +697,29 @@
     return vfn_check_launch();
 }
 
+extern "C" int vfn_winograd6_input_f32(const float* x, int N, int H, int W, int C, int ld_x, int relu, float* V, int rows_pad, void* stream) {
+    if (!x || !V || N < 1 || H < 1 || W < 1 || C < 4 || C % 4 || ld_x < C || ld_x % 4 || rows_pad < winograd6_tiles(N, H, W)) return VFN_ERR_ARG;
+    if (!tensors_fit_32bit(N, H, W, ld_x, 0, 0, 0) || (long long)64 * rows_pad * C * 4 >= 0x7fffff00LL) return VFN_ERR_ARG;
+    hipLaunchKernelGGL(winograd6_input_kernel, dim3(((long long)rows_pad * (C / 2) + 255) / 256), dim3(256), 0, (hipStream_t)stream, x, N, H, W, C, ld_x, relu,
+                       V, rows_pad);
+    return vfn_check_launch();
+}
+
+extern "C" int vfn_winograd6_output_f32(const float* Mb, int rows_pad, int N, int H, int W, int Cout, const float* scale, const float* shift,
+                                        const float* res, int res_ld, int res_mod, int relu_out, float* out, int out_ld, void* stream) {
+    if (!Mb || !out || N < 1 || H < 1 || W < 1 || Cout < 4 || Cout % 4 || out_ld < Cout || out_ld % 4 || (res && res_ld % 4) ||
+        rows_pad < winograd6_tiles(N, H, W) || res_mod < 0 || (res && res_mod % (H * W))) return VFN_ERR_ARG;
+    if (!tensors_fit_32bit(N, H, W, out_ld, res ? res_ld : 0, 0, res_mod) || (long long)64 * rows_pad * Cout * 4 >= 0x7fffff00LL) return VFN_ERR_ARG;
+    const dim3 grid(((long long)winograd6_tiles(N, H, W) * (Cout / 2) + 255) / 256);
+    if (res)
+        hipLaunchKernelGGL(winograd6_output_kernel<true>, grid, dim3(256), 0, (hipStream_t)stream, Mb, rows_pad, N, H, W, Cout, scale, shift, res, res_ld,
+                           res_mod, relu_out, out, out_ld);
+    else
+        hipLaunchKernelGGL(winograd6_output_kernel<false>, grid, dim3(256), 0, (hipStream_t)stream, Mb, rows_pad, N, H, W, Cout, scale, shift, res, res_ld,
+                           res_mod, relu_out, out, out_ld);
+    return vfn_check_launch();
+}
+
 extern "C" int vfn_winograd_output_masked_f32(const float* Mb, int rows_pad, int N, int H, int W, int Cout, const float* res, int res_ld,
                                               const float* mask, int mask_ld, int mask_after, float* out, int out_ld, void* stream) {
     if (!Mb || !out || N < 1 || H < 1 || W < 1 || Cout < 4 || Cout % 4 || out_ld < Cout || out_ld % 4 || (res && res_ld % 4) ||
diff --git a/v-floodnet_amd/csrc/refresh.hip b/v-floodnet_amd/csrc/refresh.hip
--- a/v-floodnet_amd/csrc/refresh.hip
+++ b/v-floodnet_amd/csrc/refresh.hip
@@ -7,6 +7,41 @@
 
 __device__ __forceinline__ float bn_scale(const float* gamma, const float* var, float eps, int c) {
     return __fdiv_rn(gamma[c], __fsqrt_rn(__fadd_rn(var[c], eps)));
+}
+
+__device__ void winograd6_banks(const vfn_refresh_filter& e, long long base) {
+#pragma clang fp contract(off)
+    const long long pairs = (long long)e.cout * e.cin;
+    const double G[8][3] = {{1.0, 0.0, 0.0}, {-2.0 / 9, -2.0 / 9, -2.0 / 9}, {-2.0 / 9, 2.0 / 9, -2.0 / 9},
+                            {1.0 / 90, 1.0 / 45, 2.0 / 45}, {1.0 / 90, -1.0 / 45, 2.0 / 45},
+                            {32.0 / 45, 16.0 / 45, 8.0 / 45}, {32.0 / 45, -16.0 / 45, 8.0 / 45}, {0.0, 0.0, 1.0}};
+    for (int i = threadIdx.x; i < ELEMS_PER_BLOCK; i += 256) {
+        const long long idx = base + i;
+        if (idx >= pairs) return;
+        const int ci = (int)(idx % e.cin), co = (int)(idx / e.cin);
+        const float* g = e.src + ((size_t)co * e.cin_total + e.cin_off + ci) * 9;
+        const float sc = e.gamma ? bn_scale(e.gamma, e.var, e.eps, co) : 1.f;
+        double w[3][3];
+#pragma unroll
+        for (int t = 0; t < 9; ++t) {
+            float v = g[t];
+            if (e.gamma) v = __fmul_rn(v, sc);
+            w[t / 3][t % 3] = (double)v;
+        }
+        double tmp[8][3];
+#pragma unroll
+        for (int a = 0; a < 8; ++a)
+#pragma unroll
+            for (int b = 0; b < 3; ++b) tmp[a][b] = (G[a][0] * w[0][b] + G[a][1] * w[1][b]) + G[a][2] * w[2][b];
+        float* dst = e.dst + (size_t)(e.dst_row0 + co) * e.dst_ld + ci;
+#pragma unroll
+        for (int a = 0; a < 8; ++a)
+#pragma unroll
+            for (int b = 0; b < 8; ++b) {
+                const double u = (tmp[a][0] * G[b][0] + tmp[a][1] * G[b][1]) + tmp[a][2] * G[b][2];
+                dst[(size_t)(a * 8 + b) * e.cout_ld * e.dst_ld] = (float)u;
+            }
+    }
 }
 
 __global__ __launch_bounds__(256)
@@ -19,6 +54,10 @@
     const vfn_refresh_filter e = table[lo];
     const int T = e.kh * e.kw;
     const long long base = (long long)((int)blockIdx.x - e.block0) * ELEMS_PER_BLOCK;
+    if (e.kind == 6) {
+        winograd6_banks(e, base);
+        return;
+    }
     if (e.kind >= 4) {
         const long long pairs = (long long)e.cout * e.cin;
         const double G[6][3] = {{0.25, 0.0, 0.0}, {-1.0 / 6, -1.0 / 6, -1.0 / 6}, {-1.0 / 6, 1.0 / 6, -1.0 / 6},
diff --git a/v-floodnet_amd/engine.py b/v-floodnet_amd/engine.py
--- a/v-floodnet_amd/engine.py
+++ b/v-floodnet_amd/engine.py
@@ -19,6 +19,16 @@
 _TUNED_BF16X3_PATH = _TUNED_PATH.replace('tuned_gfx950.json', 'tuned_gfx950_bf16x3.json')
 _TABLES = (_TUNED, _TUNED_BF16, _TUNED_BF16X3)
 _TABLE_PATHS = (_TUNED_PATH, _TUNED_BF16_PATH, _TUNED_BF16X3_PATH)
+_TUNED_WINO6 = {}
+_TUNED_WINO6_PATH = _TUNED_PATH.replace('tuned_gfx950.json', 'tuned_gfx950_wino6.json')
+
+
+def is_wino6_desc(d):
+    return d.w_batch_rows > 0 and d.M == 64 * d.w_batch_rows
+
+
+def table_of(d, mode):
+    return _TUNED_WINO6 if mode == 0 and is_wino6_desc(d) else _TABLES[mode]
 
 
 def _load_tuned():
@@ -26,7 +36,7 @@
     import os
     if os.environ.get('VFN_IGNORE_TUNED') == '1':
         return
-    for path, table in zip(_TABLE_PATHS, _TABLES):
+    for path, table in zip(_TABLE_PATHS + (_TUNED_WINO6_PATH,), _TABLES + (_TUNED_WINO6,)):
         alt = os.environ.get('VFN_TUNED_DIR')
         if alt and os.path.isfile(os.path.join(alt, os.path.basename(path))):
             path = os.path.join(alt, os.path.basename(path))
@@ -38,8 +48,8 @@
 
 def save_tuned(path=None, mode=0):
     import json
-    table = _TABLES[mode]
-    with open(path or _TABLE_PATHS[mode], 'w') as f:
+    table = _TUNED_WINO6 if mode == 'wino6' else _TABLES[mode]
+    with open(path or (_TUNED_WINO6_PATH if mode == 'wino6' else _TABLE_PATHS[mode]), 'w') as f:
         json.dump({','.join(str(x) for x in k): list(v) for k, v in sorted(table.items())}, f, indent=0)
 
 
@@ -62,6 +72,7 @@
 MAX_GROUP = 16
 _TRAIN_SLOTS = int(os.environ.get('VFN_TRAIN_SLOTS', 2))
 _WINOGRAD = os.environ.get('VFN_WINOGRAD', '1')
+_WINOGRAD_F6 = os.environ.get('VFN_WINOGRAD_F6', '1')
 _WINOGRAD_LP = os.environ.get('VFN_WINOGRAD_LP', '1') == '1'
 _WINOGRAD_MIN_M = int(os.environ.get('VFN_WINOGRAD_MIN_M', 10000))
 _WINO_TABLE = {}
@@ -206,7 +217,7 @@
             continue
         if cfg_filter is not None and not cfg_filter(key, c):
             continue
-        if d.cout_pad < ((d.Cout + bn - 1) // bn) * bn:
+        if d.cout_pad < ((d.Cout + bn - 1) // bn) * bn or (d.w_batch_rows > 0 and d.w_batch_rows % bm):
             continue
         if (bn > 64 and d.Cout <= 32) or (bn > 128 and d.Cout < 256):
             continue
@@ -271,6 +282,11 @@
                     continue
                 w = self.w[:self.cout].view(self.cout, 3, 3, self.cin).permute(0, 3, 1, 2)
                 t.copy_(ops.pack_winograd_weight(w).to(t.device))
+            elif mode == 'wino6':
+                if self._wino_src is not None:
+                    continue
+                w = self.w[:self.cout].view(self.cout, 3, 3, self.cin).permute(0, 3, 1, 2)
+                t.copy_(ops.pack_winograd6_weight(w).to(t.device))
             elif mode == 'wino_bf16':
                 w = self.w[:self.cout].view(self.cout, 3, 3, self.cin).permute(0, 3, 1, 2)
                 t.copy_(ops.pack_winograd_weight_bf16(w).to(t.device))
@@ -294,6 +310,18 @@
                     reg.add_filter(weight, self._w_lp['wino'], WINO, cin=self.cin, cin_off=cin_off, dst_ld=self.cin, dst_row0=row0,
                                    cout_ld=self._w_lp['wino'].shape[0] // 36)
         return self._w_lp['wino']
+
+    def w_wino6(self):
+        if 'wino6' not in self._w_lp:
+            assert self.k == 3
+            w = self.w[:self.cout].view(self.cout, 3, 3, self.cin).permute(0, 3, 1, 2)
+            self._w_lp['wino6'] = ops.pack_winograd6_weight(w).to(self.w.device)
+            if self._wino_src is not None:
+                from .refresh import WINO6
+                for reg, weight, cin_off, row0 in self._wino_src:
+                    reg.add_filter(weight, self._w_lp['wino6'], WINO6, cin=self.cin, cin_off=cin_off, dst_ld=self.cin, dst_row0=row0,
+                                   cout_ld=self._w_lp['wino6'].shape[0] // 64)
+        return self._w_lp['wino6']
 
     def w_wino_bf16(self):
         if 'wino_bf16' not in self._w_lp:
@@ -532,7 +560,9 @@
             f32_out = True
         if ((bf == 0 or (bf == 1 and _WINOGRAD_LP and not self.keep_acts and layer.cin % 64 == 0)) and in_ld is None and
                 (_WINOGRAD_TRAIN or not self.keep_acts) and x.shape[-1] == layer.cin and self.eng.use_winograd(layer, N * H * Wd, bf)):
-            return self._conv_winograd(lst, layer, x, out, N, H, Wd, res, relu_in, relu_out, name, out_ld, res_mod, bf)
+            tile = 6 if (bf == 0 and not self.keep_acts and res_mod % (H * Wd) == 0 and
+                         self.eng.winograd_tile(layer, N * H * Wd) == 6) else 4
+            return self._conv_winograd(lst, layer, x, out, N, H, Wd, res, relu_in, relu_out, name, out_ld, res_mod, bf, tile)
         d = ops.make_conv_desc(x, layer.w, layer.cout, layer.k, layer.k, layer.stride, layer.pad, out,
                                layer.scale, layer.shift, res, relu_in, relu_out,
                                cin=layer.cin, in_ld=in_ld if in_ld is not None else x.shape[-1],
@@ -559,30 +589,35 @@
         lst.append(Launch(ops.conv2d_launch, (d, cfg, bf), f'{name}[{d.M}x{layer.cout}x{K}]', 2.0 * d.M * layer.cout * K))
         return out
 
-    def _conv_winograd(self, lst, layer, x, out, N, H, Wd, res, relu_in, relu_out, name, out_ld, res_mod, bf=0):
-        rows = ops.winograd_rows(N, H, Wd)
+    def _conv_winograd(self, lst, layer, x, out, N, H, Wd, res, relu_in, relu_out, name, out_ld, res_mod, bf=0, tile=4):
+        comps = 64 if tile == 6 else 36
+        rows = ops.winograd6_rows(N, H, Wd) if tile == 6 else ops.winograd_rows(N, H, Wd)
         key = id(self._ws_cur)
-        need_v, need_m = 36 * rows * layer.cin, 36 * rows * layer.cout
+        need_v, need_m = comps * rows * layer.cin, comps * rows * layer.cout
         V, Mb = self._wino.get(key, (None, None))
         if V is None or V.numel() < need_v or Mb.numel() < need_m:
             dev = self.eng.device
             V = torch.zeros(max(need_v, V.numel() if V is not None else 0), device=dev)
             Mb = torch.empty(max(need_m, Mb.numel() if Mb is not None else 0), device=dev)
             self._wino[key] = (V, Mb)
-        Mb = Mb[:need_m].view(36 * rows, layer.cout)
+        Mb = Mb[:need_m].view(comps * rows, layer.cout)
         if bf == 1:
             V = V.view(torch.bfloat16)[:need_v].view(36 * rows, layer.cin)
             U = layer.w_wino_bf16()
         else:
-            V = V[:need_v].view(36 * rows, layer.cin)
-            U = layer.w_wino()
-        lst.append(Launch(ops.winograd_input, (x, V, rows, relu_in, N, H, Wd, layer.cin, x.shape[-1]), name + '.wino_in'))
-        dg = ops.make_winograd_gemm_desc(V, U, Mb, rows, layer.cin, layer.cout)
+            V = V[:need_v].view(comps * rows, layer.cin)
+            U = layer.w_wino6() if tile == 6 else layer.w_wino()
+        lst.append(Launch(ops.winograd_input, (x, V, rows, relu_in, N, H, Wd, layer.cin, x.shape[-1], tile), name + '.wino_in'))
+        dg = ops.make_winograd_gemm_desc(V, U, Mb, rows, layer.cin, layer.cout, comps)
         if bf:
             choice = _TABLES[bf].get((dg.M, layer.cout, layer.cin))
             if choice is None or choice[0] < ops.WINO_GEMM_CFG0:
                 tc = 5 if rows % 64 == 0 and layer.cout >= 128 and rows >= 1024 else 3
                 choice = (ops.wino_gemm_cfg(tc, 512), 1, 0)
+        elif tile == 6:
+            choice = _TUNED_WINO6.get((dg.M, layer.cout, layer.cin))
+            if choice is None or choice[0] not in ops.wino_gemm_cfg_options(rows, layer.cout):
+                choice = (ops.wino_gemm_cfg(5 if layer.cout >= 128 else 7, 768), 1, 0)
         else:
             choice = choose_cfg(dg.M, layer.cout, layer.cin, 0)
         cfg = apply_choice(dg, choice, self._ws_cur, self._cnt_cur)
@@ -590,7 +625,7 @@
         self._lp_state.pop((out.data_ptr(), tuple(out.shape)), None)
         lst.append(Launch(ops.winograd_output, (Mb, rows, out, N, H, Wd, layer.cout, layer.scale, layer.shift, res,
                                                 res.shape[-1] if res is not None else 0, res_mod, relu_out,
-                                                out_ld if out_ld is not None else out.shape[-1]), name + '.wino_out'))
+                                                out_ld if out_ld is not None else out.shape[-1], tile), name + '.wino_out'))
         return out
 
     def _trunk(self, lst, enc, bufs, N, prefix, acts=None):
@@ -905,6 +940,13 @@
             return bool(hit)
         return layer.cin >= 128 and layer.cout >= 128 and M >= _WINOGRAD_MIN_M
 
+    def winograd_tile(self, layer, M):
+        if _WINOGRAD_F6 == '0':
+            return 4
+        if _WINOGRAD_F6 == '2':
+            return 6
+        return 6 if _WINOGRAD != '2' and _WINO_TABLE.get((M, layer.cin, layer.cout)) == 2 else 4
+
     def layer_mode(self, name):
         for prefix, m_ in self.pmap:
             if name.startswith(prefix):
@@ -1353,8 +1395,8 @@
                 l_side = id(lst) in side_lists
                 if l.fn is ops.conv2d_launch:
                     d = l.args[0]
-                    key = (d.M, d.Cout, d.KH * d.KW * d.Cin, int(l.args[2]))
-                    if only_missing and key[:3] in _TABLES[key[3]]:
+                    key = (d.M, d.Cout, d.KH * d.KW * d.Cin, int(l.args[2]), is_wino6_desc(d))
+                    if only_missing and key[:3] in table_of(d, key[3]):
                         continue
                     if shape_filter is not None and not shape_filter(key[:3]):
                         continue
@@ -1362,8 +1404,11 @@
         for key, launches in seen.items():
             d = launches[0][0].args[0]
             bf = key[3]
-            best = tune_desc(d, bf, p.ws, p.cnt, iters=iters, cfg_filter=cfg_filter)
-            _TABLES[bf][key[:3]] = best
+            if key[4]:
+                best = tune_desc(d, bf, p.ws, p.cnt, iters=iters, cfg_filter=lambda k_, c_: c_ >= ops.WINO_GEMM_CFG0 and (cfg_filter is None or cfg_filter(k_, c_)))
+            else:
+                best = tune_desc(d, bf, p.ws, p.cnt, iters=iters, cfg_filter=cfg_filter)
+            table_of(d, bf)[key[:3]] = best
             for l, in_q in launches:
                 l.args = (l.args[0], apply_choice(l.args[0], best, p.ws_q if in_q else p.ws, p.cnt_q if in_q else p.cnt), bf)
         if seen:
diff --git a/v-floodnet_amd/ops.py b/v-floodnet_amd/ops.py
--- a/v-floodnet_amd/ops.py
+++ b/v-floodnet_amd/ops.py
@@ -300,30 +300,59 @@
     return (t + WINO_ROW_MULT - 1) // WINO_ROW_MULT * WINO_ROW_MULT
 
 
+_WINO6_G = torch.tensor([[1, 0, 0], [-2 / 9, -2 / 9, -2 / 9], [-2 / 9, 2 / 9, -2 / 9], [1 / 90, 1 / 45, 2 / 45], [1 / 90, -1 / 45, 2 / 45],
+                         [32 / 45, 16 / 45, 8 / 45], [32 / 45, -16 / 45, 8 / 45], [0, 0, 1]], dtype=torch.float64)
+WINO6_ROW_MULT = 64
+
+
+def pack_winograd6_weight(w):
+    cout, cin = w.shape[0], w.shape[1]
+    assert tuple(w.shape[2:]) == (3, 3)
+    g, G = w.detach().double().cpu(), _WINO6_G
+    col = lambda k: G[:, k].view(8, 1)
+    tmp = (col(0) * g[:, :, None, 0, :] + col(1) * g[:, :, None, 1, :]) + col(2) * g[:, :, None, 2, :]
+    U = (tmp[..., 0, None] * G[:, 0] + tmp[..., 1, None] * G[:, 1]) + tmp[..., 2, None] * G[:, 2]
+    cp = (cout + 255) // 256 * 256
+    out = torch.zeros(64, cp, cin, dtype=torch.float32)
+    out[:, :cout] = U.permute(2, 3, 0, 1).reshape(64, cout, cin).float()
+    return out.reshape(64 * cp, cin).contiguous()
+
+
+def winograd6_tiles(N, H, W):
+    return N * ((H + 5) // 6) * ((W + 5) // 6)
+
+
+def winograd6_rows(N, H, W):
+    return (winograd6_tiles(N, H, W) + WINO6_ROW_MULT - 1) // WINO6_ROW_MULT * WINO6_ROW_MULT
+
+
 def pack_winograd_weight_bf16(w):
     return pack_winograd_weight(w).to(torch.bfloat16).contiguous()
 
 
-def winograd_input(x, V, rows_pad, relu, N=None, H=None, W=None, cin=None, ld_x=None):
+def winograd_input(x, V, rows_pad, relu, N=None, H=None, W=None, cin=None, ld_x=None, tile=4):
     if N is None:
         N, H, W = x.shape[0], x.shape[1], x.shape[2]
     cin = cin if cin is not None else x.shape[-1]
     ld_x = ld_x if ld_x is not None else x.shape[-1]
+    if tile == 6:
+        check(_lib.lib().vfn_winograd6_input_f32(ptr(x), N, H, W, cin, ld_x, int(relu), ptr(V), rows_pad, stream()), 'vfn_winograd6_input_f32')
+        return
     if V.dtype == torch.bfloat16:
         check(_lib.lib().vfn_winograd_input_bf16(ptr(x), N, H, W, cin, ld_x, int(relu), ptr(V), rows_pad, stream()), 'vfn_winograd_input_bf16')
         return
     check(_lib.lib().vfn_winograd_input_f32(ptr(x), N, H, W, cin, ld_x, int(relu), ptr(V), rows_pad, stream()), 'vfn_winograd_input_f32')
 
 
-def winograd_output(Mb, rows_pad, out, N, H, W, cout, scale, shift, res, res_ld, res_mod, relu_out, out_ld=None):
-    check(_lib.lib().vfn_winograd_output_f32(ptr(Mb), rows_pad, N, H, W, cout, ptr(scale), ptr(shift), ptr(res), int(res_ld), int(res_mod),
-                                             int(relu_out), ptr(out), out_ld if out_ld is not None else out.shape[-1], stream()),
-          'vfn_winograd_output_f32')
-
-
-def make_winograd_gemm_desc(V, U, Mb, rows_pad, cin, cout):
-    d = make_conv_desc(V, U, cout, 1, 1, 1, 0, Mb, None, None, None, False, False, cin=cin, in_ld=cin, out_ld=cout, N=1, H=1, W=36 * rows_pad)
-    d.cout_pad = U.shape[0] // 36
+def winograd_output(Mb, rows_pad, out, N, H, W, cout, scale, shift, res, res_ld, res_mod, relu_out, out_ld=None, tile=4):
+    name = 'vfn_winograd6_output_f32' if tile == 6 else 'vfn_winograd_output_f32'
+    check(getattr(_lib.lib(), name)(ptr(Mb), rows_pad, N, H, W, cout, ptr(scale), ptr(shift), ptr(res), int(res_ld), int(res_mod),
+                                    int(relu_out), ptr(out), out_ld if out_ld is not None else out.shape[-1], stream()), name)
+
+
+def make_winograd_gemm_desc(V, U, Mb, rows_pad, cin, cout, comps=36):
+    d = make_conv_desc(V, U, cout, 1, 1, 1, 0, Mb, None, None, None, False, False, cin=cin, in_ld=cin, out_ld=cout, N=1, H=1, W=comps * rows_pad)
+    d.cout_pad = U.shape[0] // comps
     d.w_batch_rows = rows_pad
     d.k_rot = _WINO_KROT
     return d
@@ -334,22 +363,26 @@
           'vfn_winograd_gemm_f32')
 
 
-def conv2d_winograd(x, w, scale=None, shift=None, res=None, relu_in=False, relu_out=False, cfg=2, res_mod=0):
+def conv2d_winograd(x, w, scale=None, shift=None, res=None, relu_in=False, relu_out=False, cfg=2, res_mod=0, tile=4):
     N, H, W, cin = x.shape
     cout = w.shape[0]
-    rows = winograd_rows(N, H, W)
-    U = pack_winograd_weight(w).to(x.device)
-    V = torch.empty(36 * rows, cin, device=x.device, dtype=torch.float32)
-    Mb = torch.empty(36 * rows, cout, device=x.device, dtype=torch.float32)
+    if tile == 6:
+        comps, rows, tiles = 64, winograd6_rows(N, H, W), winograd6_tiles(N, H, W)
+        U = pack_winograd6_weight(w).to(x.device)
+    else:
+        comps, rows, tiles = 36, winograd_rows(N, H, W), vfn_winograd_tiles(N, H, W)
+        U = pack_winograd_weight(w).to(x.device)
+    V = torch.empty(comps * rows, cin, device=x.device, dtype=torch.float32)
+    Mb = torch.empty(comps * rows, cout, device=x.device, dtype=torch.float32)
     out = torch.empty(N, H, W, cout, device=x.device, dtype=torch.float32)
-    if rows > vfn_winograd_tiles(N, H, W):
-        V.view(36, rows, cin)[:, vfn_winograd_tiles(N, H, W):].zero_()
-    winograd_input(x, V, rows, relu_in)
-    d = make_winograd_gemm_desc(V, U, Mb, rows, cin, cout)
+    if rows > tiles and tile != 6:
+        V.view(comps, rows, cin)[:, tiles:].zero_()
+    winograd_input(x, V, rows, relu_in, tile=tile)
+    d = make_winograd_gemm_desc(V, U, Mb, rows, cin, cout, comps)
     if conv_cfg_kind(cfg) == 2:
         set_streamk(d, *streamk_scratch(x.device))
     conv2d_launch(d, cfg, 0)
-    winograd_output(Mb, rows, out, N, H, W, cout, scale, shift, res, res.shape[-1] if res is not None else 0, res_mod, relu_out)
+    winograd_output(Mb, rows, out, N, H, W, cout, scale, shift, res, res.shape[-1] if res is not None else 0, res_mod, relu_out, tile=tile)
     return out
 
 
diff --git a/v-floodnet_amd/refresh.py b/v-floodnet_amd/refresh.py
--- a/v-floodnet_amd/refresh.py
+++ b/v-floodnet_amd/refresh.py
@@ -5,7 +5,7 @@
 from . import _lib
 from ._lib import check, stream, RefreshFilter, RefreshEpilogue
 
-FORWARD, DGRAD, STEM, TAPS, WINO, WINO_DGRAD = 0, 1, 2, 3, 4, 5
+FORWARD, DGRAD, STEM, TAPS, WINO, WINO_DGRAD, WINO6 = 0, 1, 2, 3, 4, 5, 6
 
 
 def _addr(t):
```

Result: faster. 167.1 (median of 6 runs) (+3.9%).
